# ddlee-cn/LeRF-PyTorch

Hardware: AMD Instinct MI355X
Metric: Mpix/s LeRF-G x2 SR (2K->4K) (higher is better)
Workload: dtype i32+f32 (u8 io); 1 GPU; LeRF-G LUT x2 SR, 1920x1080->3840x2160 RGB uint8, S=2, max_sigma=10 (BASELINE configs[1]); input=noise, mode=frames, parallelism=independent frames per GPU, no data-path collective, ranks_reported_by_rccl=1, channels=3, library=lerf-pytorch_amd/liblerf_hip.so

## Files before the change

### include/lerf_hip.h

```cpp
#ifndef LERF_HIP_H
#define LERF_HIP_H

#include <stddef.h>
#include <stdint.h>

#ifdef __cplusplus
extern "C" {
#endif

#define LERF_ABI_VERSION 7
#define LERF_MAX_MODES 5
#define LERF_LUT_ENTRIES 83521
#define LERF_MAX_SUPPORT 8

enum {
    LERF_OK = 0,
    LERF_EINVAL = -1,
    LERF_EUNSUPPORTED = -2,
    LERF_ELAUNCH = -3,
    LERF_ENODEVICE = -4
};

enum { LERF_U8 = 0, LERF_F32 = 1, LERF_F64 = 2, LERF_I16 = 3 };
enum {
    LERF_KIND_GAUSS = 0,
    LERF_KIND_LINEAR = 1,
    LERF_KIND_NEAREST = 2,
    LERF_KIND_CUBIC = 3,
    LERF_KIND_BILINEAR = 4,
    LERF_KIND_LANCZOS2 = 5,
    LERF_KIND_LANCZOS3 = 6
};

enum {
    LERF_PAD_CONSTANT = 0,
    LERF_PAD_EDGE = 1,
    LERF_PAD_REFLECT = 2,
    LERF_PAD_SYMMETRIC = 3,
    LERF_PAD_WRAP = 4
};

typedef struct {
    const void* ptr;
    int dtype;
    int64_t sy, sx, sc;
} lerf_plane_t;

typedef struct {
    void* ptr;
    int dtype;
    int64_t sy, sx, sc;
} lerf_mplane_t;

typedef struct {
    int n_modes1;
    int n_modes2;
    char modes1[LERF_MAX_MODES];
    char modes2[LERF_MAX_MODES];
    int oC;
    const int8_t* s1[LERF_MAX_MODES];
    const int8_t* s2[LERF_MAX_MODES][2];
    const void* fused_pack;
} lerf_luts_t;

typedef struct {
    int S;
    int out_h, out_w;
    const int32_t* left_r;
    const float* dis_r;
    const int32_t* left_c;
    const float* dis_c;
    const double* dis_r64;
    const double* dis_c64;
    int pad_mode;
    int tie_queue_cap;
    int roi_y, roi_x;
    int roi_h, roi_w;
    int flags;
    int out_row_pitch;
} lerf_sr_geo_t;
#define LERF_GEO_FORCE_GENERAL 1
#define LERF_GEO_SINGLE_LAUNCH 2
#define LERF_GEO_X2_TABLES 16
#define LERF_GEO_NO_PERSIST 32
#define LERF_GEO_TILE_ROWS_64 64
#define LERF_GEO_TILE_ROWS_32 128
#define LERF_GEO_TILE_ROWS_16 256
#define LERF_GEO_INPUT_DEVICE 4
#define LERF_GEO_INPUT_HOST 8

typedef struct {
    int S;
    int out_h, out_w;
    double minv[9];
    int pad_r_lo, pad_r_hi, pad_c_lo, pad_c_hi;
    int pad_mode;
    int out_y0, out_x0, src_y0;
} lerf_warp_geo_t;

#define LERF_REMAP_PADS_FROM_MAP (-1)
typedef struct {
    int S;
    int out_h, out_w;
    const void* coords;
    int coords_dtype;
    int64_t row_stride;
    int pad_mode;
    int pad_r_lo, pad_c_lo;
} lerf_remap_geo_t;

int lerf_abi_version(void);
const char* lerf_strerror(int code);

int lerf_device_count(void);

int lerf_mode_offsets(char mode, int rot, int8_t dy[4], int8_t dx[4]);

int lerf_sr_axis_tables(int n_in, int n_out, double scale, int S,
                        int32_t* left, double* dis64, float* dis32, int32_t* pads);

int lerf_sr_axis_tables_f32(int n_in, int n_out, double scale, int S, int32_t* left, float* dis32, int32_t* pads);

int lerf_out_size(int n_in, double scale);

int lerf_invert3x3(const double m[9], double out[9]);

int lerf_warp_pads(const double minv[9], int in_h, int in_w, int out_h, int out_w, int S,
                   int32_t pads[4]);


int lerf_lut_interp_i16(const lerf_plane_t* img, int img_h, int img_w, int C,
                        int h, int w, const int8_t dy[4], const int8_t dx[4],
                        const int8_t* lut, int oC, int interval, int16_t* out, void* stream);

int lerf_lut_interp(const lerf_plane_t* img, int img_h, int img_w, int C, int h, int w, const int8_t dy[4], const int8_t dx[4],
                    const int8_t* lut, int oC, int interval, const lerf_mplane_t* out, void* stream);

#define LERF_INTERP_ACCUMULATE 1
#define LERF_INTERP_LDS 2
#define LERF_INTERP_DIRECT 4
#define LERF_INTERP_TILE64 8
#define LERF_INTERP_TILE32 16
#define LERF_INTERP_LUT_PLANAR 32
#define LERF_LUT_PLANE_BYTES 83584
int lerf_lut_interp_ex(const lerf_plane_t* img, int img_h, int img_w, int C, int h, int w, const int8_t dy[4], const int8_t dx[4],
                       const int8_t* lut, int oC, int interval, const lerf_mplane_t* out, int flags, void* stream);

enum { LERF_EPI_DIV = 0, LERF_EPI_MUL = 1, LERF_EPI_ADD = 2, LERF_EPI_CLIP = 3, LERF_EPI_ROUND = 4 };
#define LERF_EPI_MAX_OPS 8
typedef struct { int op; double a, b; } lerf_epi_op_t;
int lerf_numer_epilogue_f32(const int16_t* acc, int64_t n, int interval, const lerf_epi_op_t* ops, int n_ops, float* out, void* stream);

size_t lerf_fused_lutpack_bytes(const lerf_luts_t* luts);
int lerf_fused_lutpack_build(const lerf_luts_t* luts, void* buf, void* stream);

int lerf_lut_stages_u8(const lerf_plane_t* img, int H, int W, int C,
                       const lerf_luts_t* luts,
                       const lerf_mplane_t* feat, const lerf_mplane_t* hyper,
                       void* stream);

int lerf_resize(const lerf_plane_t* feat, const lerf_plane_t hyper[3],
                int H, int W, int C, const lerf_sr_geo_t* geo,
                int kind, double max_sigma, const lerf_mplane_t* out, void* stream);

int lerf_warp(const lerf_plane_t* feat, const lerf_plane_t hyper[3],
              int H, int W, int C, const lerf_warp_geo_t* geo,
              int kind, double max_sigma, const lerf_mplane_t* out, void* stream);

int lerf_stages_packed_u8(const uint8_t* img, int64_t in_sn, int n, int H, int W, int C,
                          const lerf_luts_t* luts, uint32_t* packed, int64_t packed_sn,
                          void* workspace, size_t workspace_bytes, void* stream);

int lerf_unpack_stages(const uint32_t* packed, int64_t n_pxch, int oC, uint8_t* feat, uint8_t* hq, void* stream);

int lerf_warp_packed(const uint32_t* packed, int64_t packed_sn, int n, int H, int W, int C, const lerf_warp_geo_t* geo,
                     int kind, double max_sigma, const lerf_mplane_t* out, int64_t out_sn, void* stream);

int lerf_remap(const lerf_plane_t* feat, const lerf_plane_t hyper[3],
               int H, int W, int C, const lerf_remap_geo_t* geo,
               int kind, double max_sigma, const lerf_mplane_t* out, void* stream);
int lerf_remap_packed(const uint32_t* packed, int64_t packed_sn, int n, int H, int W, int C, const lerf_remap_geo_t* geo,
                      int kind, double max_sigma, const lerf_mplane_t* out, int64_t out_sn, void* stream);
int lerf_remap_host_geometry(const lerf_remap_geo_t* geo, int H, int W, double* gr, double* gc, int32_t* lr, int32_t* lc,
                             int32_t pads[2]);

int lerf_remap_batched(const lerf_plane_t* feat, const lerf_plane_t hyper[3], int H, int W, int C, const lerf_remap_geo_t* geo,
                       int n_maps, int64_t map_stride, int planes_per_map, int kind, double max_sigma, const lerf_mplane_t* out,
                       void* stream);
int lerf_remap_packed_batched(const uint32_t* packed, int64_t packed_sn, int n, int H, int W, int C, const lerf_remap_geo_t* geo,
                              int n_maps, int64_t map_stride, int kind, double max_sigma, const lerf_mplane_t* out, int64_t out_sn,
                              void* stream);

int lerf_warp_tile_boxes(const lerf_warp_geo_t* geo, int H, int W, int32_t* boxes);
int lerf_warp_fused_supported(int C, const lerf_luts_t* luts, const lerf_warp_geo_t* geo, int H, int W, int kind, double max_sigma);
int lerf_warp_fused_u8(const uint8_t* img, int64_t in_sn, int n, int H, int W, int C, const lerf_luts_t* luts, const lerf_warp_geo_t* geo,
                       const int32_t* tile_boxes, int kind, double max_sigma, uint8_t* out, int64_t out_sn, void* workspace,
                       size_t workspace_bytes, void* stream);

size_t lerf_sr_fused_workspace_bytes(int H, int W, int C, int n);
int lerf_sr_fused_u8(const uint8_t* img, int64_t in_sn, int n, int H, int W, int C,
                     const lerf_luts_t* luts, const lerf_sr_geo_t* geo,
                     int kind, double max_sigma,
                     uint8_t* out, int64_t out_sn, void* workspace, size_t workspace_bytes, void* stream);
int lerf_sr_fused_supported(int C, const lerf_luts_t* luts, const lerf_sr_geo_t* geo, int H, int W, int kind, double max_sigma);
// ... 336 lines not shown
```

### lerf-pytorch_amd/_lib.py

```python
from __future__ import annotations

import ctypes as C
import os

import numpy as np

_HERE = os.path.dirname(os.path.abspath(__file__))
LIB_PATH = os.path.join(_HERE, "liblerf_hip.so")

LERF_MAX_MODES = 5
LERF_LUT_ENTRIES = 83521
LERF_MAX_SUPPORT = 8
LERF_U8, LERF_F32, LERF_F64, LERF_I16 = 0, 1, 2, 3
KIND_GAUSS, KIND_LINEAR, KIND_NEAREST, KIND_CUBIC, KIND_BILINEAR, KIND_LANCZOS2, KIND_LANCZOS3 = range(7)
KINDS = {"gauss": KIND_GAUSS, "linear": KIND_LINEAR, "nearest": KIND_NEAREST, "cubic": KIND_CUBIC,
         "bilinear": KIND_BILINEAR, "lanczos2": KIND_LANCZOS2, "lanczos3": KIND_LANCZOS3}

PAD_MODES = {"constant": 0, "edge": 1, "replicate": 1, "reflect": 2, "symmetric": 3, "wrap": 4, "circular": 4}
NUMPY_PAD_MODES = ("constant", "edge", "reflect", "symmetric", "wrap")
TORCH_PAD_MODES = ("constant", "replicate", "reflect", "circular")


def pad_mode_code(name, allowed):
    if name not in allowed:
        raise NotImplementedError("pad_mode {!r} is not implemented (supported: {})".format(name, ", ".join(allowed)))
    return PAD_MODES[name]


EXPORTS = [
    "lerf_abi_version", "lerf_strerror", "lerf_device_count", "lerf_mode_offsets", "lerf_sr_axis_tables", "lerf_sr_axis_tables_f32",
    "lerf_out_size", "lerf_invert3x3", "lerf_warp_pads", "lerf_lut_interp_i16", "lerf_lut_interp", "lerf_lut_interp_ex", "lerf_numer_epilogue_f32", "lerf_fused_lutpack_bytes", "lerf_fused_lutpack_build",
    "lerf_lut_stages_u8",
    "lerf_resize", "lerf_warp", "lerf_sr_fused_workspace_bytes", "lerf_sr_fused_supported", "lerf_sr_fused_u8",
    "lerf_sr_ragged_workspace_bytes", "lerf_sr_fused_ragged_u8", "lerf_stages_ragged_workspace_bytes", "lerf_stages_packed_ragged_u8",
    "lerf_stages_packed_u8", "lerf_unpack_stages", "lerf_warp_packed", "lerf_rect_copy_u8",
    "lerf_warp_tile_boxes", "lerf_warp_fused_supported", "lerf_warp_fused_u8",
    "lerf_remap", "lerf_remap_packed", "lerf_remap_host_geometry", "lerf_remap_batched", "lerf_remap_packed_batched",
    "lerf_metric_y_sse_u8", "lerf_metric_ssim_y_u8", "lerf_metric_masked_sse_u8",
    "lerf_swf2lut_interp_f32", "lerf_swf2lut_interp_bwd_f32", "lerf_resize_bwd_f32", "lerf_warp_bwd", "lerf_remap_bwd",
    "lerf_remap_bwd_batched",
    "lerf_srnet_weight_floats", "lerf_srnet_to_lut", "lerf_srnet_fwd_f32", "lerf_srnet_bwd_workspace_bytes", "lerf_srnet_bwd_f32",
    "lerf_imdn_weight_floats", "lerf_imdn_workspace_bytes", "lerf_imdn_fwd_f32",
    "lerf_imdn_saved_bytes", "lerf_imdn_fwd_train_f32", "lerf_imdn_bwd_workspace_bytes", "lerf_imdn_bwd_f32",
    "lerf_rr_axis", "lerf_rr_adjoint_csr", "lerf_patch_batch_u8",
    "lerf_coords_build", "lerf_coords_build_host", "lerf_coords_mesh", "lerf_coords_mesh_host", "lerf_coords_mesh_bwd_workspace_bytes",
    "lerf_coords_mesh_bwd", "lerf_coords_compose", "lerf_coords_compose_host", "lerf_coords_invert", "lerf_coords_invert_host",
    "lerf_coords_invert_raster", "lerf_coords_invert_raster_host", "lerf_coords_compose_bwd", "lerf_coords_compose_bwd_host", "lerf_coords_invert_bwd", "lerf_coords_invert_bwd_host",
    "lerf_coords_build_dev", "lerf_coords_build_bwd_workspace_bytes", "lerf_coords_build_bwd", "lerf_coords_build_bwd_host", "lerf_coords_math", "lerf_coords_math_host",
    "lerf_coords_mesh_batched", "lerf_coords_mesh_batched_host", "lerf_coords_mesh_bwd_batched", "lerf_coords_compose_batched", "lerf_coords_compose_batched_host",
    "lerf_coords_invert_batched", "lerf_coords_invert_batched_host", "lerf_coords_invert_raster_batched", "lerf_coords_invert_raster_batched_host",
    "lerf_coords_compose_bwd_batched", "lerf_coords_compose_bwd_batched_host", "lerf_coords_invert_bwd_batched", "lerf_coords_invert_bwd_batched_host",
    "lerf_coords_reproject", "lerf_coords_reproject_host", "lerf_coords_reproject_bwd_workspace_bytes", "lerf_coords_reproject_bwd",
    "lerf_coords_reproject_bwd_host",
    "lerf_splat", "lerf_splat_host", "lerf_splat_bwd", "lerf_splat_bwd_host",
    "lerf_scatter_ordered_workspace_bytes", "lerf_splat_ordered", "lerf_splat_ordered_host",
    "lerf_coords_compose_bwd_ordered", "lerf_coords_compose_bwd_ordered_host", "lerf_coords_compose_bwd_batched_ordered",
    "lerf_coords_compose_bwd_batched_ordered_host", "lerf_coords_invert_bwd_ordered", "lerf_coords_invert_bwd_ordered_host",
    "lerf_coords_invert_bwd_batched_ordered", "lerf_coords_invert_bwd_batched_ordered_host",
    "lerf_scan_exclusive_u32_block", "lerf_scan_exclusive_u32_workspace_bytes", "lerf_scan_exclusive_u32", "lerf_scan_exclusive_u32_host",
    "lerf_ubench_lds_gather",
]


class LerfError(RuntimeError):
    pass


class Plane(C.Structure):
    _fields_ = [("ptr", C.c_void_p), ("dtype", C.c_int), ("sy", C.c_int64), ("sx", C.c_int64), ("sc", C.c_int64)]


class EpiOp(C.Structure):
    _fields_ = [("op", C.c_int), ("a", C.c_double), ("b", C.c_double)]


class Luts(C.Structure):
    _fields_ = [
        ("n_modes1", C.c_int), ("n_modes2", C.c_int),
        ("modes1", C.c_char * LERF_MAX_MODES), ("modes2", C.c_char * LERF_MAX_MODES),
        ("oC", C.c_int),
        ("s1", C.c_void_p * LERF_MAX_MODES),
        ("s2", (C.c_void_p * 2) * LERF_MAX_MODES),
        ("fused_pack", C.c_void_p),
    ]


class SrGeo(C.Structure):
    _fields_ = [
        ("S", C.c_int), ("out_h", C.c_int), ("out_w", C.c_int),
        ("left_r", C.c_void_p), ("dis_r", C.c_void_p), ("left_c", C.c_void_p), ("dis_c", C.c_void_p),
        ("dis_r64", C.c_void_p), ("dis_c64", C.c_void_p),
        ("pad_mode", C.c_int),
        ("tie_queue_cap", C.c_int),
        ("roi_y", C.c_int), ("roi_x", C.c_int), ("roi_h", C.c_int), ("roi_w", C.c_int),
        ("flags", C.c_int),
        ("out_row_pitch", C.c_int),
    ]


GEO_FORCE_GENERAL, GEO_SINGLE_LAUNCH, GEO_INPUT_DEVICE, GEO_INPUT_HOST, GEO_X2_TABLES, GEO_NO_PERSIST = 1, 2, 4, 8, 16, 32
GEO_TILE_ROWS_64, GEO_TILE_ROWS_32, GEO_TILE_ROWS_16 = 64, 128, 256


class SrItem(C.Structure):
    _fields_ = [("img", C.c_void_p), ("out", C.c_void_p), ("H", C.c_int), ("W", C.c_int), ("geo", SrGeo)]


class StageItem(C.Structure):
    _fields_ = [("img", C.c_void_p), ("packed", C.c_void_p), ("H", C.c_int), ("W", C.c_int)]


class Rect(C.Structure):
    _fields_ = [("y", C.c_int), ("x", C.c_int), ("h", C.c_int), ("w", C.c_int), ("off", C.c_int64)]


LERF_MAX_RECTS = 8


class WarpGeo(C.Structure):
    _fields_ = [
        ("S", C.c_int), ("out_h", C.c_int), ("out_w", C.c_int),
        ("minv", C.c_double * 9),
        ("pad_r_lo", C.c_int), ("pad_r_hi", C.c_int), ("pad_c_lo", C.c_int), ("pad_c_hi", C.c_int),
        ("pad_mode", C.c_int),
        ("out_y0", C.c_int), ("out_x0", C.c_int), ("src_y0", C.c_int),
    ]


REMAP_PADS_FROM_MAP = -1

COORDS_MODELS = {"homography": 0, "radial": 1, "brown": 2, "fisheye": 16, "equirect": 17}
COORDS_MODEL_PARAMS = {"homography": 9, "radial": 8, "brown": 21, "fisheye": 17, "equirect": 13}
COORDS_MATH_OPS = {"sqrt": 0, "atan": 1, "atan2": 2}
MESH_INTERPS = {"bilinear": 0, "bicubic": 1}


class RemapGeo(C.Structure):
    _fields_ = [
        ("S", C.c_int), ("out_h", C.c_int), ("out_w", C.c_int),
        ("coords", C.c_void_p), ("coords_dtype", C.c_int), ("row_stride", C.c_int64),
        ("pad_mode", C.c_int),
        ("pad_r_lo", C.c_int), ("pad_c_lo", C.c_int),
    ]


class RrAxis(C.Structure):
    _fields_ = [("n_in", C.c_int), ("n_out", C.c_int), ("taps", C.c_int), ("left", C.c_void_p), ("row_ptr", C.c_void_p),
                ("idx", C.c_void_p), ("w", C.c_void_p), ("pad_mode", C.c_int)]


class PatchDesc(C.Structure):
    _fields_ = [("lr_off", C.c_int64), ("hr_off", C.c_int64), ("lr_h", C.c_int32), ("lr_w", C.c_int32), ("lr_pitch", C.c_int32),
                ("hr_h", C.c_int32), ("hr_w", C.c_int32), ("hr_pitch", C.c_int32), ("li", C.c_int32), ("lj", C.c_int32),
                ("hi", C.c_int32), ("hj", C.c_int32), ("chan", C.c_int32), ("fliplr", C.c_int32), ("flipud", C.c_int32),
                ("k", C.c_int32)]


PATCH_DESC_DTYPE = np.dtype([(n, np.int64 if t is C.c_int64 else np.int32) for n, t in PatchDesc._fields_])
assert PATCH_DESC_DTYPE.itemsize == C.sizeof(PatchDesc) == 72


_lib = None


def use_library(path):
    global LIB_PATH
    if _lib is not None:
        raise LerfError("use_library(%s): liblerf_hip.so is already loaded from %s" % (path, LIB_PATH))
    LIB_PATH = os.path.abspath(path)


def lib():
    global _lib
    if _lib is not None:
        return _lib
    if not os.path.exists(LIB_PATH):
        raise LerfError(
            "liblerf_hip.so not found at %s -- build it with `python __graft_entry__.py` "
            "(hipcc --offload-arch=gfx950); there is no CPU fallback." % LIB_PATH)
    try:
        import torch
    except ImportError:
        pass
    L = C.CDLL(LIB_PATH)
    L.lerf_abi_version.restype = C.c_int
    L.lerf_strerror.restype = C.c_char_p
    L.lerf_strerror.argtypes = [C.c_int]
    L.lerf_device_count.restype = C.c_int
    L.lerf_mode_offsets.argtypes = [C.c_char, C.c_int, C.c_void_p, C.c_void_p]
    L.lerf_sr_axis_tables.argtypes = [C.c_int, C.c_int, C.c_double, C.c_int, C.c_void_p, C.c_void_p, C.c_void_p, C.c_void_p]
    L.lerf_sr_axis_tables_f32.argtypes = [C.c_int, C.c_int, C.c_double, C.c_int, C.c_void_p, C.c_void_p, C.c_void_p]
    L.lerf_out_size.argtypes = [C.c_int, C.c_double]
    L.lerf_invert3x3.argtypes = [C.c_void_p, C.c_void_p]
    L.lerf_warp_pads.argtypes = [C.c_void_p, C.c_int, C.c_int, C.c_int, C.c_int, C.c_int, C.c_void_p]
    L.lerf_lut_interp_i16.argtypes = [C.POINTER(Plane), C.c_int, C.c_int, C.c_int, C.c_int, C.c_int, C.c_void_p,
                                      C.c_void_p, C.c_void_p, C.c_int, C.c_int, C.c_void_p, C.c_void_p]
    L.lerf_lut_interp.argtypes = [C.POINTER(Plane), C.c_int, C.c_int, C.c_int, C.c_int, C.c_int, C.c_void_p,
                                  C.c_void_p, C.c_void_p, C.c_int, C.c_int, C.POINTER(Plane), C.c_void_p]
    L.lerf_lut_interp_ex.argtypes = [C.POINTER(Plane), C.c_int, C.c_int, C.c_int, C.c_int, C.c_int, C.c_void_p,
                                     C.c_void_p, C.c_void_p, C.c_int, C.c_int, C.POINTER(Plane), C.c_int, C.c_void_p]
    L.lerf_numer_epilogue_f32.argtypes = [C.c_void_p, C.c_int64, C.c_int, C.c_void_p, C.c_int, C.c_void_p, C.c_void_p]
    L.lerf_warp_tile_boxes.argtypes = [C.POINTER(WarpGeo), C.c_int, C.c_int, C.c_void_p]
    L.lerf_warp_fused_supported.argtypes = [C.c_int, C.POINTER(Luts), C.POINTER(WarpGeo), C.c_int, C.c_int, C.c_int, C.c_double]
    L.lerf_warp_fused_u8.argtypes = [C.c_void_p, C.c_int64, C.c_int, C.c_int, C.c_int, C.c_int, C.POINTER(Luts), C.POINTER(WarpGeo), C.c_void_p,
                                     C.c_int, C.c_double, C.c_void_p, C.c_int64, C.c_void_p, C.c_size_t, C.c_void_p]
    L.lerf_fused_lutpack_bytes.restype = C.c_size_t
    L.lerf_fused_lutpack_bytes.argtypes = [C.POINTER(Luts)]
    L.lerf_fused_lutpack_build.argtypes = [C.POINTER(Luts), C.c_void_p, C.c_void_p]
    L.lerf_lut_stages_u8.argtypes = [C.POINTER(Plane), C.c_int, C.c_int, C.c_int, C.POINTER(Luts),
                                     C.POINTER(Plane), C.POINTER(Plane), C.c_void_p]
    L.lerf_resize.argtypes = [C.POINTER(Plane), C.POINTER(Plane), C.c_int, C.c_int, C.c_int, C.POINTER(SrGeo),
                              C.c_int, C.c_double, C.POINTER(Plane), C.c_void_p]
    L.lerf_warp.argtypes = [C.POINTER(Plane), C.POINTER(Plane), C.c_int, C.c_int, C.c_int, C.POINTER(WarpGeo),
                            C.c_int, C.c_double, C.POINTER(Plane), C.c_void_p]
    L.lerf_stages_packed_u8.argtypes = [C.c_void_p, C.c_int64, C.c_int, C.c_int, C.c_int, C.c_int, C.POINTER(Luts),
                                        C.c_void_p, C.c_int64, C.c_void_p, C.c_size_t, C.c_void_p]
    L.lerf_unpack_stages.argtypes = [C.c_void_p, C.c_int64, C.c_int, C.c_void_p, C.c_void_p, C.c_void_p]
    L.lerf_warp_packed.argtypes = [C.c_void_p, C.c_int64, C.c_int, C.c_int, C.c_int, C.c_int, C.POINTER(WarpGeo), C.c_int, C.c_double,
                                   C.POINTER(Plane), C.c_int64, C.c_void_p]
    L.lerf_remap.argtypes = [C.POINTER(Plane), C.POINTER(Plane), C.c_int, C.c_int, C.c_int, C.POINTER(RemapGeo),
                             C.c_int, C.c_double, C.POINTER(Plane), C.c_void_p]
    L.lerf_remap_packed.argtypes = [C.c_void_p, C.c_int64, C.c_int, C.c_int, C.c_int, C.c_int, C.POINTER(RemapGeo), C.c_int, C.c_double,
                                    C.POINTER(Plane), C.c_int64, C.c_void_p]
    L.lerf_remap_batched.argtypes = [C.POINTER(Plane), C.POINTER(Plane), C.c_int, C.c_int, C.c_int, C.POINTER(RemapGeo), C.c_int,
                                     C.c_int64, C.c_int, C.c_int, C.c_double, C.POINTER(Plane), C.c_void_p]
    L.lerf_remap_packed_batched.argtypes = [C.c_void_p, C.c_int64, C.c_int, C.c_int, C.c_int, C.c_int, C.POINTER(RemapGeo), C.c_int,
                                            C.c_int64, C.c_int, C.c_double, C.POINTER(Plane), C.c_int64, C.c_void_p]
    L.lerf_remap_host_geometry.argtypes = [C.POINTER(RemapGeo), C.c_int, C.c_int, C.c_void_p, C.c_void_p, C.c_void_p, C.c_void_p,
                                           C.c_void_p]
    L.lerf_rect_copy_u8.argtypes = [C.c_void_p, C.c_int, C.c_int, C.c_int, C.c_int, C.c_void_p, C.POINTER(Rect), C.c_int, C.c_int,
                                    C.c_void_p]
    L.lerf_sr_fused_supported.argtypes = [C.c_int, C.POINTER(Luts), C.POINTER(SrGeo), C.c_int, C.c_int, C.c_int, C.c_double]
    L.lerf_sr_ragged_workspace_bytes.restype = C.c_size_t
    L.lerf_sr_ragged_workspace_bytes.argtypes = [C.POINTER(SrItem), C.c_int, C.c_int]
    L.lerf_sr_fused_ragged_u8.argtypes = [C.POINTER(SrItem), C.c_int, C.c_int, C.POINTER(Luts), C.c_int, C.c_double, C.c_void_p,
                                          C.c_size_t, C.c_void_p]
    L.lerf_stages_ragged_workspace_bytes.restype = C.c_size_t
    L.lerf_stages_ragged_workspace_bytes.argtypes = [C.POINTER(StageItem), C.c_int, C.c_int]
    L.lerf_stages_packed_ragged_u8.argtypes = [C.POINTER(StageItem), C.c_int, C.c_int, C.POINTER(Luts), C.c_void_p, C.c_size_t,
                                               C.c_void_p]
    L.lerf_sr_fused_workspace_bytes.restype = C.c_size_t
    L.lerf_sr_fused_workspace_bytes.argtypes = [C.c_int, C.c_int, C.c_int, C.c_int]
    L.lerf_sr_fused_u8.argtypes = [C.c_void_p, C.c_int64, C.c_int, C.c_int, C.c_int, C.c_int, C.POINTER(Luts),
                                   C.POINTER(SrGeo), C.c_int, C.c_double, C.c_void_p, C.c_int64, C.c_void_p, C.c_size_t, C.c_void_p]
    L.lerf_metric_y_sse_u8.argtypes = [C.c_void_p, C.c_int64, C.c_void_p, C.c_int64, C.c_int, C.c_int, C.c_int,
                                       C.c_void_p, C.c_void_p]
    L.lerf_metric_ssim_y_u8.argtypes = [C.c_void_p, C.c_int64, C.c_void_p, C.c_int64, C.c_int, C.c_int, C.c_void_p, C.c_void_p]
    L.lerf_metric_masked_sse_u8.argtypes = [C.c_void_p, C.c_void_p, C.c_void_p, C.c_int64, C.c_void_p, C.c_void_p]
    L.lerf_swf2lut_interp_f32.argtypes = [C.c_void_p, C.c_int, C.c_char, C.c_void_p, C.c_int, C.c_int, C.c_int, C.c_int,
                                          C.c_void_p, C.c_void_p]
    L.lerf_swf2lut_interp_bwd_f32.argtypes = [C.c_void_p, C.c_int, C.c_char, C.c_void_p, C.c_void_p, C.c_int, C.c_int, C.c_int,
                                              C.c_int, C.c_void_p, C.c_void_p, C.c_void_p]
    L.lerf_resize_bwd_f32.argtypes = [C.c_void_p, C.c_void_p, C.c_void_p, C.c_void_p, C.c_int, C.c_int, C.c_int, C.POINTER(SrGeo),
                                      C.c_int, C.c_double, C.c_void_p, C.c_void_p, C.c_void_p, C.c_void_p, C.c_void_p, C.c_void_p]
    L.lerf_warp_bwd.argtypes = [C.c_void_p, C.c_void_p, C.c_void_p, C.c_void_p, C.c_int, C.c_int, C.c_int, C.POINTER(WarpGeo),
                                C.c_int, C.c_double, C.c_void_p, C.c_void_p, C.c_void_p, C.c_void_p, C.c_void_p, C.c_void_p]
    L.lerf_remap_bwd.argtypes = [C.c_void_p, C.c_void_p, C.c_void_p, C.c_void_p, C.c_int, C.c_int, C.c_int, C.POINTER(RemapGeo),
                                 C.c_int, C.c_double, C.c_void_p, C.c_void_p, C.c_void_p, C.c_void_p, C.c_void_p, C.c_void_p, C.c_void_p]
    L.lerf_remap_bwd_batched.argtypes = [C.c_void_p, C.c_void_p, C.c_void_p, C.c_void_p, C.c_int, C.c_int, C.c_int, C.POINTER(RemapGeo),
                                         C.c_int, C.c_int64, C.c_int, C.c_int, C.c_double, C.c_void_p, C.c_void_p, C.c_void_p, C.c_void_p,
                                         C.c_void_p, C.c_void_p, C.c_void_p]
    L.lerf_srnet_weight_floats.restype = C.c_size_t
    L.lerf_srnet_weight_floats.argtypes = [C.c_int]
    L.lerf_srnet_to_lut.argtypes = [C.c_void_p, C.c_int, C.c_int, C.c_void_p, C.c_void_p, C.c_void_p]
    L.lerf_srnet_fwd_f32.argtypes = [C.c_void_p, C.c_int, C.c_char, C.c_void_p, C.c_int, C.c_int, C.c_int, C.c_int, C.c_void_p,
                                     C.c_void_p]
    L.lerf_srnet_bwd_workspace_bytes.restype = C.c_size_t
    L.lerf_srnet_bwd_workspace_bytes.argtypes = [C.c_int, C.c_int, C.c_int, C.c_int]
    L.lerf_srnet_bwd_f32.argtypes = [C.c_void_p, C.c_int, C.c_char, C.c_void_p, C.c_void_p, C.c_int, C.c_int, C.c_int, C.c_int,
                                     C.c_void_p, C.c_void_p, C.c_void_p, C.c_size_t, C.c_void_p]
    L.lerf_imdn_weight_floats.restype = C.c_size_t
    L.lerf_imdn_weight_floats.argtypes = [C.c_int, C.c_int, C.c_int]
    L.lerf_imdn_workspace_bytes.restype = C.c_size_t
    L.lerf_imdn_workspace_bytes.argtypes = [C.c_int, C.c_int, C.c_int, C.c_int]
# ... 45 lines not shown
        getattr(L, "lerf_coords_%s_batched" % name).argtypes = batched + [C.c_void_p]
        getattr(L, "lerf_coords_%s_batched_host" % name).argtypes = batched
    L.lerf_coords_mesh_bwd_batched.argtypes = L.lerf_coords_mesh_bwd.argtypes[:-1] + [C.c_int, C.c_int64, C.c_int64, C.c_void_p]
    _reproject = [C.c_int, C.c_void_p, C.c_int, C.c_void_p, C.c_int, C.c_int64, C.c_void_p, C.c_int, C.c_int64, C.c_int64, C.c_void_p, C.c_int64,
                  C.c_int, C.c_int, C.c_int, C.c_int]
    L.lerf_coords_reproject.argtypes, L.lerf_coords_reproject_host.argtypes = _reproject + [C.c_void_p], _reproject
    _reproject_bwd = [C.c_int, C.c_void_p, C.c_int, C.c_void_p, C.c_int, C.c_int64, C.c_void_p, C.c_void_p, C.c_int, C.c_int, C.c_int, C.c_int,
                      C.c_void_p, C.c_void_p]
    L.lerf_coords_reproject_bwd.argtypes = _reproject_bwd + [C.c_void_p, C.c_size_t, C.c_void_p]
    L.lerf_coords_reproject_bwd_host.argtypes = _reproject_bwd
    L.lerf_coords_reproject_bwd_workspace_bytes.restype = C.c_size_t
    L.lerf_coords_reproject_bwd_workspace_bytes.argtypes = [C.c_int] * 3
    _splat_in = [C.c_void_p, C.c_int, C.c_int, C.c_int, C.c_int, C.c_int64, C.c_void_p, C.c_int, C.c_int64, C.c_int64, C.c_void_p, C.c_int64]
    _splat = _splat_in + [C.c_void_p, C.c_int, C.c_int, C.c_int, C.c_int64, C.c_int]
    _splat_bwd = _splat_in + [C.c_void_p, C.c_int, C.c_int, C.c_int, C.c_int64] + [C.c_void_p, C.c_int64] * 3 + [C.c_int]
    L.lerf_splat.argtypes, L.lerf_splat_host.argtypes = _splat + [C.c_void_p], _splat
    L.lerf_splat_bwd.argtypes, L.lerf_splat_bwd_host.argtypes = _splat_bwd + [C.c_void_p], _splat_bwd
    _ordered = [C.c_void_p, C.c_size_t, C.c_int]
    L.lerf_scatter_ordered_workspace_bytes.restype = C.c_size_t
    L.lerf_scatter_ordered_workspace_bytes.argtypes = [C.c_int64, C.c_int64, C.c_int]
    L.lerf_splat_ordered.argtypes, L.lerf_splat_ordered_host.argtypes = _splat + _ordered + [C.c_void_p], _splat + _ordered
    for name, single, n_strides in (("compose_bwd", _compose_bwd, 5), ("invert_bwd", _invert_bwd, 4)):
        batched = single + [C.c_int] + [C.c_int64] * n_strides
        getattr(L, "lerf_coords_%s_ordered" % name).argtypes = single + _ordered + [C.c_void_p]
        getattr(L, "lerf_coords_%s_ordered_host" % name).argtypes = single + _ordered
        getattr(L, "lerf_coords_%s_batched_ordered" % name).argtypes = batched + _ordered + [C.c_void_p]
        getattr(L, "lerf_coords_%s_batched_ordered_host" % name).argtypes = batched + _ordered
    L.lerf_scan_exclusive_u32_workspace_bytes.restype = C.c_size_t
    L.lerf_scan_exclusive_u32_workspace_bytes.argtypes = [C.c_int64]
    L.lerf_scan_exclusive_u32.argtypes = [C.c_void_p, C.c_int64, C.c_void_p, C.c_size_t, C.c_void_p]
    L.lerf_scan_exclusive_u32_host.argtypes = [C.c_void_p, C.c_int64]
    L.lerf_ubench_lds_gather.argtypes = [C.c_int, C.c_int, C.c_int, C.c_void_p, C.c_void_p]
    for name in EXPORTS:
        getattr(L, name)
    if L.lerf_abi_version() != 7:
        raise LerfError("liblerf_hip.so ABI version mismatch")
    _lib = L
    return L


def check(rc: int, what: str = ""):
    if rc != 0:
        msg = lib().lerf_strerror(rc).decode()
        if rc == -1:
            raise ValueError("%s: %s" % (what, msg))
        raise LerfError("%s: %s (code %d)" % (what, msg, rc))


_MODE_OFFSETS = {}


def mode_offsets(mode: str, rot: int):
    hit = _MODE_OFFSETS.get((mode, int(rot)))
    if hit is not None:
        return hit[0].copy(), hit[1].copy()
    dy, dx = _mode_offsets(mode, rot)
    _MODE_OFFSETS[(mode, int(rot))] = (dy.copy(), dx.copy())
    return dy, dx


def _mode_offsets(mode: str, rot: int):
    dy = np.zeros(4, np.int8)
    dx = np.zeros(4, np.int8)
    rc = lib().lerf_mode_offsets(mode.encode()[:1] if mode else b"\0", int(rot), dy.ctypes.data, dx.ctypes.data)
    if rc != 0:
        raise ValueError("Mode {} not implemented.".format(mode))
    return dy, dx


def out_size(n_in: int, scale: float) -> int:
    return int(lib().lerf_out_size(int(n_in), float(scale)))


def sr_axis_tables(n_in: int, n_out: int, scale: float, S: int):
    left = np.zeros(n_out, np.int32)
    dis64 = np.zeros((n_out, S), np.float64)
    dis32 = np.zeros((n_out, S), np.float32)
    pads = np.zeros(2, np.int32)
    check(lib().lerf_sr_axis_tables(int(n_in), int(n_out), float(scale), int(S), left.ctypes.data,
                                    dis64.ctypes.data, dis32.ctypes.data, pads.ctypes.data), "lerf_sr_axis_tables")
    return left, dis64, dis32, (int(pads[0]), int(pads[1]))


def sr_axis_tables_f32(n_in: int, n_out: int, scale: float, S: int):
    left = np.zeros(n_out, np.int32)
    dis32 = np.zeros((n_out, S), np.float32)
    pads = np.zeros(2, np.int32)
    check(lib().lerf_sr_axis_tables_f32(int(n_in), int(n_out), float(scale), int(S), left.ctypes.data,
                                        dis32.ctypes.data, pads.ctypes.data), "lerf_sr_axis_tables_f32")
    return left, dis32.astype(np.float64), dis32, (int(pads[0]), int(pads[1]))


def warp_pads(minv: np.ndarray, in_hw, out_hw, S: int):
    m = np.ascontiguousarray(minv, dtype=np.float64).reshape(9)
    pads = np.zeros(4, np.int32)
    check(lib().lerf_warp_pads(m.ctypes.data, int(in_hw[0]), int(in_hw[1]), int(out_hw[0]), int(out_hw[1]), int(S),
                               pads.ctypes.data), "lerf_warp_pads")
    return tuple(int(p) for p in pads)


def remap_host_geometry(coords: np.ndarray, in_hw, S: int, pads=None):
    c = np.asarray(coords)
    if c.ndim != 3 or c.shape[2] != 2 or c.dtype not in (np.float32, np.float64):
        raise ValueError("coords must be a float32 / float64 [oH, oW, 2] array")
    c = np.ascontiguousarray(c)
    oH, oW = c.shape[:2]
    g = RemapGeo()
    g.S, g.out_h, g.out_w = int(S), oH, oW
    g.coords, g.coords_dtype, g.row_stride = c.ctypes.data, (LERF_F32 if c.dtype == np.float32 else LERF_F64), 2 * oW
    g.pad_r_lo, g.pad_c_lo = (REMAP_PADS_FROM_MAP, REMAP_PADS_FROM_MAP) if pads is None else (int(pads[0]), int(pads[1]))
    gr, gc = np.zeros((oH, oW), np.float64), np.zeros((oH, oW), np.float64)
    lr, lc = np.zeros((oH, oW), np.int32), np.zeros((oH, oW), np.int32)
    out = np.zeros(2, np.int32)
    check(lib().lerf_remap_host_geometry(C.byref(g), int(in_hw[0]), int(in_hw[1]), gr.ctypes.data, gc.ctypes.data, lr.ctypes.data,
                                         lc.ctypes.data, out.ctypes.data), "lerf_remap_host_geometry")
    return gr, gc, lr, lc, (int(out[0]), int(out[1]))


class _Operands:

    def is_float(self, a):
        return a.dtype == self.f32 or a.dtype == self.f64

    def code(self, a):
        return LERF_F32 if a.dtype == self.f32 else LERF_F64

    def map(self, a, what):
        if not self.is_array(a) or a.ndim != 3 or a.shape[2] != 2 or a.shape[0] < 1 or a.shape[1] < 1:
            raise ValueError("%s must be %s [h, w, 2]" % (what, self.noun))
        if not self.is_float(a):
            raise ValueError("%s must be float32 or float64, not %s" % (what, a.dtype))
        s = self.strides(a)
        if s[2] != 1 or s[1] != 2 or s[0] is None:
            raise ValueError("%s: contiguous (row, col) pairs, column stride 2" % what)
        return a, s[0]

    def out(self, out, out_hw, dtype, default, device, what):
        oH, oW = int(out_hw[0]), int(out_hw[1])
        if out is None:
            if oH < 1 or oW < 1:
                raise ValueError("%s: out_hw must be positive" % what)
            out = self.new((oH, oW, 2), self.dtype(dtype, default, what), device)
        elif tuple(out.shape[:2]) != (oH, oW):
            raise ValueError("%s: out must be [%d, %d, 2]" % (what, oH, oW))
        return self.map(out, "out")

    def batch(self, a, what, out=False):
        if not (self.is_array(a) and a.ndim == 4):
            a, s = self.map(a, what)
            return a, s, 0, 0
        if a.shape[3] != 2 or min(a.shape[:3]) < 1:
            raise ValueError("%s must be %s [B, h, w, 2]" % (what, self.noun))
        if not self.is_float(a):
            raise ValueError("%s must be float32 or float64, not %s" % (what, a.dtype))
        for copy in (False, True):
            if copy:
                if out:
                    raise ValueError("%s: contiguous (row, col) pairs, even row and set strides, sets that do not overlap" % what)
                a = self.contiguous(a)
            s = self.strides(a)
            B, h, w = a.shape[:3]
            if s[3] == 1 and s[2] == 2 and s[1] is not None and s[1] % 2 == 0 and s[1] >= 2 * w and (
                    B == 1 or (s[0] is not None and s[0] % 2 == 0 and s[0] >= (h - 1) * s[1] + 2 * w)):
                return a, s[1], (0 if B == 1 else s[0]), B
        raise ValueError("%s: contiguous (row, col) pairs, column stride 2" % what)

# ... 595 lines not shown
```

### lerf-pytorch_amd/csrc/lerf_api.hip

```cpp
#include <math.h>
#include <string.h>

#include "lerf_dispatch.h"
#include "lerf_kernels.h"
#include "lerf_remap_point.h"

using namespace lerf;

namespace {

inline hipStream_t as_stream(void* s) {
    clear_stale_error();
    return reinterpret_cast<hipStream_t>(s);
}

inline int check_launch() { return launch_status(); }

inline bool plane_ok(const lerf_plane_t* p) { return p && p->ptr; }

inline int hyper_count(int kind) { return kind == LERF_KIND_GAUSS ? 3 : (kind == LERF_KIND_LINEAR ? 1 : 0); }

inline bool hyper_planes_ok(const lerf_plane_t* hyper, int nh) {
    if (nh > 0 && !hyper) return false;
    for (int k = 0; k < nh; ++k)
        if (!hyper[k].ptr || hyper[k].dtype != hyper[0].dtype || hyper[k].sy != hyper[0].sy ||
            hyper[k].sx != hyper[0].sx || hyper[k].sc != hyper[0].sc)
            return false;
    return true;
}

void warp_operands(WarpArgs& a, const lerf_plane_t* feat, const lerf_plane_t* hyper, int nh, int H, int W, int C, int kind, double max_sigma,
                   const lerf_mplane_t* out) {
    a.feat = feat->ptr; a.in_dtype = feat->dtype; a.fy = feat->sy; a.fx = feat->sx; a.fc = feat->sc;
    for (int k = 0; k < 3; ++k) a.h[k] = nh > 0 ? (k < nh ? hyper[k].ptr : hyper[0].ptr) : feat->ptr;
    a.h_dtype = nh > 0 ? hyper[0].dtype : feat->dtype;
    a.hy = nh > 0 ? hyper[0].sy : 0; a.hx = nh > 0 ? hyper[0].sx : 0; a.hc = nh > 0 ? hyper[0].sc : 0;
    a.H = H; a.W = W; a.C = C;
    a.kind = kind; a.max_sigma = max_sigma;
    a.out = out->ptr; a.out_dtype = out->dtype; a.oy = out->sy; a.ox = out->sx; a.oc = out->sc;
}

int build_stage_luts(const lerf_luts_t* L, int stage, StageLuts* out) {
    int n = stage == 1 ? L->n_modes1 : L->n_modes2;
    if (n < 1 || n > LERF_MAX_MODES) return LERF_EINVAL;
    out->n_modes = n;
    for (int m = 0; m < n; ++m) {
        char mode = stage == 1 ? L->modes1[m] : L->modes2[m];
        for (int r = 0; r < 4; ++r)
            if (!mode_offsets(mode, r, out->off[m][r].dy, out->off[m][r].dx)) return LERF_EINVAL;
        if (stage == 1) {
            if (!L->s1[m]) return LERF_EINVAL;
            out->lut[m][0] = out->lut[m][1] = L->s1[m];
        } else {
            if (!L->s2[m][0] || !L->s2[m][1]) return LERF_EINVAL;
            out->lut[m][0] = L->s2[m][0];
            out->lut[m][1] = L->s2[m][1];
        }
    }
    return LERF_OK;
}

}

extern "C" {

int lerf_abi_version(void) { return LERF_ABI_VERSION; }

const char* lerf_strerror(int code) {
    switch (code) {
        case LERF_OK: return "ok";
        case LERF_EINVAL: return "invalid argument";
        case LERF_EUNSUPPORTED: return "unsupported configuration";
        case LERF_ELAUNCH: return "HIP launch failed";
        case LERF_ENODEVICE: return "no gfx950 device";
        default: return "unknown error";
    }
}

int lerf_device_count(void) {
    int n = 0;
    if (hipGetDeviceCount(&n) != hipSuccess) return LERF_ENODEVICE;
    return n;
}

int lerf_mode_offsets(char mode, int rot, int8_t dy[4], int8_t dx[4]) {
    if (!dy || !dx) return LERF_EINVAL;
    return mode_offsets(mode, rot, dy, dx) ? LERF_OK : LERF_EINVAL;
}

int lerf_out_size(int n_in, double scale) { return host::out_size(n_in, scale); }

int lerf_sr_axis_tables(int n_in, int n_out, double scale, int S, int32_t* left, double* dis64, float* dis32, int32_t* pads) {
    return host::sr_axis_tables(n_in, n_out, scale, S, left, dis64, dis32, pads);
}

int lerf_sr_axis_tables_f32(int n_in, int n_out, double scale, int S, int32_t* left, float* dis32, int32_t* pads) {
    return host::sr_axis_tables_f32(n_in, n_out, scale, S, left, dis32, pads);
}

int lerf_invert3x3(const double m[9], double out[9]) { return host::invert3x3(m, out); }

int lerf_warp_pads(const double minv[9], int in_h, int in_w, int out_h, int out_w, int S, int32_t pads[4]) {
    return host::warp_pads(minv, in_h, in_w, out_h, out_w, S, pads);
}

int lerf_lut_interp_i16(const lerf_plane_t* img, int img_h, int img_w, int C, int h, int w, const int8_t dy[4],
                        const int8_t dx[4], const int8_t* lut, int oC, int interval, int16_t* out, void* stream) {
    if (!out) return LERF_EINVAL;
    lerf_mplane_t o;
    o.ptr = out; o.dtype = LERF_I16; o.sy = w; o.sx = 1; o.sc = (int64_t)h * w;
    return lerf_lut_interp(img, img_h, img_w, C, h, w, dy, dx, lut, oC, interval, &o, stream);
}

int lerf_lut_interp(const lerf_plane_t* img, int img_h, int img_w, int C, int h, int w, const int8_t dy[4], const int8_t dx[4],
                    const int8_t* lut, int oC, int interval, const lerf_mplane_t* out, void* stream) {
    return lerf_lut_interp_ex(img, img_h, img_w, C, h, w, dy, dx, lut, oC, interval, out, 0, stream);
}

int lerf_lut_interp_ex(const lerf_plane_t* img, int img_h, int img_w, int C, int h, int w, const int8_t dy[4], const int8_t dx[4],
                       const int8_t* lut, int oC, int interval, const lerf_mplane_t* out, int flags, void* stream) {
    if (!plane_ok(img) || (img->dtype != LERF_U8 && img->dtype != LERF_F32) || !lut || !dy || !dx) return LERF_EINVAL;
    if (!out || !out->ptr || (out->dtype != LERF_I16 && out->dtype != LERF_F32 && out->dtype != LERF_F64)) return LERF_EINVAL;
    if (img_h < 1 || img_w < 1 || C < 1 || h < 1 || w < 1) return LERF_EINVAL;
    if (flags & ~(LERF_INTERP_ACCUMULATE | LERF_INTERP_LDS | LERF_INTERP_DIRECT | LERF_INTERP_TILE64 | LERF_INTERP_TILE32 | LERF_INTERP_LUT_PLANAR)) return LERF_EINVAL;
    if ((flags & LERF_INTERP_LDS) && (flags & LERF_INTERP_DIRECT)) return LERF_EINVAL;
    Offsets4 off;
    memcpy(off.dy, dy, 4);
    memcpy(off.dx, dx, 4);
    int rc = launch_lut_interp(img->ptr, img->dtype, img->sy, img->sx, img->sc, img_h, img_w, C, h, w, off, lut, oC, interval,
                               out->ptr, out->dtype, out->sy, out->sx, out->sc, flags, as_stream(stream));
    return rc != LERF_OK ? rc : check_launch();
}

int lerf_numer_epilogue_f32(const int16_t* acc, int64_t n, int interval, const lerf_epi_op_t* ops, int n_ops, float* out, void* stream) {
    if (!acc || !out || n < 1 || (n_ops > 0 && !ops)) return LERF_EINVAL;
    int rc = launch_numer_epilogue(acc, n, interval, ops, n_ops, out, as_stream(stream));
    return rc != LERF_OK ? rc : check_launch();
}

size_t lerf_fused_lutpack_bytes(const lerf_luts_t* luts) { return luts ? fused_lutpack_bytes(luts) : 0; }

int lerf_fused_lutpack_build(const lerf_luts_t* luts, void* buf, void* stream) {
    if (!luts || !buf) return LERF_EINVAL;
    if (fused_lutpack_bytes(luts) == 0) return LERF_EUNSUPPORTED;
    int rc = fused_lutpack_build(luts, buf, as_stream(stream));
    return rc != LERF_OK ? rc : check_launch();
}

int lerf_lut_stages_u8(const lerf_plane_t* img, int H, int W, int C, const lerf_luts_t* luts,
                       const lerf_mplane_t* feat, const lerf_mplane_t* hyper, void* stream) {
    if (!plane_ok(img) || img->dtype != LERF_U8 || !luts || H < 1 || W < 1 || C < 1) return LERF_EINVAL;
    if (!feat || !feat->ptr || feat->dtype != LERF_U8) return LERF_EINVAL;
    if (luts->oC != 1 && luts->oC != 3) return LERF_EUNSUPPORTED;
    StageLuts s1, s2;
    int rc = build_stage_luts(luts, 1, &s1);
    if (rc != LERF_OK) return rc;
    hipStream_t st = as_stream(stream);
    rc = launch_lut_stage((const uint8_t*)img->ptr, img->sy, img->sx, img->sc, H, W, C, s1, 1, kQ * luts->n_modes1, 0,
                          (uint8_t*)feat->ptr, feat->sy, feat->sx, feat->sc, st);
    if (rc != LERF_OK) return rc;
    if (hyper && hyper->ptr) {
        if (hyper->dtype != LERF_U8) return LERF_EINVAL;
        rc = build_stage_luts(luts, 2, &s2);
        if (rc != LERF_OK) return rc;
        rc = launch_lut_stage((const uint8_t*)feat->ptr, feat->sy, feat->sx, feat->sc, H, W, C, s2, luts->oC,
                              kQ * 4 * luts->n_modes2, 127, (uint8_t*)hyper->ptr, hyper->sy, hyper->sx, hyper->sc, st);
        if (rc != LERF_OK) return rc;
    }
    return check_launch();
}

int lerf_resize(const lerf_plane_t* feat, const lerf_plane_t hyper[3], int H, int W, int C, const lerf_sr_geo_t* geo,
                int kind, double max_sigma, const lerf_mplane_t* out, void* stream) {
    if (!plane_ok(feat) || !geo || !out || !out->ptr || H < 1 || W < 1 || C < 1) return LERF_EINVAL;
    if (kind < LERF_KIND_GAUSS || kind > LERF_KIND_LANCZOS3) return LERF_EUNSUPPORTED;
    const int nh = hyper_count(kind);
    if (!hyper_planes_ok(hyper, nh)) return LERF_EINVAL;
    if (!geo->left_r || !geo->left_c || geo->out_h < 1 || geo->out_w < 1) return LERF_EINVAL;
    ResizeArgs a{};
    a.feat = feat->ptr; a.in_dtype = feat->dtype; a.fy = feat->sy; a.fx = feat->sx; a.fc = feat->sc;
// ... 443 lines not shown
```

### lerf-pytorch_amd/csrc/lerf_fused.hip

```cpp
#define LERF_FUSED_NS fused
#define LERF_FUSED_CH 3
#define LERF_FUSED_WITH_WARP 1
#include "lerf_fused_impl.h"

namespace lerf {

static bool modes_ok(const char* m, int n) {
    if (n < 1 || n > fused::MAXM) return false;
    for (int i = 0; i < n; ++i)
        if (m[i] != 's' && m[i] != 'd' && m[i] != 'y' && m[i] != 'c' && m[i] != 't') return false;
    return true;
}
static bool luts_packable(const lerf_luts_t* L) {
    return L && (L->oC == 1 || L->oC == 3) && modes_ok(L->modes1, L->n_modes1) && modes_ok(L->modes2, L->n_modes2);
}

static bool fused_fast(const FusedArgs& a) {
    const lerf_luts_t* L = a.luts;
    if (a.C != 3 || a.items != nullptr) return false;
    if (a.flags & LERF_GEO_FORCE_GENERAL) return false;
    if (L->n_modes1 != 3 || L->n_modes2 != 3 || memcmp(L->modes1, "sct", 3) != 0 || memcmp(L->modes2, "sct", 3) != 0) return false;
    return (int64_t)a.oH <= 4 * (int64_t)a.H + 8 && (int64_t)a.oW <= 4 * (int64_t)a.W + 8;
}

static bool shape_ok(int H, int W, int oH, int oW) {
    if (oH < H || oW < W) return false;
    return (int64_t)oH <= 8 * (int64_t)H + 8 && (int64_t)oW <= 8 * (int64_t)W + 8;
}

bool fused_supported(const FusedArgs& a) {
    const lerf_luts_t* L = a.luts;
    if (!luts_packable(L) || !L->fused_pack) return false;
    if ((a.C != 1 && a.C != 3 && a.C != 4) || (a.S != 2 && a.S != 4)) return false;
    if (a.kind == LERF_KIND_LINEAR && a.S != 2) return false;
    if (a.kind == LERF_KIND_GAUSS && !(a.max_sigma <= s3::kNoShiftMaxSigma)) return false;
    if (a.pad_mode < LERF_PAD_CONSTANT || a.pad_mode > LERF_PAD_WRAP) return false;
    const bool roi = a.roi_h > 0 && a.roi_w > 0;
    if (a.pad_mode == LERF_PAD_WRAP && (a.workspace == nullptr || (a.flags & LERF_GEO_SINGLE_LAUNCH) || roi)) return false;
    if (a.items != nullptr) {
        if (a.n_items < 1 || roi) return false;
        for (int i = 0; i < a.n_items; ++i)
            if (a.items[i].H < 1 || a.items[i].W < 1 || !shape_ok(a.items[i].H, a.items[i].W, a.items[i].oH, a.items[i].oW)) return false;
        return true;
    }
    if (roi && (a.roi_y < 0 || a.roi_x < 0 || a.roi_y + a.roi_h > a.H || a.roi_x + a.roi_w > a.W)) return false;
    return shape_ok(roi ? a.roi_h : a.H, roi ? a.roi_w : a.W, a.oH, a.oW);
}

size_t fused_workspace_bytes(const FusedArgs& a) {
    if (a.items != nullptr) {
        size_t t = 0;
        for (int i = 0; i < a.n_items; ++i) t += ((size_t)a.items[i].H * a.items[i].W * a.C + 15) / 16 * 16;
        return t;
    }
    return (size_t)a.n * (((size_t)a.H * a.W * a.C + 15) / 16 * 16);
}

static int tile_rows_for(const FusedArgs& a) {
    if (a.flags & LERF_GEO_TILE_ROWS_64) return 64;
    if (a.flags & LERF_GEO_TILE_ROWS_32) return 32;
    if (a.flags & LERF_GEO_TILE_ROWS_16) return 16;
    auto tiles = [&](int th) {
        int64_t t = 0;
        if (a.items != nullptr) {
            for (int i = 0; i < a.n_items; ++i) t += (int64_t)((a.items[i].H + th - 1) / th) * ((a.items[i].W + 63) / 64);
            return t;
        }
        const bool roi = a.roi_h > 0 && a.roi_w > 0;
        return (int64_t)a.n * (((roi ? a.roi_h : a.H) + th - 1) / th) * (((roi ? a.roi_w : a.W) + 63) / 64);
    };
    constexpr int64_t kEnough = 192;
    if (tiles(64) >= kEnough) return 64;
    if (tiles(32) >= kEnough) return 32;
    return tiles(32) >= 96 ? 32 : 16;
}

int launch_sr_fused(const FusedArgs& a, hipStream_t st) {
    if (a.C == 1) return launch_sr_fused_c1(a, st);
    if (a.C == 4) return launch_sr_fused_c4(a, st);
    if (a.C != 3) return LERF_EUNSUPPORTED;
    const int th = tile_rows_for(a);
    if (th == 32) return launch_sr_fused_h32(a, st);
    if (th == 16) return launch_sr_fused_h16(a, st);
    return fused_fast(a) ? fused::launch_sr<false>(a, st) : launch_sr_fused_g3(a, st);
// ... 84 lines not shown
```

### lerf-pytorch_amd/csrc/lerf_fused_impl.h

```cpp
#include <string.h>
#include <atomic>
#include <type_traits>

#include "lerf_kernels.h"
#include "lerf_simplex_lds.h"
#include "lerf_stage3.h"
#include "lerf_warp_px.h"

namespace lerf {
namespace LERF_FUSED_NS {

constexpr int NT = 1024;
constexpr int NW = NT / 64;
constexpr int CH = LERF_FUSED_CH;
static_assert(CH == 1 || CH == 3 || CH == 4, "192 pixel-channels per tile row");
#ifndef LERF_FUSED_TH
#define LERF_FUSED_TH 64
#endif
constexpr int TH = LERF_FUSED_TH, TW = 192 / CH;
constexpr int R1 = 3, R2 = 3;
constexpr int MAXM = 4;
constexpr int LUT_PAD = 83584;
constexpr int NBIN = 3;
__host__ __device__ constexpr int bin_lo(int b) { return b == 0 ? 0 : (b == 1 ? 6 : (b == 2 ? 11 : 16)); }
// ... 1047 lines not shown
                uint32_t rb0 = lds_pixel_hi(cpa + (uint32_t)o0.o[0]), rc0 = lds_pixel_hi(cpa + (uint32_t)o0.o[1]),
                         rd0 = lds_pixel_hi(cpa + (uint32_t)o0.o[2]);
                uint32_t rb1 = lds_pixel_hi(cpa + (uint32_t)o1.o[0]), rc1 = lds_pixel_hi(cpa + (uint32_t)o1.o[1]),
                         rd1 = lds_pixel_hi(cpa + (uint32_t)o1.o[2]);
                asm volatile("s_waitcnt lgkmcnt(0)" : "+v"(ra), "+v"(rb0), "+v"(rc0), "+v"(rd0), "+v"(rb1), "+v"(rc1), "+v"(rd1));
                const int basea = (int)(__umul24(msb_of(ra), kStrideA * 4) + qbase);
                const unsigned ka = key_of(ra, st_a);
                const Walk<4> W0 = simplex_walk<4>(ka, basea, rb0, rc0, rd0, st_b, st_c, st_d);
                const Walk<4> W1 = simplex_walk<4>(ka, basea, rb1, rc1, rd1, st_b, st_c, st_d);
                uint32_t d0[5], d1[5];
#pragma unroll
                for (int n = 0; n < 5; ++n) d0[n] = W0.ld32(n);
#pragma unroll
                for (int n = 0; n < 5; ++n) d1[n] = W1.ld32(n);
                __builtin_amdgcn_sched_barrier(0);
                const unsigned w0[5] = {(unsigned)kQ - W0.f0, W0.f0 - W0.f1, W0.f1 - W0.f2, W0.f2 - W0.f3, W0.f3};
                const unsigned w1[5] = {(unsigned)kQ - W1.f0, W1.f0 - W1.f1, W1.f1 - W1.f2, W1.f2 - W1.f3, W1.f3};
                uint32_t a = accA[k], bb = accB[k];
#pragma unroll
                for (int n = 0; n < 5; ++n) {
                    a = mad_u24(w0[n], d0[n], a);
                    bb = mad_hi16(w0[n], d0[n], bb);
                }
#pragma unroll
                for (int n = 0; n < 5; ++n) {
                    a = mad_u24(w1[n], d1[n], a);
                    bb = mad_hi16(w1[n], d1[n], bb);
                }
                accA[k] = a;
                accB[k] = bb;
            }
        }
        __syncthreads();
        LERF_STAMP_ADD(9, t_look);
        if (++l == NL2) { l = 0; ++bi; }
    }
    LERF_STAMP(10);
    const int div2 = GEN ? kQ * 4 * P.n2 : kQ * 12;
#pragma unroll
    for (int k = 0; k < MAXR; ++k) {
        if ((vmask >> k) & 1u) {
            int n0 = (int)(accA[k] & 0xFFFFu) - div2;
            int n2 = (int)(accA[k] >> 16) - div2;
            int n1 = (int)((accB[k] - (accA[k] >> 16)) >> 8) - div2;
            uint32_t h0 = (uint32_t)rne_div_clip255_fast(n0, div2);
            uint32_t h1 = (uint32_t)rne_div_clip255_fast(n1, div2);
            uint32_t h2 = (uint32_t)rne_div_clip255_fast(n2, div2);
            const uint32_t a = (k & 1) ? (slot2[k >> 1] >> 16) : (slot2[k >> 1] & 0xFFFFu);
            const uint32_t row = a / (uint32_t)D::FP;
            const uint32_t p = a - row * (uint32_t)(D::FP - D::HP) - (uint32_t)(D::HO * D::HP + D::HO * CH);
            Dt[p] = h0 | (h1 << 8) | (h2 << 16) | ((uint32_t)Bt[a] << 24);
        }
    }
}

template <typename D, typename Outside>
__device__ __forceinline__ void fill_outside(uint32_t* Dt, int hy0, int hx0, int H, int W, int tid, Outside outside_pixel) {
    __syncthreads();
    for (int p = tid; p < D::NH; p += NT) {
        const int ry = p / D::HP, r3 = p - ry * D::HP, rx = r3 / CH, c = r3 - rx * CH;
        const int gy = hy0 + ry, gx = hx0 + rx;
        const int cy = clampi(gy, 0, H - 1), cx = clampi(gx, 0, W - 1);
        if (cy != gy || cx != gx)
            Dt[p] = (Dt[(cy - hy0) * D::HP + (cx - hx0) * CH + c] & 0x00FFFFFFu) | (outside_pixel(gy, gx, c) << 24);
    }
}

template <typename D>
__device__ __forceinline__ void emit_tile(const uint32_t* Dt, uint32_t* eo, int H, int W, int ty0, int tx0, int tid) {
    const int lane = tid & 63, wave = tid >> 6;
    __syncthreads();
    const int rows = min(TH, H - ty0), cols3 = min(TW, W - tx0) * CH;
    for (int il = wave; il < rows; il += NW) {
        const uint32_t* srow = Dt + (il + D::HR) * D::HP + D::HR * CH;
        uint32_t* drow = eo + ((int64_t)(ty0 + il) * W + tx0) * CH;
        for (int x = lane; x < cols3; x += 64) drow[x] = srow[x];
    }
}

struct MagicDiv {
    unsigned n, magic;
    __device__ __forceinline__ explicit MagicDiv(int n_)
        : n((unsigned)n_), magic((unsigned)((0x100000000ull + (unsigned)n_ - 1) / (unsigned)(n_ > 0 ? n_ : 1))) {}
    __device__ __forceinline__ int div(int t) const { return n == 1 ? t : (int)__umulhi((unsigned)t, magic); }
};

template <typename D, int S>
struct GeoTables {
    int* lr; float* dr; int* lc; float* dc; int* grp;
    __device__ __forceinline__ explicit GeoTables(uint8_t* smem)
        : lr(reinterpret_cast<int*>(smem + D::OFF_GEO)), dr(reinterpret_cast<float*>(lr + D::GEO_ROWS)), lc(reinterpret_cast<int*>(dr + D::GEO_ROWS * S)),
          dc(reinterpret_cast<float*>(lc + D::GEO_COLS)), grp(reinterpret_cast<int*>(dc + D::GEO_COLS * S)) {}
};

template <typename D>
__device__ __forceinline__ void stage3_geo_search(const FrameView& F, int tyi, int txi, int ty0, int tx0, int* ctl, int tid) {
    const int lane = tid & 63, wave = tid >> 6;
    if (wave < 4) {
        const bool rows = wave < 2;
        const int* tab = rows ? F.left_r : F.left_c;
        const int n = rows ? F.oH : F.oW;
        const int ti = rows ? tyi : txi, tn = rows ? F.tiles_y : F.tiles_x, t0 = rows ? ty0 : tx0;
        int r;
        if (!(wave & 1)) r = ti == 0 ? 0 : wave_lower_bound(tab, n, t0 - D::R3, lane);
        else r = ti == tn - 1 ? n : wave_lower_bound(tab, n, t0 + (rows ? TH : TW) - D::R3, lane);
        if (lane == 0) ctl[CTL_I0 + wave] = r;
    }
}
template <typename D, int S, int KIND>
__device__ __forceinline__ void stage3_geo_stage(uint8_t* smem, const FrameView& F, float max_sigma, int hy0, int hx0, const int* ctl,
                                                 int tid) {
    const GeoTables<D, S> g(smem);
    const int gi0 = ctl[CTL_I0], gi1 = ctl[CTL_I1], gj0 = ctl[CTL_J0], gj1 = ctl[CTL_J1];
    const float gscale = KIND == LERF_KIND_GAUSS ? s3::gauss_scale(max_sigma) : 1.0f;
    for (int e = tid; e < gi1 - gi0; e += NT) {
        g.lr[e] = F.left_r[gi0 + e] - hy0;
#pragma unroll
        for (int b = 0; b < S; ++b) g.dr[e * S + b] = F.dis_r[(gi0 + e) * S + b] * gscale;
    }
    for (int e = tid; e < gj1 - gj0; e += NT) {
        g.lc[e] = F.left_c[gj0 + e] - hx0;
#pragma unroll
        for (int a = 0; a < S; ++a) g.dc[e * S + a] = F.dis_c[(gj0 + e) * S + a] * gscale;
    }
}

template <typename D_, int S_, int KIND_>
struct Stage3 {
    using D = D_;
    static constexpr int S = S_, SS = S_ * S_, KIND = KIND_;
    static constexpr bool GAUSS = KIND_ == LERF_KIND_GAUSS;
    static constexpr int GMAX = S_ == 2 ? 5 : 3;
    static constexpr bool BLK = GAUSS && (S_ == 2 || S_ == 4) && D::OUT_FITS;
    static constexpr bool BLKL = KIND_ == LERF_KIND_LINEAR && S_ == 2 && D::OUT_FITS;
    static constexpr int QRP = S_ == 4 ? 2 : 1, QCP = S_ == 4 ? 2 : 1;
    static constexpr bool QUADS = BLK && QRP * QCP > 1;
    GeoTables<D, S> g;
    const uint32_t* Dt;
    uint32_t* tq; int* tq_count;
    uint8_t* outt;
    int* cgrp;
    const double* dis_r64; const double* dis_c64;
    uint8_t* seg0;
    int64_t rowpitch;
    bool rows_align;
    int i0, j0, nrow, ncol;
    int ncolc, ndw, ophase;
    MagicDiv by_ndw;
    int ngrp, gsame, rcode, ccode;
    bool lin_ok;

    __device__ __forceinline__ Stage3(uint8_t* smem, const Params& P, const FrameView& F, uint8_t* outp, int* ctl) : g(smem), by_ndw(1) {
        Dt = reinterpret_cast<const uint32_t*>(smem + D::OFF_D);
        tq = reinterpret_cast<uint32_t*>(smem + D::OFF_TQ);
        tq_count = ctl + CTL_TQ_COUNT;
        outt = smem + D::OFF_OUT;
        cgrp = reinterpret_cast<int*>(smem + D::OFF_CGRP);
        dis_r64 = F.dis_r64; dis_c64 = F.dis_c64;
        i0 = ctl[CTL_I0]; j0 = ctl[CTL_J0];
        nrow = ctl[CTL_I1] - i0; ncol = ctl[CTL_J1] - j0;
        ncolc = ncol * CH;
        rowpitch = P.out_pitch > 0 ? (int64_t)P.out_pitch : (int64_t)F.oW * CH;
        seg0 = outp + (int64_t)i0 * rowpitch + (int64_t)j0 * CH;
        rows_align = (rowpitch & 3) == 0;
        const bool seg_aligned = rows_align && (reinterpret_cast<uintptr_t>(seg0) & 3u) == 0;
        ndw = seg_aligned ? (ncolc + 3) >> 2 : (ncolc + 6) >> 2;
        ophase = (int)(reinterpret_cast<uintptr_t>(seg0) & 15u);
    }
    __device__ __forceinline__ void read_census(const int* ctl) {
        ngrp = ctl[CTL_NGRP];
        gsame = __builtin_amdgcn_readfirstlane(ctl[CTL_GSAME]);
        rcode = __builtin_amdgcn_readfirstlane(ctl[CTL_RCODE]); ccode = __builtin_amdgcn_readfirstlane(ctl[CTL_CCODE]);
        if constexpr (BLKL) lin_ok = ctl[CTL_LIN_ROWS_OK] != 0 && ctl[CTL_LIN_COLS_OK] != 0;
        else lin_ok = false;
        by_ndw = MagicDiv(ndw);
    }
};

__device__ __forceinline__ void pair_census(const int* t, int n, int lane, int* code, int* step) {
    bool ok0 = true, ok1 = true, step1 = true;
    for (int base = 0; base < n; base += 64) {
        const int k = base + lane;
        if (k + 1 < n && t[k + 1] != t[k]) { if (k & 1) ok1 = false; else ok0 = false; }
        if (!(k & 1) && k + 2 < n && t[k + 2] != t[k] + 1) step1 = false;
    }
    const bool p0 = __ballot(!ok0) == 0ull, p1 = __ballot(!ok1) == 0ull, q1 = __ballot(!step1) == 0ull;
    if (lane == 0) { *code = p0 ? 1 : (p1 ? 2 : 0); *step = q1 ? 1 : 0; }
}

template <typename X_>
__device__ __forceinline__ void stage3_census(const X_& X, int* ctl, int tid) {
    constexpr int KIND = X_::KIND, GMAX = X_::GMAX;
    const int lane = tid & 63, wave = tid >> 6;
    const int nrow = X.nrow, ncol = X.ncol;
    const int* g_lr = X.g.lr;
    const int* g_lc = X.g.lc;
    int* g_grp = X.g.grp;
    if (wave == 0) {
        int ng = 0;
        for (int base = 0; base < nrow; base += 64) {
            const int il = base + lane;
            bool start = false;
            if (il < nrow)
                start = il == 0 || !X.rows_align || g_lr[il] != g_lr[il - 1] || (il >= GMAX && g_lr[il - GMAX] == g_lr[il]);
            const unsigned long long m = __ballot(start);
            if (start) g_grp[ng + __builtin_amdgcn_mbcnt_hi((unsigned)(m >> 32), __builtin_amdgcn_mbcnt_lo((unsigned)m, 0u))] = il;
            ng += __popcll(m);
        }
        if (lane == 0) g_grp[ng] = nrow;
        const int g0 = ng > 0 ? g_grp[1] - g_grp[0] : 0;
        bool same = true, small = true;
        for (int base = 0; base < ng; base += 64) {
            const int idx = base + lane;
            if (idx < ng && g_grp[idx + 1] - g_grp[idx] != g0) same = false;
            if (X_::BLKL && idx < ng && g_grp[idx + 1] - g_grp[idx] > 2) small = false;
        }
        const bool uniform = __ballot(!same) == 0ull;
        if (lane == 0) {
            ctl[CTL_NGRP] = ng;
            ctl[CTL_GSAME] = uniform ? g0 : 0;
            ctl[CTL_TQ_COUNT] = 0;
        }
        if constexpr (X_::BLKL) {
            const bool ok = __ballot(!small) == 0ull;
            if (lane == 0) ctl[CTL_LIN_ROWS_OK] = ok ? 1 : 0;
        }
    } else if (wave == 1 && X_::BLKL) {
        int* g_cgrp = X.cgrp;
        constexpr int NCMAX = 2 * TW + 14;
        int nc = 0;
        for (int base = 0; base < ncol; base += 64) {
            const int jl = base + lane;
            bool start = false;
            if (jl < ncol) {
                int back = 0;
                while (back < 16 && jl - back - 1 >= 0 && g_lc[jl - back - 1] == g_lc[jl]) ++back;
                start = (back & 1) == 0;
            }
            const unsigned long long m = __ballot(start);
            if (start) {
                const int idx = nc + (int)__builtin_amdgcn_mbcnt_hi((unsigned)(m >> 32), __builtin_amdgcn_mbcnt_lo((unsigned)m, 0u));
                if (idx < NCMAX) g_cgrp[idx] = jl;
            }
            nc += __popcll(m);
        }
        if (lane == 0) {
            if (nc <= NCMAX) g_cgrp[nc] = ncol;
            ctl[CTL_NCGRP] = nc;
            ctl[CTL_LIN_COLS_OK] = (nc <= NCMAX) ? 1 : 0;
        }
    } else if (wave == 1) {
        pair_census(g_lc, ncol, lane, &ctl[CTL_CCODE], &ctl[CTL_CSTEP]);
    } else if (wave == 2 && KIND == LERF_KIND_GAUSS) {
        pair_census(g_lr, nrow, lane, &ctl[CTL_RCODE], &ctl[CTL_RSTEP]);
    }
}

template <typename X_>
__device__ __forceinline__ uint8_t resolve_output(const X_& X, float max_sigma, int il, int xc) {
    using D = typename X_::D;
    constexpr int S = X_::S;
    const int jl = xc / CH;
    const int c = xc - jl * CH;
    const uint32_t* dp = X.Dt + X.g.lr[il] * D::HP + X.g.lc[jl] * CH + c;
    return s3::resolve_taps_u8<X_::GAUSS, S>([&](int a, int b) __attribute__((always_inline)) { return dp[b * D::HP + a * CH]; },
                                            X.dis_r64 + (int64_t)(X.i0 + il) * S, X.dis_c64 + (int64_t)(X.j0 + jl) * S, max_sigma);
}
template <int N>
__device__ __forceinline__ unsigned tie_mask(const float (&dist)[N]) {
    unsigned m = 0;
#pragma unroll
    for (int q = 0; q < N; ++q)
        if (__builtin_fabsf(dist[q]) > 0.5f - s3::kTieEps) m |= 1u << q;
    return m;
}
template <typename X_, typename Decode, typename Patch>
__device__ __forceinline__ void queue_ties(const X_& X, const Params& P, unsigned mask, Decode decode, Patch patch) {
    while (mask != 0) {
        const int q = __builtin_ctz(mask);
        mask &= mask - 1;
        int il, xc;
        decode(q, il, xc);
        const int slot = atomicAdd(X.tq_count, 1);
        if (slot < P.tq_cap) {
            X.tq[slot] = ((uint32_t)il << 16) | (uint32_t)xc;
            continue;
        }
        patch(q, resolve_output(X, P.max_sigma, il, xc));
    }
}
__device__ __forceinline__ void put_block_byte(float xf, bool have, uint8_t* dst, float& dist, float& dmax) {
    const float rr = __builtin_rintf(xf);
    dist = have ? xf - rr : 0.0f;
    dmax = __builtin_fmaxf(dmax, __builtin_fabsf(dist));
    if (have) *dst = (uint8_t)__builtin_amdgcn_cvt_pk_u8_f32(rr, 0u, 0u);
}

template <int GS, typename X_>
__device__ __forceinline__ void stage3_tasks(const X_& X, const Params& P, int tid) {
    using D = typename X_::D;
    constexpr int S = X_::S, SS = X_::SS, KIND = X_::KIND;
    constexpr int GN = GS > 0 ? GS : X_::GMAX;
    const int* g_lr = X.g.lr; const float* g_dr = X.g.dr; const int* g_lc = X.g.lc; const float* g_dc = X.g.dc; const int* g_grp = X.g.grp;
    const uint32_t* Dt = X.Dt;
    const int ndw = X.ndw, ncolc = X.ncolc;
    const int64_t rowpitch = X.rowpitch;
    const float ms255 = P.max_sigma * (1.0f / 255.0f);
    const int ntask = X.ngrp * ndw;
    for (int t = tid; t < ntask; t += NT) {
        const int g = X.by_ndw.div(t);
        const int dw = t - g * ndw;
        const int il0 = g_grp[g];
        const int gs = GS > 0 ? GS : g_grp[g + 1] - il0;
        uint8_t* seg = X.seg0 + il0 * rowpitch;
        const int a0 = (int)(reinterpret_cast<uintptr_t>(seg) & 3u);
        const int b0 = dw * 4 - a0;
        const int lr = g_lr[il0];
        uint32_t packed[GN];
        constexpr bool DIST = S == 2;
        float dist[DIST ? GN * 4 : 1];
        float dmax = 0.0f;
        unsigned tiebits = 0;
#pragma unroll
        for (int r = 0; r < GN; ++r) packed[r] = 0;
        s3::f2 DXP[S];
        if constexpr (KIND == LERF_KIND_GAUSS && S == 4 && GS == 2) {
#pragma unroll
            for (int b = 0; b < S; ++b) { DXP[b].x = g_dr[il0 * S + b]; DXP[b].y = g_dr[(il0 + 1) * S + b]; }
        }
#pragma unroll
        for (int u = 0; u < 4; ++u) {
            const int xc = min(max(b0 + u, 0), ncolc - 1);
            const int jl = xc / CH;
            const int c = xc - jl * CH;
            const int lc = g_lc[jl];
            if constexpr (KIND == LERF_KIND_GAUSS && S == 4 && GS == 2) {
                s3::f2 PT[SS], KV[SS];
#pragma unroll
                for (int a = 0; a < S; ++a) {
                    const float dy = g_dc[jl * S + a];
#pragma unroll
                    for (int b = 0; b < S; ++b) {
                        const uint32_t d = Dt[(lr + b) * D::HP + (lc + a) * CH + c];
                        const float tyv = s3::gauss_t_u8((float)((d >> 16) & 0xFFu), dy);
                        PT[a * S + b].x = s3::gauss_m2rho_u8((float)(d & 0xFFu)) * tyv;
                        PT[a * S + b].y = tyv * tyv;
                        KV[a * S + b].x = (float)((d >> 8) & 0xFFu);
                        KV[a * S + b].y = (float)(d >> 24);
                    }
                }
                s3::f2 NUM, DEN;
#pragma unroll
                for (int a = 0; a < S; ++a)
#pragma unroll
                    for (int b = 0; b < S; ++b) {
                        const int k = a * S + b;
                        const s3::f2 TX = s3::pk_mul_blo(DXP[b], KV[k]);
                        const s3::f2 E = s3::pk_fma_pb<false>(TX, PT[k], s3::pk_fma_ppb<true>(TX, PT[k]));
                        s3::f2 W;
                        W.x = __builtin_amdgcn_exp2f(-E.x);
                        W.y = __builtin_amdgcn_exp2f(-E.y);
                        if (k == 0) {
                            DEN = W;
                            NUM = s3::pk_mul_bhi_after_trans(W, KV[k]);
                        } else {
                            DEN = DEN + W;
                            NUM = s3::pk_fma_bhi_after_trans(W, KV[k], NUM);
                        }
                    }
#pragma unroll
                for (int r = 0; r < 2; ++r) {
                    const float xf = s3::finish_div(r ? NUM.y : NUM.x, r ? DEN.y : DEN.x);
                    bool tie;
                    packed[r] = s3::pack_u8_tie(xf, u, packed[r], &tie);
                    if (tie) tiebits |= 1u << (r * 4 + u);
                }
                continue;
            }
            float p0[SS], k1[SS], ty[SS], v[SS];
#pragma unroll
            for (int a = 0; a < S; ++a) {
                const float dy = g_dc[jl * S + a];
#pragma unroll
                for (int b = 0; b < S; ++b) {
                    const uint32_t d = Dt[(lr + b) * D::HP + (lc + a) * CH + c];
                    v[a * S + b] = (float)(d >> 24);
                    const float k0 = (float)(d & 0xFFu);
                    if (KIND == LERF_KIND_GAUSS) {
                        const float tyv = s3::gauss_t_u8((float)((d >> 16) & 0xFFu), dy);
                        p0[a * S + b] = s3::gauss_m2rho_u8(k0) * tyv;
                        k1[a * S + b] = (float)((d >> 8) & 0xFFu);
                        ty[a * S + b] = tyv * tyv;
                    } else {
                        const float alpha = s3::lin_alpha_u8(k0, ms255);
                        p0[a * S + b] = alpha;
                        ty[a * S + b] = s3::lin_factor(alpha, dy, s3::dist_class_f(dy));
                        k1[a * S + b] = 0.0f;
                    }
                }
            }
#pragma unroll
            for (int r = 0; r < GN; ++r) {
                if (r < gs) {
                    float e[SS];
#pragma unroll
                    for (int a = 0; a < S; ++a)
#pragma unroll
                        for (int b = 0; b < S; ++b) {
                            const float dx = g_dr[(il0 + r) * S + b];
                            if (KIND == LERF_KIND_GAUSS)
                                e[a * S + b] = s3::gauss_form_cols(s3::gauss_t_u8(k1[a * S + b], dx), ty[a * S + b], p0[a * S + b]);
                            else
                                e[a * S + b] = s3::lin_factor(p0[a * S + b], dx, s3::dist_class_f(dx)) * ty[a * S + b];
                        }
                    const float xf = s3::finish<KIND == LERF_KIND_GAUSS, SS, true, true, true>(e, v);
                    if (DIST) {
                        packed[r] = s3::pack_u8_dist(xf, u, packed[r], &dist[DIST ? r * 4 + u : 0]);
                        dmax = __builtin_fmaxf(dmax, __builtin_fabsf(dist[DIST ? r * 4 + u : 0]));
                    } else {
                        bool tie;
                        packed[r] = s3::pack_u8_tie(xf, u, packed[r], &tie);
                        if (tie) tiebits |= 1u << (r * 4 + u);
                    }
                }
            }
        }
        if ((DIST ? dmax > 0.5f - s3::kTieEps : tiebits != 0) && X.dis_r64 != nullptr) {
            unsigned tiemask = tiebits;
            if (DIST) {
#pragma unroll
                for (int q = 0; q < GN * 4; ++q)
                    if ((GS > 0 || (q >> 2) < gs) && __builtin_fabsf(dist[DIST ? q : 0]) > 0.5f - s3::kTieEps) tiemask |= 1u << q;
            }
            queue_ties(X, P, tiemask,
                       [&](int q, int& il, int& xc) __attribute__((always_inline)) { il = il0 + (q >> 2); xc = min(max(b0 + (q & 3), 0), ncolc - 1); },
                       [&](int q, uint32_t r8) __attribute__((always_inline)) {
                           const int r = q >> 2, u = q & 3;
#pragma unroll
                           for (int rr = 0; rr < GN; ++rr)
                               packed[rr] = rr == r ? (packed[rr] & ~(0xFFu << (8 * u))) | (r8 << (8 * u)) : packed[rr];
                       });
        }
#pragma unroll
        for (int r = 0; r < GN; ++r) {
            if (r < gs) {
                uint8_t* sr = seg + r * rowpitch;
                if (b0 >= 0 && b0 + 3 < ncolc) {
                    __builtin_nontemporal_store(packed[r], reinterpret_cast<uint32_t*>(sr + b0));
                } else {
#pragma unroll
                    for (int u = 0; u < 4; ++u)
                        if (b0 + u >= 0 && b0 + u < ncolc) sr[b0 + u] = (uint8_t)(packed[r] >> (8 * u));
                }
            }
        }
    }
}

template <bool UNI, typename X_>
__device__ __forceinline__ void stage3_blocks(const X_& X, const Params& P, int tid) {
    if constexpr (X_::BLK) {
        using D = typename X_::D;
        constexpr int S = X_::S;
        const int* g_lr = X.g.lr; const float* g_dr = X.g.dr; const int* g_lc = X.g.lc; const float* g_dc = X.g.dc;
        const int nrow = X.nrow, ncol = X.ncol, ophase = X.ophase;
        const int rofs = UNI ? 0 : X.rcode - 1, cofs = UNI ? 0 : X.ccode - 1;
        const int ncg = (ncol + cofs + 1) >> 1;
        const int nblk = ((nrow + rofs + 1) >> 1) * ncg;
        const MagicDiv by_ncg(ncg);
        for (int t = tid; t < nblk; t += NT) {
            const int g = by_ncg.div(t);
            const int h = t - g * ncg;
            const int il0 = 2 * g - rofs, jl0 = 2 * h - cofs;
            const int lr = g_lr[UNI ? il0 : max(il0, 0)], lc = g_lc[UNI ? jl0 : max(jl0, 0)];
            s3::f2 DX[S], DY[S];
#pragma unroll
            for (int b = 0; b < S; ++b) { DX[b].x = g_dr[il0 * S + b]; DX[b].y = g_dr[il0 * S + S + b]; }
#pragma unroll
            for (int a = 0; a < S; ++a) { DY[a].x = g_dc[jl0 * S + a]; DY[a].y = g_dc[jl0 * S + S + a]; }
            const uint32_t* dp = X.Dt + lr * D::HP + lc * CH;
            uint8_t* ob = X.outt + il0 * D::OUT_PITCH + ophase + jl0 * CH;
            float dist[4 * CH];
            float dmax = 0.0f;
#pragma unroll
            for (int c = 0; c < CH; ++c) {
                s3::f2 NUM[2], DEN[2];
#pragma unroll
                for (int a = 0; a < S; ++a)
#pragma unroll
                    for (int b = 0; b < S; ++b) {
                        const s3::BlockTap T(dp[b * D::HP + a * CH + c]);
                        s3::f2 P0, TY2;
                        T.cols(DY[a], P0, TY2);
                        T.sum(T.rows(DX[b]), P0, TY2, a == 0 && b == 0, NUM, DEN);
                    }
#pragma unroll
                for (int r = 0; r < 2; ++r)
#pragma unroll
                    for (int q = 0; q < 2; ++q) {
                        const float den = q ? DEN[r].y : DEN[r].x, num = q ? NUM[r].y : NUM[r].x;
                        const bool have = UNI || ((unsigned)(il0 + r) < (unsigned)nrow && (unsigned)(jl0 + q) < (unsigned)ncol);
                        put_block_byte(s3::finish_div(num, den), have, ob + r * D::OUT_PITCH + q * CH + c, dist[(c * 2 + r) * 2 + q], dmax);
                    }
            }
            if (dmax > 0.5f - s3::kTieEps && X.dis_r64 != nullptr)
                queue_ties(X, P, tie_mask(dist),
                           [&](int q, int& il, int& xc) __attribute__((always_inline)) { il = il0 + ((q >> 1) & 1); xc = (jl0 + (q & 1)) * CH + (q >> 2); },
                           [&](int q, uint32_t r8) __attribute__((always_inline)) { ob[((q >> 1) & 1) * D::OUT_PITCH + (q & 1) * CH + (q >> 2)] = (uint8_t)r8; });
        }
    }
}

template <typename X_>
__device__ __forceinline__ void stage3_quads(const X_& X, const Params& P, int tid) {
    if constexpr (X_::QUADS) {
        using D = typename X_::D;
        constexpr int S = X_::S, RP = X_::QRP, CP = X_::QCP, TR = S + RP - 1, TC = S + CP - 1;
        const int* g_lr = X.g.lr; const float* g_dr = X.g.dr; const int* g_lc = X.g.lc; const float* g_dc = X.g.dc;
        const int ophase = X.ophase;
        const int ncq = (X.ncol >> 1) / CP;
        const int ntq = ((X.nrow >> 1) / RP) * ncq;
        const MagicDiv by_ncq(ncq);
        for (int t = tid; t < ntq; t += NT) {
            const int g = by_ncq.div(t);
            const int h = t - g * ncq;
            const int il0 = 2 * RP * g, jl0 = 2 * CP * h;
            const int lr = g_lr[il0], lc = g_lc[jl0];
            s3::f2 DX[RP][S], DY[CP][S];
#pragma unroll
            for (int rp = 0; rp < RP; ++rp)
#pragma unroll
                for (int b = 0; b < S; ++b) { DX[rp][b].x = g_dr[(il0 + 2 * rp) * S + b]; DX[rp][b].y = g_dr[(il0 + 2 * rp + 1) * S + b]; }
#pragma unroll
            for (int cp = 0; cp < CP; ++cp)
#pragma unroll
                for (int a = 0; a < S; ++a) { DY[cp][a].x = g_dc[(jl0 + 2 * cp) * S + a]; DY[cp][a].y = g_dc[(jl0 + 2 * cp + 1) * S + a]; }
            const uint32_t* dp = X.Dt + lr * D::HP + lc * CH;
            uint8_t* ob = X.outt + il0 * D::OUT_PITCH + ophase + jl0 * CH;
#pragma unroll 1
            for (int c = 0; c < CH; ++c) {
                s3::f2 NUM[RP][CP][2], DEN[RP][CP][2];
#pragma unroll
                for (int A = 0; A < TC; ++A) {
#pragma unroll
                    for (int B = 0; B < TR; ++B) {
                        const s3::BlockTap T(dp[B * D::HP + A * CH + c]);
                        s3::f2 P0[CP], TY2[CP], TX[RP];
#pragma unroll
                        for (int cp = 0; cp < CP; ++cp) {
                            const int a = A - cp;
                            if (a >= 0 && a < S) T.cols(DY[cp][a < 0 ? 0 : (a >= S ? 0 : a)], P0[cp], TY2[cp]);
                        }
#pragma unroll
                        for (int rp = 0; rp < RP; ++rp) {
                            const int b = B - rp;
                            if (b >= 0 && b < S) TX[rp] = T.rows(DX[rp][b < 0 ? 0 : (b >= S ? 0 : b)]);
                        }
#pragma unroll
                        for (int cp = 0; cp < CP; ++cp) {
                            const int a = A - cp;
                            if (a < 0 || a >= S) continue;
#pragma unroll
                            for (int rp = 0; rp < RP; ++rp) {
                                const int b = B - rp;
                                if (b < 0 || b >= S) continue;
                                T.sum(TX[rp], P0[cp], TY2[cp], a == 0 && b == 0, NUM[rp][cp], DEN[rp][cp]);
                            }
                        }
                    }
                }
                float dist[RP * CP * 4];
                float dmax = 0.0f;
#pragma unroll
                for (int rp = 0; rp < RP; ++rp)
#pragma unroll
                    for (int cp = 0; cp < CP; ++cp)
#pragma unroll
                        for (int r = 0; r < 2; ++r)
#pragma unroll
                            for (int q = 0; q < 2; ++q) {
                                const float den = q ? DEN[rp][cp][r].y : DEN[rp][cp][r].x, num = q ? NUM[rp][cp][r].y : NUM[rp][cp][r].x;
                                put_block_byte(s3::finish_div(num, den), true, ob + (2 * rp + r) * D::OUT_PITCH + (2 * cp + q) * CH + c,
                                               dist[((rp * CP + cp) * 2 + r) * 2 + q], dmax);
                            }
                if (dmax > 0.5f - s3::kTieEps && X.dis_r64 != nullptr)
                    queue_ties(X, P, tie_mask(dist),
                               [&](int k, int& il, int& xc) __attribute__((always_inline)) {
                                   const int rp = (k >> 2) / CP, cp = (k >> 2) - rp * CP;
                                   il = il0 + 2 * rp + ((k >> 1) & 1);
                                   xc = (jl0 + 2 * cp + (k & 1)) * CH + c;
                               },
                               [&](int k, uint32_t r8) __attribute__((always_inline)) {
                                   const int rp = (k >> 2) / CP, cp = (k >> 2) - rp * CP;
                                   ob[(2 * rp + ((k >> 1) & 1)) * D::OUT_PITCH + (2 * cp + (k & 1)) * CH + c] = (uint8_t)r8;
                               });
            }
        }
    }
}

template <typename X_>
__device__ __forceinline__ void stage3_blocks_lin(const X_& X, const Params& P, const int* ctl, int tid) {
    if constexpr (X_::BLKL) {
        using D = typename X_::D;
        const int* g_lr = X.g.lr; const float* g_dr = X.g.dr; const int* g_lc = X.g.lc; const float* g_dc = X.g.dc; const int* g_grp = X.g.grp;
        const int* g_cgrp = X.cgrp;
        const int ophase = X.ophase;
        const float ms255 = P.max_sigma * (1.0f / 255.0f);
        const int ncg = __builtin_amdgcn_readfirstlane(ctl[CTL_NCGRP]);
        const int nblk = X.ngrp * ncg;
        const MagicDiv by_ncg(ncg);
        for (int t = tid; t < nblk; t += NT) {
            const int g = by_ncg.div(t);
            const int h = t - g * ncg;
            const int il0 = g_grp[g], jl0 = g_cgrp[h];
            const bool two_r = g_grp[g + 1] - il0 > 1, two_c = g_cgrp[h + 1] - jl0 > 1;
            const int lr = g_lr[il0], lc = g_lc[jl0];
            float ax[2][2], mx[2][2], ay[2][2], my[2][2];
            auto abs_and_mask = [](const float* d, float (&a)[2][2], float (&m)[2][2]) __attribute__((always_inline)) {
#pragma unroll
                for (int k = 0; k < 4; ++k) {
                    a[k >> 1][k & 1] = __builtin_fabsf(d[k]);
                    m[k >> 1][k & 1] = s3::dist_class_f(d[k]) != 0 ? 1.0f : 0.0f;
                }
            };
            abs_and_mask(g_dr + il0 * 2, ax, mx);
            abs_and_mask(g_dc + jl0 * 2, ay, my);
            const uint32_t* dp = X.Dt + lr * D::HP + lc * CH;
            uint8_t* ob = X.outt + il0 * D::OUT_PITCH + ophase + jl0 * CH;
            float dist[4 * CH];
            float dmax = 0.0f;
#pragma unroll
            for (int c = 0; c < CH; ++c) {
                float v[4], fy[2][4], fx[2][4];
#pragma unroll
                for (int a = 0; a < 2; ++a)
#pragma unroll
                    for (int b = 0; b < 2; ++b) {
                        const uint32_t d = dp[b * D::HP + a * CH + c];
                        v[a * 2 + b] = (float)(d >> 24);
                        const float alpha = s3::lin_alpha_u8((float)(d & 0xFFu), ms255);
#pragma unroll
                        for (int q = 0; q < 2; ++q) fy[q][a * 2 + b] = s3::lin_factor_abs(alpha, ay[q][a], my[q][a]);
#pragma unroll
                        for (int r = 0; r < 2; ++r) fx[r][a * 2 + b] = s3::lin_factor_abs(alpha, ax[r][b], mx[r][b]);
                    }
#pragma unroll
                for (int r = 0; r < 2; ++r)
#pragma unroll
                    for (int q = 0; q < 2; ++q) {
                        float e[4];
#pragma unroll
                        for (int k = 0; k < 4; ++k) e[k] = fx[r][k] * fy[q][k];
                        const bool have = (r == 0 || two_r) && (q == 0 || two_c);
                        put_block_byte(s3::finish<false, 4, true, true, true>(e, v), have, ob + r * D::OUT_PITCH + q * CH + c,
                                       dist[(c * 2 + r) * 2 + q], dmax);
                    }
            }
            if (dmax > 0.5f - s3::kTieEps && X.dis_r64 != nullptr)
                queue_ties(X, P, tie_mask(dist),
                           [&](int q, int& il, int& xc) __attribute__((always_inline)) { il = il0 + ((q >> 1) & 1); xc = (jl0 + (q & 1)) * CH + (q >> 2); },
                           [&](int q, uint32_t r8) __attribute__((always_inline)) { ob[((q >> 1) & 1) * D::OUT_PITCH + (q & 1) * CH + (q >> 2)] = (uint8_t)r8; });
        }
    }
}

template <typename X_>
__device__ __forceinline__ void flush_blocks(const X_& X, int tid) {
    using D = typename X_::D;
    typedef uint32_t v4u __attribute__((ext_vector_type(4)));
    const int ophase = X.ophase, ncolc = X.ncolc, nrow = X.nrow;
    const int64_t rowpitch = X.rowpitch;
    const uint8_t* outt = X.outt;
    const int nchunk = (ophase + ncolc + 15) >> 4;
    const MagicDiv by_nchunk(nchunk);
    uint8_t* gbase = X.seg0 - ophase;
    const int total = nrow * nchunk;
    const int full_lo = ophase == 0 ? 0 : 1, full_hi = ((ophase + ncolc) & 15) == 0 ? nchunk : nchunk - 1;
    for (int i = tid; i < total; i += NT) {
        const int row = by_nchunk.div(i);
        const int ch = i - row * nchunk;
        if (ch >= full_lo && ch < full_hi) {
            const v4u x = *reinterpret_cast<const v4u*>(outt + row * D::OUT_PITCH + ch * 16);
            uint8_t* dst = gbase + row * rowpitch + ch * 16;
            const uintptr_t line = reinterpret_cast<uintptr_t>(dst) & ~(uintptr_t)63;
            const uintptr_t r0 = reinterpret_cast<uintptr_t>(gbase + row * rowpitch) + (uintptr_t)ophase;
            if (line >= r0 && line + 64 <= r0 + (uintptr_t)ncolc) __builtin_nontemporal_store(x, reinterpret_cast<v4u*>(dst));
            else *reinterpret_cast<v4u*>(dst) = x;
        }
    }
    for (int i = tid; i < 2 * nrow; i += NT) {
        const int row = i >> 1;
        const int ch = (i & 1) ? nchunk - 1 : 0;
        if (ch >= full_lo && ch < full_hi) continue;
        if ((i & 1) && nchunk == 1) continue;
        const uint8_t* src = outt + row * D::OUT_PITCH + ch * 16;
        uint8_t* dst = gbase + row * rowpitch + ch * 16;
        const int lo = max(ophase - ch * 16, 0), hi = min(ophase + ncolc - ch * 16, 16);
        const v4u x = *reinterpret_cast<const v4u*>(src);
#pragma unroll
        for (int k = 0; k < 4; ++k) {
            const uint32_t w = x[k];
            if (lo <= 4 * k && hi >= 4 * k + 4) {
                *reinterpret_cast<uint32_t*>(dst + 4 * k) = w;
            } else {
#pragma unroll
                for (int u = 0; u < 4; ++u)
                    if (4 * k + u >= lo && 4 * k + u < hi) dst[4 * k + u] = (uint8_t)(w >> (8 * u));
            }
        }
    }
}

template <bool IMAGE, typename X_>
__device__ __forceinline__ void stage3_ties(const X_& X, const Params& P, int tid) {
    using D = typename X_::D;
    if (IMAGE) {
        __syncthreads();
        LERF_STAMP(15);
    }
    if (X.dis_r64 == nullptr) return;
    if (!IMAGE) {
        asm volatile("s_waitcnt vmcnt(0)" ::: "memory");
        __syncthreads();
    }
    const int nq = min(*X.tq_count, P.tq_cap);
    for (int i = tid; i < nq; i += NT) {
        const uint32_t e = X.tq[i];
        const int il = (int)(e >> 16), xc = (int)(e & 0xFFFFu);
        const uint8_t r8 = resolve_output(X, P.max_sigma, il, xc);
        if (IMAGE) X.outt[il * D::OUT_PITCH + X.ophase + xc] = r8;
        else X.seg0[il * X.rowpitch + xc] = r8;
    }
    if (IMAGE && nq > 0) __syncthreads();
}

constexpr int LERF_FUSED_WARP = 16;
template <int S, int KINDW, bool EMIT, bool FROM_FEAT = false, bool GEN = false>
__global__ void __launch_bounds__(NT)
sr_fused_kernel(Params P, std::conditional_t<GEN, RaggedTable, NoTable> T) {
    constexpr int KIND = KINDW & 15;
    constexpr bool WARP = (KINDW & LERF_FUSED_WARP) != 0;
    static_assert(!WARP || (!EMIT && S == 2 && CH == 3 && !GEN), "tile-fused warp: RGB, 2 x 2 support, specialised kernel");
    using D = Dims<S, GEN, EMIT>;
    extern __shared__ __attribute__((aligned(16))) uint8_t smem[];
    const int tid = threadIdx.x;

    int bid = xcd_order((int)blockIdx.x, (int)gridDim.x);
    const FrameView F = frame_view<GEN>(P, T, bid);
    const int tyi = bid / F.tiles_x, txi = bid - tyi * F.tiles_x;
    const int ty0 = P.ty_org + tyi * TH, tx0 = P.tx_org + txi * TW;
    const int H = F.H, W = F.W;
    const uint8_t* __restrict__ img = F.img;
    uint8_t* __restrict__ outp = F.out;

    const int hy0 = ty0 - D::HR, hx0 = tx0 - D::HR;
    const int fy0 = ty0 - D::R3 - R2, fx0 = tx0 - D::R3 - R2;
    const int iy0 = fy0 - R1, ix0 = fx0 - R1;

    uint8_t* Bt = smem + D::OFF_B;
    int* ctl = reinterpret_cast<int*>(smem + D::OFF_CTL);
    const bool interior = FROM_FEAT ? (fy0 >= 0 && fx0 >= 0 && fy0 + D::FY <= F.H && fx0 + D::FX <= F.W)
                                    : (iy0 >= 0 && ix0 >= 0 && iy0 + D::IY <= F.H && ix0 + D::IX <= F.W);
    const int Hc = interior ? -1 : F.H, Wc = F.W;

    LERF_STAMP_RT(13);
    LERF_STAMP(0);
#ifdef LERF_STAMPS
    if (tid == 0) { P.stamps[(size_t)blockIdx.x * 16 + 8] = 0; P.stamps[(size_t)blockIdx.x * 16 + 9] = 0; P.stamps[(size_t)blockIdx.x * 16 + 15] = 0; }
#endif
    auto geo_search = [&]() { stage3_geo_search<D>(F, tyi, txi, ty0, tx0, ctl, tid); };
    auto geo_stage = [&]() { stage3_geo_stage<D, S, KIND>(smem, F, P.max_sigma, hy0, hx0, ctl, tid); };
    auto early_search = [&]() { if (D::GEO_EARLY && !EMIT && !WARP) geo_search(); };
    if constexpr (!FROM_FEAT) {
        stage1<D, GEN, false, false>(smem, P, img, H, W, fy0, fx0, interior, Bt, tid, early_search, [&](int k) {
            if (k == 0) {
                if (D::GEO_EARLY && !EMIT && !WARP) geo_stage();
                LERF_STAMP(1);
            } else {
                LERF_STAMP(1 + k);
            }
        });
    } else {
        load_feat_tile<D>(Bt, F.feat, H, W, fy0, fx0, interior, tid, early_search);
        __syncthreads();
        if (D::GEO_EARLY && !EMIT && !WARP) geo_stage();
        LERF_STAMP(6);
    }

    uint32_t* Dt = reinterpret_cast<uint32_t*>(smem + D::OFF_D);

    const int pad_mode = P.pad_mode;
    auto outside_pixel = [&](int gy, int gx, int c) -> uint32_t {
        if (pad_mode == LERF_PAD_CONSTANT) return 0u;
        bool zy, zx;
        const int sy = pad_index(gy, H, pad_mode, &zy), sx = pad_index(gx, W, pad_mode, &zx);
        const int ry = sy - fy0, rx = sx - fx0;
        if (ry >= 0 && ry < D::FY && rx >= 0 && rx < D::FX) return (uint32_t)Bt[ry * D::FP + rx * CH + c];
        if (FROM_FEAT) return (uint32_t)F.feat[((int64_t)sy * W + sx) * CH + c];
        return 0u;
    };

    if constexpr (KIND == LERF_KIND_LINEAR)
        stage2_linear<D, GEN, FROM_FEAT>(smem, P, Bt, Dt, F.feat, W, hy0, hx0, fy0, fx0, interior, Hc, Wc, tid, outside_pixel);
    else
        stage2_gauss<D, GEN>(smem, P, Bt, Dt, hy0, hx0, fy0, fx0, Hc, Wc, tid);
    if (!EMIT && !WARP && KIND == LERF_KIND_GAUSS && Hc >= 0) fill_outside<D>(Dt, hy0, hx0, H, W, tid, outside_pixel);

    if constexpr (WARP) {
        __syncthreads();
        warp_tile<KIND, D::HP>(P, Dt, hy0, hx0, ty0, tx0, H, W, tyi * F.tiles_x + txi, outp, tid);
        return;
    }
    if (EMIT) {
        emit_tile<D>(Dt, F.emit, H, W, ty0, tx0, tid);
        return;
    }

    if (!D::GEO_EARLY) {
        geo_search();
        __syncthreads();
        geo_stage();
    }
    __syncthreads();
    using X3 = Stage3<D, S, KIND>;
    X3 X(smem, P, F, outp, ctl);
    LERF_STAMP(11);
    stage3_census(X, ctl, tid);
    __syncthreads();
    X.read_census(ctl);
    const bool image_ok = X.rows_align && (X.rowpitch & 15) == 0 && X.nrow <= D::OUT_ROWS && X.ophase + X.ncolc <= D::OUT_PITCH;
    const bool blk = X3::BLK && image_ok && X.rcode != 0 && X.ccode != 0;
    const bool blk_uni = blk && X.rcode == 1 && X.ccode == 1 && ((X.nrow | X.ncol) & 1) == 0;
    const bool quad = X3::QUADS && blk_uni && __builtin_amdgcn_readfirstlane(ctl[CTL_CSTEP]) != 0 && __builtin_amdgcn_readfirstlane(ctl[CTL_RSTEP]) != 0 &&
                      ((X.nrow >> 1) % X3::QRP) == 0 && ((X.ncol >> 1) % X3::QCP) == 0;
    const bool blkl = X3::BLKL && __builtin_amdgcn_readfirstlane((image_ok && X.lin_ok) ? 1 : 0) != 0;
    constexpr bool WIDE = KIND == LERF_KIND_GAUSS && S == 2;
    if (quad) stage3_quads(X, P, tid);
    else if (blk_uni) stage3_blocks<true>(X, P, tid);
    else if (blk) stage3_blocks<false>(X, P, tid);
    else if (blkl) stage3_blocks_lin(X, P, ctl, tid);
    else if (X.gsame == 2) stage3_tasks<2>(X, P, tid);
    else if (WIDE && X.gsame == 3) stage3_tasks<WIDE ? 3 : 0>(X, P, tid);
    else if (WIDE && X.gsame == 4) stage3_tasks<WIDE ? 4 : 0>(X, P, tid);
    else stage3_tasks<0>(X, P, tid);
    if (blk || blkl) {
        stage3_ties<true>(X, P, tid);
        flush_blocks(X, tid);
    } else {
        stage3_ties<false>(X, P, tid);
    }
#ifdef LERF_STAMPS
    __syncthreads();
    LERF_STAMP(12);
    LERF_STAMP_RT(14);
#endif
}

constexpr int up16c(int x) { return (x + 15) / 16 * 16; }
struct DimsA {
    static constexpr int FY = TH, FX = TW, FP = FX * CH, NF = FY * FP;
    static constexpr int IY = FY + 2 * R1, IX = FX + 2 * R1, IPB = IX * CH, IP = (IPB + 3 + 3) / 4 * 4, NI = IY * IP;
    static constexpr int OFF_LUT = 0;
    static constexpr int OFF_C = LUT_PAD;
    static constexpr int OFF_ACC = OFF_C + up16c(NI);
    static constexpr int OFF_F = OFF_ACC + up16c(NF * 2);
    static constexpr int LDS_BYTES = OFF_F + up16c(NF);
};

template <bool GEN = false>
__global__ void __launch_bounds__(NT)
s1_kernel(Params P, std::conditional_t<GEN, RaggedTable, NoTable> T) {
    using D = DimsA;
    extern __shared__ __attribute__((aligned(16))) uint8_t smem[];
    const int tid = threadIdx.x;
    int bid = xcd_order((int)blockIdx.x, (int)gridDim.x);
    const FrameView F = frame_view<GEN>(P, T, bid);
    const int tyi = bid / F.tiles_x, txi = bid - tyi * F.tiles_x;
    const int fy0 = P.ty_org + tyi * TH, fx0 = P.tx_org + txi * TW;
    const int iy0 = fy0 - R1, ix0 = fx0 - R1;
    const int H = F.H, W = F.W;
    const uint8_t* __restrict__ img = F.img;
    const bool interior = iy0 >= 0 && ix0 >= 0 && iy0 + D::IY <= H && ix0 + D::IX <= W;
    uint8_t* Ft = smem + D::OFF_F;
    LERF_STAMP(0);
    stage1<D, GEN, true, true>(smem, P, img, H, W, fy0, fx0, interior, Ft, tid, []() {}, NoMark{});
    LERF_STAMP(1);
    uint8_t* __restrict__ fdst = F.feat;
    const int rows = min(TH, H - fy0), cols3 = min(TW, W - fx0) * CH;
    const bool dwords = cols3 == D::FP && ((W * CH) & 3) == 0 && (reinterpret_cast<uintptr_t>(F.feat) & 3) == 0;
    if (dwords) {
        constexpr int RD = D::FP / 4;
        uint32_t* dst = reinterpret_cast<uint32_t*>(fdst + ((int64_t)fy0 * W + fx0) * CH);
        const int rowdw = (W * CH) >> 2;
        for (int i = tid; i < rows * RD; i += NT) {
            const int r = i / RD;
            __builtin_nontemporal_store(reinterpret_cast<const uint32_t*>(Ft)[i], &dst[(int64_t)r * rowdw + (i - r * RD)]);
        }
    } else {
        for (int i = tid; i < rows * cols3; i += NT) {
            const int r = i / cols3, c3 = i - r * cols3;
            fdst[((int64_t)(fy0 + r) * W + fx0) * CH + c3] = Ft[r * D::FP + c3];
        }
    }
#ifdef LERF_STAMPS
    __syncthreads();
    LERF_STAMP(2);
#endif
}

#undef LERF_ADDTID
#undef LERF_ADDTID4
#undef LERF_SET_M0


template <auto KERN>
static int ensure_lds(int bytes) {
    static std::atomic<uint64_t> done{0};
    int dev = 0;
    if (hipGetDevice(&dev) != hipSuccess) return LERF_ELAUNCH;
    const uint64_t bit = 1ull << (dev & 63);
    if (done.load(std::memory_order_relaxed) & bit) return LERF_OK;
    if (hipFuncSetAttribute(reinterpret_cast<const void*>(KERN), hipFuncAttributeMaxDynamicSharedMemorySize, bytes) != hipSuccess)
        return LERF_ELAUNCH;
    done.fetch_or(bit, std::memory_order_relaxed);
    return LERF_OK;
}

inline size_t feat_slice_bytes(int H, int W) { return ((size_t)H * W * CH + 15) / 16 * 16; }

template <int S, int KIND, bool EMIT, bool GEN>
static int launch_fused_t(const FusedArgs& a, hipStream_t st) {
    using D = Dims<S, GEN, EMIT>;
    using TableT = std::conditional_t<GEN, RaggedTable, NoTable>;
    const lerf_luts_t* L = a.luts;
    Params P{};
    P.tq_cap = a.tq_cap == 0 ? D::TQ_CAP : (a.tq_cap < 0 ? 0 : (a.tq_cap > D::TQ_CAP ? D::TQ_CAP : a.tq_cap));
    P.pad_mode = a.pad_mode;
    P.host_input = a.host_input ? 1 : 0;
    P.out_pitch = a.out_pitch;
    P.img = a.img; P.in_sn = a.in_sn; P.out = a.out; P.out_sn = a.out_sn;
    P.H = a.H; P.W = a.W; P.oH = a.oH; P.oW = a.oW;
    const bool roi = a.roi_h > 0 && a.roi_w > 0;
    P.ty_org = roi ? a.roi_y : 0; P.tx_org = roi ? a.roi_x : 0;
    P.tiles_y = ((roi ? a.roi_h : a.H) + TH - 1) / TH;
    P.tiles_x = ((roi ? a.roi_w : a.W) + TW - 1) / TW;
    P.pack = (const uint8_t*)L->fused_pack;
    P.left_r = a.left_r; P.dis_r = a.dis_r; P.left_c = a.left_c; P.dis_c = a.dis_c;
    P.dis_r64 = a.dis_r64; P.dis_c64 = a.dis_c64;
    P.max_sigma = a.max_sigma;
    P.n1 = L->n_modes1; P.n2 = L->n_modes2;
    P.stamps = EMIT ? nullptr : (unsigned long long*)a.workspace;
    for (int l = 0; l < 2 * P.n2; ++l) {
        const char mc = L->modes2[l >> 1];
        const Off3 o0 = tile_offsets<D::FP>(mc, l & 1), o1 = tile_offsets<D::FP>(mc, (l & 1) + 2);
        for (int i = 0; i < 3; ++i) {
            P.s2off[l][i] = o0.o[i];
            P.s2off[l][3 + i] = o1.o[i];
        }
    }
    for (int m = 0; m < P.n1; ++m)
        for (int r = 0; r < 4; ++r) {
            const DyDx q = pattern_dydx(L->modes1[m], r);
            for (int i = 0; i < 3; ++i) P.s1dyx[m][3 * r + i] = (q.dy[i] << 16) | (q.dx[i] & 0xFFFF);
        }
    for (int l = 0; l < 2 * P.n2; ++l)
        for (int h = 0; h < 2; ++h) {
            const DyDx q = pattern_dydx(L->modes2[l >> 1], (l & 1) + 2 * h);
            for (int i = 0; i < 3; ++i) P.s2dyx[l][3 * h + i] = (q.dy[i] << 16) | (q.dx[i] & 0xFFFF);
        }
    P.emit = (uint32_t*)a.emit; P.emit_sn = a.emit_sn;
    P.feat = nullptr; P.feat_sn = 0;
    if constexpr ((KIND & LERF_FUSED_WARP) != 0) {
        if (!a.wgeo || !a.wboxes || a.workspace == nullptr || a.roi_h > 0 || a.items != nullptr) return LERF_EINVAL;
        P.wgeo = *a.wgeo;
        P.wboxes = a.wboxes;
    }
    auto set_s1off = [&](Params& Q, int pitch_kind) {
        for (int m = 0; m < Q.n1; ++m)
            for (int r = 0; r < 4; ++r) {
                const Off3 o = pitch_kind == 0 ? tile_offsets<D::IP>(L->modes1[m], r) : tile_offsets<DimsA::IP>(L->modes1[m], r);
                for (int i = 0; i < 3; ++i) Q.s1off[m][3 * r + i] = o.o[i];
            }
    };
    set_s1off(P, 0);
    bool two = a.workspace != nullptr && !(a.flags & LERF_GEO_SINGLE_LAUNCH);
#ifdef LERF_STAMPS
    size_t stamp_bytes = 0;
    {
        const size_t per = 16 * sizeof(unsigned long long);
        const size_t nb = (size_t)a.n * P.tiles_y * P.tiles_x;
        stamp_bytes = ((2 * nb + nb / 4 + 64) * per + 255) & ~(size_t)255;
        two = two && a.items == nullptr && !EMIT && a.workspace_bytes >= stamp_bytes + (size_t)a.n * feat_slice_bytes(a.H, a.W);
    }
#endif
    auto ka = s1_kernel<GEN>;
    auto kb = sr_fused_kernel<S, KIND, EMIT, true, GEN>;
    auto kc = sr_fused_kernel<S, KIND, EMIT, false, GEN>;
    int rc;
    if (two) {
        if ((rc = ensure_lds<s1_kernel<GEN>>(DimsA::LDS_BYTES)) != LERF_OK) return rc;
        if ((rc = ensure_lds<sr_fused_kernel<S, KIND, EMIT, true, GEN>>(D::LDS_BYTES)) != LERF_OK) return rc;
    } else if ((rc = ensure_lds<sr_fused_kernel<S, KIND, EMIT, false, GEN>>(D::LDS_BYTES)) != LERF_OK) return rc;

    if constexpr (GEN) {
        if (a.items != nullptr) {
            size_t ws_off = 0;
            for (int i0 = 0; i0 < a.n_items; i0 += RAGGED_MAX) {
                RaggedTable T{};
                T.n = a.n_items - i0 < RAGGED_MAX ? a.n_items - i0 : RAGGED_MAX;
                int64_t blocks = 0;
                for (int k = 0; k < T.n; ++k) {
                    const FusedItem& it = a.items[i0 + k];
                    FrameDesc& d = T.d[k];
                    d.img = it.img; d.out = it.out; d.emit = (uint32_t*)it.emit;
                    d.left_r = it.left_r; d.dis_r = it.dis_r; d.left_c = it.left_c; d.dis_c = it.dis_c;
                    d.dis_r64 = (it.dis_r64 && it.dis_c64) ? it.dis_r64 : nullptr;
                    d.dis_c64 = (it.dis_r64 && it.dis_c64) ? it.dis_c64 : nullptr;
                    d.H = it.H; d.W = it.W; d.oH = it.oH; d.oW = it.oW;
                    d.tiles_x = (it.W + TW - 1) / TW; d.tiles_y = (it.H + TH - 1) / TH;
                    d.first_block = (int)blocks;
                    blocks += (int64_t)d.tiles_x * d.tiles_y;
                    d.feat = two ? (uint8_t*)a.workspace + ws_off : nullptr;
                    if (two) ws_off += feat_slice_bytes(it.H, it.W);
                }
                if (blocks > 0x7FFFFFFF) return LERF_EUNSUPPORTED;
                if (two) {
                    Params Pa = P;
                    set_s1off(Pa, 1);
                    hipLaunchKernelGGL(ka, dim3((unsigned)blocks), dim3(NT), DimsA::LDS_BYTES, st, Pa, T);
                    hipLaunchKernelGGL(kb, dim3((unsigned)blocks), dim3(NT), D::LDS_BYTES, st, P, T);
                } else {
                    hipLaunchKernelGGL(kc, dim3((unsigned)blocks), dim3(NT), D::LDS_BYTES, st, P, T);
                }
            }
            return LERF_OK;
        }
    }
    const int64_t blocks = (int64_t)a.n * P.tiles_y * P.tiles_x;
    if (blocks > 0x7FFFFFFF) return LERF_EUNSUPPORTED;
    TableT T{};
    if (two) {
        P.feat = (uint8_t*)a.workspace;
#ifdef LERF_STAMPS
        P.feat += stamp_bytes;
#endif
        P.feat_sn = (int64_t)feat_slice_bytes(a.H, a.W);
        Params Pa = P;
#ifdef LERF_STAMPS
        Pa.stamps = P.stamps + (size_t)blocks * 16;
#endif
        set_s1off(Pa, 1);
        int64_t blocks1 = blocks;
        if (roi) {
            const int reach = R2 + D::R3;
            const int y0 = a.roi_y - reach > 0 ? a.roi_y - reach : 0, x0 = a.roi_x - reach > 0 ? (a.roi_x - reach) & ~3 : 0;
            const int y1 = a.roi_y + a.roi_h + reach < a.H ? a.roi_y + a.roi_h + reach : a.H;
            const int x1 = a.roi_x + a.roi_w + reach < a.W ? a.roi_x + a.roi_w + reach : a.W;
            Pa.ty_org = y0; Pa.tx_org = x0;
            Pa.tiles_y = (y1 - y0 + TH - 1) / TH; Pa.tiles_x = (x1 - x0 + TW - 1) / TW;
            blocks1 = (int64_t)a.n * Pa.tiles_y * Pa.tiles_x;
            if (blocks1 > 0x7FFFFFFF) return LERF_EUNSUPPORTED;
        }
        hipLaunchKernelGGL(ka, dim3((unsigned)blocks1), dim3(NT), DimsA::LDS_BYTES, st, Pa, T);
        hipLaunchKernelGGL(kb, dim3((unsigned)blocks), dim3(NT), D::LDS_BYTES, st, P, T);
        return LERF_OK;
    }
    hipLaunchKernelGGL(kc, dim3((unsigned)blocks), dim3(NT), D::LDS_BYTES, st, P, T);
    return LERF_OK;
}

template <bool GEN>
static int launch_sr(const FusedArgs& a, hipStream_t st) {
    if (a.kind == LERF_KIND_GAUSS) {
        if (a.S == 2) return launch_fused_t<2, LERF_KIND_GAUSS, false, GEN>(a, st);
        if (a.S == 4) return launch_fused_t<4, LERF_KIND_GAUSS, false, GEN>(a, st);
    } else if (a.kind == LERF_KIND_LINEAR) {
        if (a.S == 2) return launch_fused_t<2, LERF_KIND_LINEAR, false, GEN>(a, st);
    }
    return LERF_EUNSUPPORTED;
}
#ifdef LERF_FUSED_WITH_WARP
static int launch_warp(const FusedArgs& a, hipStream_t st) {
    if (a.kind == LERF_KIND_GAUSS) return launch_fused_t<2, LERF_KIND_GAUSS | LERF_FUSED_WARP, false, false>(a, st);
    if (a.kind == LERF_KIND_LINEAR) return launch_fused_t<2, LERF_KIND_LINEAR | LERF_FUSED_WARP, false, false>(a, st);
    return LERF_EUNSUPPORTED;
}
#endif
template <bool GEN>
static int launch_stages(const FusedArgs& a, hipStream_t st) {
    if (a.luts->oC == 3) return launch_fused_t<2, LERF_KIND_GAUSS, true, GEN>(a, st);
    if (a.luts->oC == 1) return launch_fused_t<2, LERF_KIND_LINEAR, true, GEN>(a, st);
    return LERF_EUNSUPPORTED;
}

}
}
```

### lerf-pytorch_amd/csrc/lerf_host_geometry.h

```cpp
#pragma once

#include <math.h>
#include <stdint.h>

#include "lerf_hip.h"

#ifdef __HIPCC__
#define LERF_HD __host__ __device__
#else
#define LERF_HD
#endif

namespace lerf {

constexpr float kEps32 = 1.1920928955078125e-07f;

LERF_HD inline int clampi(int v, int lo, int hi) { return v < lo ? lo : (v > hi ? hi : v); }

LERF_HD inline bool mode_pattern(char mode, int8_t dy[4], int8_t dx[4]) {
    dy[0] = 0; dx[0] = 0;
    switch (mode) {
        case 's': dy[1] = 0; dx[1] = 1; dy[2] = 1; dx[2] = 0; dy[3] = 1; dx[3] = 1; return true;
        case 'd': dy[1] = 0; dx[1] = 2; dy[2] = 2; dx[2] = 0; dy[3] = 2; dx[3] = 2; return true;
        case 'y': dy[1] = 1; dx[1] = 1; dy[2] = 1; dx[2] = 2; dy[3] = 2; dx[3] = 1; return true;
        case 'c': dy[1] = 0; dx[1] = 1; dy[2] = 0; dx[2] = 2; dy[3] = 0; dx[3] = 3; return true;
        case 't': dy[1] = 1; dx[1] = 1; dy[2] = 2; dx[2] = 2; dy[3] = 3; dx[3] = 3; return true;
        default: return false;
    }
}

LERF_HD inline bool mode_offsets(char mode, int rot, int8_t dy[4], int8_t dx[4]) {
    if (!mode_pattern(mode, dy, dx)) return false;
    rot &= 3;
    for (int k = 0; k < 4; ++k)
        for (int r = 0; r < rot; ++r) {
            int8_t t = dy[k];
            dy[k] = dx[k];
            dx[k] = (int8_t)(-t);
        }
    return true;
}

LERF_HD inline void project_unclipped(const double* m, int i, int j, double* row, double* col) {
#pragma clang fp contract(off)
    double x = (double)j, y = (double)i;
    double X = m[0] * x + m[1] * y + m[2];
    double Y = m[3] * x + m[4] * y + m[5];
    double Wh = m[6] * x + m[7] * y + m[8];
    X = X / Wh;
    Y = Y / Wh;
    *row = Y;
    *col = X;
}

LERF_HD inline void project_point(const double* m, int i, int j, int H, int W, double* gr, double* gc) {
    double r, c;
    project_unclipped(m, i, j, &r, &c);
    r = r < 0.0 ? 0.0 : (r > (double)H ? (double)H : r);
    c = c < 0.0 ? 0.0 : (c > (double)W ? (double)W : c);
    *gr = r;
    *gc = c;
}

LERF_HD inline int left_boundary(double g, int S) {
#pragma clang fp contract(off)
    return (int)ceil(g - (double)S / 2 - (double)kEps32);
}


LERF_HD inline int pad_index(int i, int n, int mode, bool* zero) {
    *zero = false;
    if (i >= 0 && i < n) return i;
    if (mode == 1) return i < 0 ? 0 : n - 1;
    if (mode == 2) {
        const int p = 2 * (n - 1);
        if (p == 0) return 0;
        const int m = ((i % p) + p) % p;
        return m < n ? m : p - m;
    }
    if (mode == 3) {
        const int p = 2 * n;
        const int m = ((i % p) + p) % p;
        return m < n ? m : p - 1 - m;
    }
    if (mode == 4) return ((i % n) + n) % n;
    *zero = true;
    return i < 0 ? 0 : n - 1;
}

struct WarpPixel {
    double gr, gc;
    int lr, lc;
};

LERF_HD inline WarpPixel pixel_of_point(double gr, double gc, int S, int pad_r_lo, int pad_c_lo) {
    WarpPixel p;
    p.gr = gr;
    p.gc = gc;
    p.lr = left_boundary(p.gr, S) + pad_r_lo;
    p.lc = left_boundary(p.gc, S) + pad_c_lo;
    p.gr += (double)pad_r_lo;
    p.gc += (double)pad_c_lo;
    return p;
}

LERF_HD inline WarpPixel warp_pixel(const double minv[9], int S, int pad_r_lo, int pad_c_lo, int i, int j, int H, int W) {
    double gr, gc;
    project_point(minv, i, j, H, W, &gr, &gc);
    return pixel_of_point(gr, gc, S, pad_r_lo, pad_c_lo);
}

LERF_HD inline double clip_coord(double v, int n) { return !(v >= 0.0) ? 0.0 : (v > (double)n ? (double)n : v); }

LERF_HD inline WarpPixel remap_pixel(double row, double col, int S, int pad_r_lo, int pad_c_lo, int H, int W) {
    return pixel_of_point(clip_coord(row, H), clip_coord(col, W), S, pad_r_lo, pad_c_lo);
}

LERF_HD inline int remap_pad_lo(double v0, int n, int S) {
    const int l = left_boundary(clip_coord(v0, n), S);
    return -l > 0 ? -l : 0;
}

struct SourceTap {
    int cl;
    bool inside;
    int s;
    bool z;
};

LERF_HD inline SourceTap source_tap(int s, int n, int pad_mode) {
    SourceTap t;
    t.cl = clampi(s, 0, n - 1);
    t.inside = s == t.cl;
    t.s = pad_index(s, n, pad_mode, &t.z);
    return t;
}

struct AxisTap : SourceTap {
    double d;
};

LERF_HD inline AxisTap axis_tap(double g, int l, int k, int n, int pad_lo, int pad_mode) {
    AxisTap t;
    const int p = clampi(l + k, 0, n - 1);
    t.d = g - (double)p;
    const SourceTap s = source_tap(p - pad_lo, n, pad_mode);
    t.cl = s.cl;
    t.inside = s.inside;
    t.s = s.s;
    t.z = s.z;
    return t;
}


namespace host {

inline int dclass(double x) { return (x >= -1.0 && x < 0.0) ? 1 : ((x >= 0.0 && x <= 1.0) ? 2 : 0); }
inline int fclass(float x) { return (x >= -1.0f && x < 0.0f) ? 1 : ((x >= 0.0f && x <= 1.0f) ? 2 : 0); }

inline float class_preserving_f32(double d) {
    float f = (float)d;
    int want = dclass(d);
    if (fclass(f) == want) return f;
    float up = nextafterf(f, INFINITY), dn = nextafterf(f, -INFINITY);
    if (fclass(up) == want) return up;
    if (fclass(dn) == want) return dn;
    return f;
}


inline int out_size(int n_in, double scale) { return (int)ceil(scale * (double)n_in); }

inline int sr_axis_tables(int n_in, int n_out, double scale, int S, int32_t* left, double* dis64, float* dis32,
                        int32_t* pads) {
#pragma clang fp contract(off)
    if (n_in < 1 || n_out < 1 || !(scale > 0.0) || S < 1 || S > LERF_MAX_SUPPORT || !left || !dis64) return LERF_EINVAL;
    const double a = (double)(n_in - 1) / 2;
    const double b = (double)(n_out - 1) / (2 * scale);
    int pad_lo = 0;
    for (int i = 0; i < n_out; ++i) {
        double g = (double)i / scale + a - b;
        int l = left_boundary(g, S);
        if (i == 0) pad_lo = -l;
        left[i] = l;
        double gp = g + (double)pad_lo;
        for (int k = 0; k < S; ++k) {
            double d = gp - (double)(l + pad_lo + k);
            dis64[i * S + k] = d;
            if (dis32) dis32[i * S + k] = class_preserving_f32(d);
        }
    }
    if (pads) {
        pads[0] = pad_lo;
        pads[1] = left[n_out - 1] + S - 1 - n_in + 1;
    }
    return LERF_OK;
}

inline int sr_axis_tables_f32(int n_in, int n_out, double scale, int S, int32_t* left, float* dis32, int32_t* pads) {
#pragma clang fp contract(off)
    if (n_in < 1 || n_out < 1 || !(scale > 0.0) || S < 1 || S > LERF_MAX_SUPPORT || !left || !dis32) return LERF_EINVAL;
    const float sf = (float)scale;
    const float a = (float)((double)(n_in - 1) / 2);
    const float b = (float)((double)(n_out - 1) / (2 * scale));
    const float half = (float)((double)S / 2);
    int pad_lo = 0;
    for (int i = 0; i < n_out; ++i) {
        float g = (float)i / sf;
        g = g + a;
        g = g - b;
        float t = g - half;
        t = t - kEps32;
        const int l = (int)ceilf(t);
        if (i == 0) pad_lo = -l;
        left[i] = l;
        const float gp = g + (float)pad_lo;
        for (int k = 0; k < S; ++k) dis32[i * S + k] = gp - (float)(l + pad_lo + k);
    }
    if (pads) {
        pads[0] = pad_lo;
        pads[1] = left[n_out - 1] + S - 1 - n_in + 1;
    }
    return LERF_OK;
}

inline int invert3x3(const double m[9], double out[9]) {
    if (!m || !out) return LERF_EINVAL;
    double c00 = m[4] * m[8] - m[5] * m[7], c01 = m[5] * m[6] - m[3] * m[8], c02 = m[3] * m[7] - m[4] * m[6];
    double det = m[0] * c00 + m[1] * c01 + m[2] * c02;
    if (det == 0.0) return LERF_EINVAL;
    out[0] = c00 / det;
    out[1] = (m[2] * m[7] - m[1] * m[8]) / det;
    out[2] = (m[1] * m[5] - m[2] * m[4]) / det;
    out[3] = c01 / det;
    out[4] = (m[0] * m[8] - m[2] * m[6]) / det;
    out[5] = (m[2] * m[3] - m[0] * m[5]) / det;
    out[6] = c02 / det;
    out[7] = (m[1] * m[6] - m[0] * m[7]) / det;
    out[8] = (m[0] * m[4] - m[1] * m[3]) / det;
    return LERF_OK;
}

inline int warp_pads(const double minv[9], int in_h, int in_w, int out_h, int out_w, int S, int32_t pads[4]) {
    if (!minv || !pads || in_h < 1 || in_w < 1 || out_h < 1 || out_w < 1 || S < 1) return LERF_EINVAL;
    double gr, gc;
    project_point(minv, 0, 0, in_h, in_w, &gr, &gc);
    int l0r = left_boundary(gr, S), l0c = left_boundary(gc, S);
    project_point(minv, out_h - 1, out_w - 1, in_h, in_w, &gr, &gc);
    int l1r = left_boundary(gr, S), l1c = left_boundary(gc, S);
    pads[0] = -l0r > 0 ? -l0r : 0;
    pads[1] = (l1r + S - 1 - in_h + 1) > 0 ? (l1r + S - 1 - in_h + 1) : 0;
    pads[2] = -l0c > 0 ? -l0c : 0;
    pads[3] = (l1c + S - 1 - in_w + 1) > 0 ? (l1c + S - 1 - in_w + 1) : 0;
    return LERF_OK;
}

inline int remap_geometry(const lerf_remap_geo_t* geo, int H, int W, double* gr, double* gc, int32_t* lr, int32_t* lc, int32_t pads[2]) {
    if (!geo || !geo->coords || H < 1 || W < 1 || geo->out_h < 1 || geo->out_w < 1 || geo->S < 1 || geo->S > LERF_MAX_SUPPORT) return LERF_EINVAL;
    if ((geo->coords_dtype != LERF_F32 && geo->coords_dtype != LERF_F64) || geo->row_stride < 2 * (int64_t)geo->out_w) return LERF_EINVAL;
    auto entry = [&](int i, int j, int k) -> double {
        const int64_t o = (int64_t)i * geo->row_stride + 2 * (int64_t)j + k;
        return geo->coords_dtype == LERF_F32 ? (double)((const float*)geo->coords)[o] : ((const double*)geo->coords)[o];
    };
    const int pr = geo->pad_r_lo < 0 ? remap_pad_lo(entry(0, 0, 0), H, geo->S) : geo->pad_r_lo;
    const int pc = geo->pad_c_lo < 0 ? remap_pad_lo(entry(0, 0, 1), W, geo->S) : geo->pad_c_lo;
    if (pads) { pads[0] = pr; pads[1] = pc; }
    for (int i = 0; i < geo->out_h; ++i)
        for (int j = 0; j < geo->out_w; ++j) {
            const WarpPixel p = remap_pixel(entry(i, j, 0), entry(i, j, 1), geo->S, pr, pc, H, W);
            const int64_t o = (int64_t)i * geo->out_w + j;
            if (gr) gr[o] = p.gr;
            if (gc) gc[o] = p.gc;
            if (lr) lr[o] = p.lr;
            if (lc) lc[o] = p.lc;
        }
    return LERF_OK;
}

LERF_HD inline void warp_owner_key(const double minv[9], int pad_r_lo, int pad_c_lo, int i, int j, int H, int W, int* key_r, int* key_c) {
    const WarpPixel p = warp_pixel(minv, 2, pad_r_lo, pad_c_lo, i, j, H, W);
    const int r0 = axis_tap(p.gr, p.lr, 0, H, pad_r_lo, LERF_PAD_CONSTANT).cl, c0 = axis_tap(p.gc, p.lc, 0, W, pad_c_lo, LERF_PAD_CONSTANT).cl;
    *key_r = r0 + 1 < H - 1 ? r0 + 1 : H - 1;
    *key_c = c0 + 1 < W - 1 ? c0 + 1 : W - 1;
}

inline int warp_tile_boxes(const double minv[9], int pad_r_lo, int pad_c_lo, int H, int W, int oH, int oW, int tile, int32_t* boxes) {
    if (!minv || !boxes || H < 1 || W < 1 || oH < 1 || oW < 1 || tile < 1) return LERF_EINVAL;
    const int ty = (H + tile - 1) / tile, tx = (W + tile - 1) / tile;
    for (int t = 0; t < ty * tx; ++t) { boxes[4 * t] = oH; boxes[4 * t + 1] = -1; boxes[4 * t + 2] = oW; boxes[4 * t + 3] = -1; }
    for (int i = 0; i < oH; ++i)
        for (int j = 0; j < oW; ++j) {
            int kr, kc;
            warp_owner_key(minv, pad_r_lo, pad_c_lo, i, j, H, W, &kr, &kc);
            int32_t* b = boxes + 4 * ((kr / tile) * tx + kc / tile);
            if (i < b[0]) b[0] = i;
            if (i > b[1]) b[1] = i;
            if (j < b[2]) b[2] = j;
            if (j > b[3]) b[3] = j;
        }
    for (int t = 0; t < ty * tx; ++t) {
        int32_t* b = boxes + 4 * t;
        if (b[1] < 0) { b[0] = b[1] = b[2] = b[3] = 0; continue; }
        b[0] = b[0] - 2 > 0 ? b[0] - 2 : 0;
        b[1] = b[1] + 3 < oH ? b[1] + 3 : oH;
        b[2] = b[2] - 2 > 0 ? b[2] - 2 : 0;
        b[3] = b[3] + 3 < oW ? b[3] + 3 : oW;
    }
    return LERF_OK;
// ... 33 lines not shown
```

### lerf-pytorch_amd/csrc/lerf_host_sanitize.cpp

```cpp
#include "lerf_host_geometry.h"

using namespace lerf;

extern "C" {
int lerf_abi_version(void) { return LERF_ABI_VERSION; }
int lerf_mode_offsets(char mode, int rot, int8_t dy[4], int8_t dx[4]) {
    if (!dy || !dx) return LERF_EINVAL;
    return mode_offsets(mode, rot, dy, dx) ? LERF_OK : LERF_EINVAL;
}
int lerf_out_size(int n_in, double scale) { return host::out_size(n_in, scale); }
int lerf_sr_axis_tables(int n_in, int n_out, double scale, int S, int32_t* left, double* dis64, float* dis32, int32_t* pads) {
    return host::sr_axis_tables(n_in, n_out, scale, S, left, dis64, dis32, pads);
}
int lerf_sr_axis_tables_f32(int n_in, int n_out, double scale, int S, int32_t* left, float* dis32, int32_t* pads) {
    return host::sr_axis_tables_f32(n_in, n_out, scale, S, left, dis32, pads);
}
int lerf_invert3x3(const double m[9], double out[9]) { return host::invert3x3(m, out); }
int lerf_warp_pads(const double minv[9], int in_h, int in_w, int out_h, int out_w, int S, int32_t pads[4]) {
    return host::warp_pads(minv, in_h, in_w, out_h, out_w, S, pads);
}
int lerf_warp_tile_boxes(const lerf_warp_geo_t* geo, int H, int W, int32_t* boxes) {
    if (!geo || geo->S != 2) return LERF_EINVAL;
    return host::warp_tile_boxes(geo->minv, geo->pad_r_lo, geo->pad_c_lo, H, W, geo->out_h, geo->out_w, 64, boxes);
}
int lerf_rr_adjoint_csr(int n_in, int n_out, int taps, const int32_t* left, const void* w, int w_dtype, int pad_mode,
                        int32_t* row_ptr, int32_t* idx, void* wt) {
    return host::rr_adjoint_csr(n_in, n_out, taps, left, w, w_dtype, pad_mode, row_ptr, idx, wt);
}
int lerf_remap_host_geometry(const lerf_remap_geo_t* geo, int H, int W, double* gr, double* gc, int32_t* lr, int32_t* lc,
                             int32_t pads[2]) {
    return host::remap_geometry(geo, H, W, gr, gc, lr, lc, pads);
}
int lerf_rr_axis(const void*, int, int64_t, int64_t, const lerf_rr_axis_t*, int, void*, int, void*) { return LERF_ENODEVICE; }
}
```

### lerf-pytorch_amd/ops.py

```python
from __future__ import annotations

import ctypes as C

import numpy as np

from . import _lib
from ._lib import KINDS


def _torch():
    return _lib.require_gpu()


class SrGeometry:

    def __init__(self, in_hw, scale_factors=None, out_hw=None, support=2, device=None, arithmetic="f64", dis_scale=1.0,
                 pad_mode=0):
        torch = _torch()
        H, W = int(in_hw[0]), int(in_hw[1])
        if out_hw is not None and scale_factors is None:
            scale_factors = [out_hw[0] / H, out_hw[1] / W]
        if not isinstance(scale_factors, (list, tuple)):
            scale_factors = [scale_factors, scale_factors]
        sh, sw = float(scale_factors[0]), float(scale_factors[1])
        if not (sh > 0.0 and sw > 0.0):
            raise ValueError("scale factors must be positive")
        if not 1 <= int(support) <= _lib.LERF_MAX_SUPPORT:
            raise NotImplementedError("support size {} (after anti-aliasing enlargement) exceeds the kernels' maximum of {}"
                                      .format(support, _lib.LERF_MAX_SUPPORT))
        if out_hw is None:
            out_hw = (_lib.out_size(H, sh), _lib.out_size(W, sw))
        self.in_hw, self.out_hw, self.scales, self.S = (H, W), (int(out_hw[0]), int(out_hw[1])), (sh, sw), int(support)
        self.device = torch.device(device if device is not None else "cuda")
        self.pad_mode = int(pad_mode)
        tables = {"f64": _lib.sr_axis_tables, "torch32": _lib.sr_axis_tables_f32}[arithmetic]
        lr, dr64, dr32, pr = tables(H, self.out_hw[0], sh, self.S)
        lc, dc64, dc32, pc = tables(W, self.out_hw[1], sw, self.S)
        if float(dis_scale) != 1.0:
            dr64, dc64 = float(dis_scale) * dr64, float(dis_scale) * dc64
            dr32, dc32 = dr64.astype(np.float32), dc64.astype(np.float32)
        self.pad_vec = ((0, 0), pr, pc)
        self.host = dict(left_r=lr, dis_r=dr64, dis_r32=dr32, left_c=lc, dis_c=dc64, dis_c32=dc32)
        if sh == 2.0 and sw == 2.0 and arithmetic == "f64" and float(dis_scale) == 1.0 and self.S == 2 \
                and self.out_hw == (2 * H, 2 * W):
            self.flags = _lib.GEO_X2_TABLES
        self._upload()

    def _upload(self):
        torch = _torch()
        h = self.host
        up = lambda a: torch.from_numpy(np.ascontiguousarray(a)).to(self.device)
        self.t = dict(left_r=up(h["left_r"]), dis_r=up(h["dis_r32"]), left_c=up(h["left_c"]), dis_c=up(h["dis_c32"]),
                      dis_r64=up(h["dis_r"]), dis_c64=up(h["dis_c"]))
        g = _lib.SrGeo()
        g.S, g.out_h, g.out_w = self.S, self.out_hw[0], self.out_hw[1]
        g.pad_mode = getattr(self, "pad_mode", 0)
        g.tie_queue_cap = int(getattr(self, "tie_queue_cap", 0))
        g.roi_y, g.roi_x, g.roi_h, g.roi_w = getattr(self, "roi", (0, 0, 0, 0))
        g.flags = int(getattr(self, "flags", 0))
        for k in ("left_r", "dis_r", "left_c", "dis_c", "dis_r64", "dis_c64"):
            setattr(g, k, self.t[k].data_ptr())
        self.struct = g

    def with_tie_queue_cap(self, cap):
        g = object.__new__(SrGeometry)
        g.__dict__.update(self.__dict__)
        g.tie_queue_cap = 0 if cap is None else (-1 if int(cap) == 0 else int(cap))
        g._upload()
        return g

    def with_flags(self, flags):
        g = object.__new__(SrGeometry)
        g.__dict__.update(self.__dict__)
        g.flags = int(getattr(self, "flags", 0)) | int(flags)
        g._upload()
        return g

    def _check_partition_pad(self):
        if self.pad_mode == _lib.PAD_MODES["wrap"]:
            raise ValueError("strip / block partitions do not support pad_mode 'wrap' (the far side of the frame is on another rank)")

    def row_slice(self, lr_row0, lr_rows, out_row0, out_row1):
        self._check_partition_pad()
        g = object.__new__(SrGeometry)
        g.in_hw = (int(lr_rows), self.in_hw[1])
        g.out_hw = (int(out_row1 - out_row0), self.out_hw[1])
        g.scales, g.S, g.device, g.pad_vec = self.scales, self.S, self.device, self.pad_vec
        g.pad_mode = self.pad_mode
        g.flags = int(getattr(self, "flags", 0))
        h = self.host
        g.host = dict(left_r=(h["left_r"][out_row0:out_row1] - lr_row0).astype(np.int32),
                      dis_r=h["dis_r"][out_row0:out_row1], dis_r32=h["dis_r32"][out_row0:out_row1],
                      left_c=h["left_c"], dis_c=h["dis_c"], dis_c32=h["dis_c32"])
        g._upload()
        return g

    def block_slice(self, lr_row0, lr_rows, out_row0, out_row1, lr_col0, lr_cols, out_col0, out_col1, roi=None):
        g = self.row_slice(lr_row0, lr_rows, out_row0, out_row1)
        h = self.host
        g.in_hw = (int(lr_rows), int(lr_cols))
        g.out_hw = (int(out_row1 - out_row0), int(out_col1 - out_col0))
        g.host.update(left_c=(h["left_c"][out_col0:out_col1] - lr_col0).astype(np.int32),
                      dis_c=h["dis_c"][out_col0:out_col1], dis_c32=h["dis_c32"][out_col0:out_col1])
        if roi is not None:
            g.roi = tuple(int(v) for v in roi)
        g._upload()
        return g

    def ref(self):
        return C.byref(self.struct)


class WarpGeometry:

    def __init__(self, in_hw, matrix, out_hw, support=2, pad_mode=0, out_rect=None, src_y0=0):
        m = np.asarray(matrix.detach().cpu().numpy() if hasattr(matrix, "detach") else matrix, dtype=np.float64)
        if m.shape != (3, 3):
            raise ValueError("matrix must be 3x3")
        self.matrix = m
        self.minv = np.linalg.inv(m)
        self.in_hw, self.out_hw, self.S = (int(in_hw[0]), int(in_hw[1])), (int(out_hw[0]), int(out_hw[1])), int(support)
        pads = _lib.warp_pads(self.minv, self.in_hw, self.out_hw, self.S)
        self.pad_vec = ((0, 0), (pads[0], pads[1]), (pads[2], pads[3]))
        g = _lib.WarpGeo()
        g.S, g.out_h, g.out_w = self.S, self.out_hw[0], self.out_hw[1]
        for i, v in enumerate(self.minv.reshape(9)):
            g.minv[i] = float(v)
        g.pad_r_lo, g.pad_r_hi, g.pad_c_lo, g.pad_c_hi = pads
        g.pad_mode = self.pad_mode = int(pad_mode)
        self.full_out_hw = self.out_hw
        if out_rect is not None:
            i0, i1, j0, j1 = (int(v) for v in out_rect)
            if not (0 <= i0 < i1 <= self.out_hw[0] and 0 <= j0 < j1 <= self.out_hw[1]):
                raise ValueError("out_rect outside the output")
            g.out_y0, g.out_x0, g.out_h, g.out_w = i0, j0, i1 - i0, j1 - j0
            self.out_hw = (i1 - i0, j1 - j0)
        g.src_y0 = self.src_y0 = int(src_y0)
        self.struct = g

    def ref(self):
        return C.byref(self.struct)

    def tile_boxes(self, device):
        torch = _torch()
        key = str(device)
        cache = self.__dict__.setdefault("_boxes", {})
        if key not in cache:
            H, W = self.in_hw
            nt = ((H + 63) // 64) * ((W + 63) // 64)
            b = np.zeros((nt, 4), dtype=np.int32)
            _lib.check(_lib.lib().lerf_warp_tile_boxes(self.ref(), H, W, b.ctypes.data), "lerf_warp_tile_boxes")
            cache[key] = (torch.from_numpy(b).to(device), b)
        return cache[key][0]


class RemapGeometry:

    def __init__(self, in_hw, coords, support=2, pad_mode=0, pads=None):
        self.in_hw, self.S, self.pad_mode = (int(in_hw[0]), int(in_hw[1])), int(support), int(pad_mode)
        if self.in_hw[0] < 1 or self.in_hw[1] < 1:
            raise ValueError("in_hw must be positive")
        dev = getattr(coords, "is_cuda", False)
        c = coords if dev else np.asarray(coords.detach().numpy() if hasattr(coords, "detach") else coords)
        if c.ndim not in (3, 4) or c.shape[-1] != 2 or any(n < 1 for n in c.shape[:-1]):
            raise ValueError("coords must be [oH, oW, 2] or [B, oH, oW, 2]")
        self.batched = c.ndim == 4
        self.n_maps = int(c.shape[0]) if self.batched else 1
        if dev:
            torch = _torch()
            c = c.detach()
            if c.dtype not in (torch.float32, torch.float64):
                raise ValueError("coords must be float32 or float64")
# ... 864 lines not shown
```

Before: 29080 Mpix/s.

## Add exact-x2 fused SR path computing geometry analytically instead of LDS tables

Result: faster. 29380 Mpix/s, median of 6 (+1.0%).

```diff
diff --git a/include/lerf_hip.h b/include/lerf_hip.h
--- a/include/lerf_hip.h
+++ b/include/lerf_hip.h
@@ -88,6 +88,8 @@
 #define LERF_GEO_TILE_ROWS_16 256
 #define LERF_GEO_INPUT_DEVICE 4
 #define LERF_GEO_INPUT_HOST 8
+#define LERF_GEO_EXACT_X2 512
+#define LERF_GEO_FORCE_TABLES 1024
 
 typedef struct {
     int S;
@@ -120,6 +122,12 @@
                         int32_t* left, double* dis64, float* dis32, int32_t* pads);
 
 int lerf_sr_axis_tables_f32(int n_in, int n_out, double scale, int S, int32_t* left, float* dis32, int32_t* pads);
+
+int lerf_sr_x2_tables(int n_out, int S, int32_t* left, double* dis64, float* dis32);
+int lerf_sr_x2_owned(int n_in, int tile, int32_t* ranges);
+int lerf_sr_geometry_flags(int H, int W, int out_h, int out_w, double scale_h, double scale_w, int S,
+                           const int32_t* left_r, const double* dis_r64, const float* dis_r32,
+                           const int32_t* left_c, const double* dis_c64, const float* dis_c32);
 
 int lerf_out_size(int n_in, double scale);
 
diff --git a/lerf-pytorch_amd/_lib.py b/lerf-pytorch_amd/_lib.py
--- a/lerf-pytorch_amd/_lib.py
+++ b/lerf-pytorch_amd/_lib.py
@@ -29,6 +29,7 @@
 
 EXPORTS = [
     "lerf_abi_version", "lerf_strerror", "lerf_device_count", "lerf_mode_offsets", "lerf_sr_axis_tables", "lerf_sr_axis_tables_f32",
+    "lerf_sr_x2_tables", "lerf_sr_x2_owned", "lerf_sr_geometry_flags",
     "lerf_out_size", "lerf_invert3x3", "lerf_warp_pads", "lerf_lut_interp_i16", "lerf_lut_interp", "lerf_lut_interp_ex", "lerf_numer_epilogue_f32", "lerf_fused_lutpack_bytes", "lerf_fused_lutpack_build",
     "lerf_lut_stages_u8",
     "lerf_resize", "lerf_warp", "lerf_sr_fused_workspace_bytes", "lerf_sr_fused_supported", "lerf_sr_fused_u8",
@@ -100,6 +101,7 @@
 
 GEO_FORCE_GENERAL, GEO_SINGLE_LAUNCH, GEO_INPUT_DEVICE, GEO_INPUT_HOST, GEO_X2_TABLES, GEO_NO_PERSIST = 1, 2, 4, 8, 16, 32
 GEO_TILE_ROWS_64, GEO_TILE_ROWS_32, GEO_TILE_ROWS_16 = 64, 128, 256
+GEO_EXACT_X2, GEO_FORCE_TABLES = 512, 1024
 
 
 class SrItem(C.Structure):
@@ -190,6 +192,9 @@
     L.lerf_mode_offsets.argtypes = [C.c_char, C.c_int, C.c_void_p, C.c_void_p]
     L.lerf_sr_axis_tables.argtypes = [C.c_int, C.c_int, C.c_double, C.c_int, C.c_void_p, C.c_void_p, C.c_void_p, C.c_void_p]
     L.lerf_sr_axis_tables_f32.argtypes = [C.c_int, C.c_int, C.c_double, C.c_int, C.c_void_p, C.c_void_p, C.c_void_p]
+    L.lerf_sr_x2_tables.argtypes = [C.c_int, C.c_int, C.c_void_p, C.c_void_p, C.c_void_p]
+    L.lerf_sr_x2_owned.argtypes = [C.c_int, C.c_int, C.c_void_p]
+    L.lerf_sr_geometry_flags.argtypes = [C.c_int, C.c_int, C.c_int, C.c_int, C.c_double, C.c_double, C.c_int] + [C.c_void_p] * 6
     L.lerf_out_size.argtypes = [C.c_int, C.c_double]
     L.lerf_invert3x3.argtypes = [C.c_void_p, C.c_void_p]
     L.lerf_warp_pads.argtypes = [C.c_void_p, C.c_int, C.c_int, C.c_int, C.c_int, C.c_int, C.c_void_p]
@@ -401,6 +406,30 @@
     return left, dis64, dis32, (int(pads[0]), int(pads[1]))
 
 
+def sr_x2_tables(n_out: int, S: int):
+    left = np.empty(n_out, np.int32)
+    dis64 = np.empty((n_out, S), np.float64)
+    dis32 = np.empty((n_out, S), np.float32)
+    check(lib().lerf_sr_x2_tables(int(n_out), int(S), left.ctypes.data, dis64.ctypes.data, dis32.ctypes.data), "lerf_sr_x2_tables")
+    return left, dis64, dis32
+
+
+def sr_x2_owned(n_in: int, tile: int):
+    r = np.empty(((int(n_in) + int(tile) - 1) // int(tile), 2), np.int32)
+    check(lib().lerf_sr_x2_owned(int(n_in), int(tile), r.ctypes.data), "lerf_sr_x2_owned")
+    return r
+
+
+def sr_geometry_flags(in_hw, out_hw, scales, S, left_r, dis_r64, dis_r32, left_c, dis_c64, dis_c32) -> int:
+    arrs = [np.ascontiguousarray(a, t) for a, t in ((left_r, np.int32), (dis_r64, np.float64), (dis_r32, np.float32),
+                                                    (left_c, np.int32), (dis_c64, np.float64), (dis_c32, np.float32))]
+    if arrs[0].size != out_hw[0] or arrs[3].size != out_hw[1] or any(a.size != n * S for a, n in
+                                                                     zip(arrs[1:3] + arrs[4:6], (out_hw[0],) * 2 + (out_hw[1],) * 2)):
+        return 0
+    return int(lib().lerf_sr_geometry_flags(int(in_hw[0]), int(in_hw[1]), int(out_hw[0]), int(out_hw[1]), float(scales[0]), float(scales[1]),
+                                            int(S), *[a.ctypes.data for a in arrs]))
+
+
 def sr_axis_tables_f32(n_in: int, n_out: int, scale: float, S: int):
     left = np.zeros(n_out, np.int32)
     dis32 = np.zeros((n_out, S), np.float32)
diff --git a/lerf-pytorch_amd/csrc/lerf_api.hip b/lerf-pytorch_amd/csrc/lerf_api.hip
--- a/lerf-pytorch_amd/csrc/lerf_api.hip
+++ b/lerf-pytorch_amd/csrc/lerf_api.hip
@@ -96,6 +96,18 @@
 
 int lerf_sr_axis_tables_f32(int n_in, int n_out, double scale, int S, int32_t* left, float* dis32, int32_t* pads) {
     return host::sr_axis_tables_f32(n_in, n_out, scale, S, left, dis32, pads);
+}
+
+int lerf_sr_x2_tables(int n_out, int S, int32_t* left, double* dis64, float* dis32) {
+    return host::sr_x2_tables(n_out, S, left, dis64, dis32);
+}
+
+int lerf_sr_x2_owned(int n_in, int tile, int32_t* ranges) { return host::sr_x2_owned(n_in, tile, ranges); }
+
+int lerf_sr_geometry_flags(int H, int W, int out_h, int out_w, double scale_h, double scale_w, int S, const int32_t* left_r,
+                           const double* dis_r64, const float* dis_r32, const int32_t* left_c, const double* dis_c64,
+                           const float* dis_c32) {
+    return host::sr_geometry_flags(H, W, out_h, out_w, scale_h, scale_w, S, left_r, dis_r64, dis_r32, left_c, dis_c64, dis_c32);
 }
 
 int lerf_invert3x3(const double m[9], double out[9]) { return host::invert3x3(m, out); }
diff --git a/lerf-pytorch_amd/csrc/lerf_fused.hip b/lerf-pytorch_amd/csrc/lerf_fused.hip
--- a/lerf-pytorch_amd/csrc/lerf_fused.hip
+++ b/lerf-pytorch_amd/csrc/lerf_fused.hip
@@ -1,5 +1,6 @@
 #define LERF_FUSED_NS fused
 #define LERF_FUSED_CH 3
+#define LERF_FUSED_X2 1
 #define LERF_FUSED_WITH_WARP 1
 #include "lerf_fused_impl.h"
 
diff --git a/lerf-pytorch_amd/csrc/lerf_fused_impl.h b/lerf-pytorch_amd/csrc/lerf_fused_impl.h
--- a/lerf-pytorch_amd/csrc/lerf_fused_impl.h
+++ b/lerf-pytorch_amd/csrc/lerf_fused_impl.h
@@ -1153,19 +1153,100 @@
     unsigned n, magic;
     __device__ __forceinline__ explicit MagicDiv(int n_)
         : n((unsigned)n_), magic((unsigned)((0x100000000ull + (unsigned)n_ - 1) / (unsigned)(n_ > 0 ? n_ : 1))) {}
+    __device__ __forceinline__ constexpr MagicDiv(unsigned n_, unsigned magic_) : n(n_), magic(magic_) {}
     __device__ __forceinline__ int div(int t) const { return n == 1 ? t : (int)__umulhi((unsigned)t, magic); }
+    template <bool KNOWN, int N>
+    __device__ __forceinline__ static MagicDiv of(int n_) {
+        constexpr bool POW2 = N > 1 && (N & (N - 1)) == 0;
+        if (KNOWN && POW2 && n_ == N) return MagicDiv((unsigned)N, (unsigned)(0x100000000ull / (unsigned)N));
+        return MagicDiv(n_);
+    }
 };
 
 template <typename D, int S>
-struct GeoTables {
-    int* lr; float* dr; int* lc; float* dc; int* grp;
-    __device__ __forceinline__ explicit GeoTables(uint8_t* smem)
-        : lr(reinterpret_cast<int*>(smem + D::OFF_GEO)), dr(reinterpret_cast<float*>(lr + D::GEO_ROWS)), lc(reinterpret_cast<int*>(dr + D::GEO_ROWS * S)),
-          dc(reinterpret_cast<float*>(lc + D::GEO_COLS)), grp(reinterpret_cast<int*>(dc + D::GEO_COLS * S)) {}
+struct GeoTab {
+    static constexpr bool X2 = false;
+    int* lr_; float* dr_; int* lc_; float* dc_; int* grp_; int* cgrp_;
+    const double* dis_r64; const double* dis_c64;
+    int i0, j0;
+    __device__ __forceinline__ explicit GeoTab(uint8_t* smem)
+        : lr_(reinterpret_cast<int*>(smem + D::OFF_GEO)), dr_(reinterpret_cast<float*>(lr_ + D::GEO_ROWS)), lc_(reinterpret_cast<int*>(dr_ + D::GEO_ROWS * S)),
+          dc_(reinterpret_cast<float*>(lc_ + D::GEO_COLS)), grp_(reinterpret_cast<int*>(dc_ + D::GEO_COLS * S)),
+          cgrp_(reinterpret_cast<int*>(smem + D::OFF_CGRP)), dis_r64(nullptr), dis_c64(nullptr), i0(0), j0(0) {}
+    __device__ __forceinline__ int lr(int il) const { return lr_[il]; }
+    __device__ __forceinline__ int lc(int jl) const { return lc_[jl]; }
+    __device__ __forceinline__ float dr(int il, int b) const { return dr_[il * S + b]; }
+    __device__ __forceinline__ float dc(int jl, int a) const { return dc_[jl * S + a]; }
+    __device__ __forceinline__ float dr_pair(int pair, int off, int b) const { return dr_[(2 * pair + off) * S + b]; }
+    __device__ __forceinline__ float dc_pair(int pair, int off, int a) const { return dc_[(2 * pair + off) * S + a]; }
+    __device__ __forceinline__ int grp(int g) const { return grp_[g]; }
+    __device__ __forceinline__ int cgrp(int h) const { return cgrp_[h]; }
+    __device__ __forceinline__ void dis64(int il, int jl, double (&dx)[S], double (&dy)[S]) const {
+#pragma unroll
+        for (int b = 0; b < S; ++b) dx[b] = dis_r64[(int64_t)(i0 + il) * S + b];
+#pragma unroll
+        for (int a = 0; a < S; ++a) dy[a] = dis_c64[(int64_t)(j0 + jl) * S + a];
+    }
 };
 
-template <typename D>
+template <typename D, int S>
+struct GeoX2 {
+    static constexpr bool X2 = true;
+    static_assert(S == 2, "the exact-x2 flavour serves the 2 x 2 support");
+    int rbase, cbase;
+    int nrow, ncol;
+    bool rows_align;
+    float kd[2][S];
+    __device__ __forceinline__ explicit GeoX2(uint8_t*) {}
+    __device__ __forceinline__ void set(int i0, int j0, int nrow_, int ncol_, int ty0, int tx0, bool rows_align_, float gscale) {
+        rbase = i0 + 1 - 2 * ty0; cbase = j0 + 1 - 2 * tx0;
+        nrow = nrow_; ncol = ncol_; rows_align = rows_align_;
+#pragma unroll
+        for (int p = 0; p < 2; ++p)
+#pragma unroll
+            for (int k = 0; k < S; ++k) {
+                kd[p][k] = (float)x2_dis(p, k, S) * gscale;
+            }
+    }
+    __device__ __forceinline__ int lr(int il) const { return (il + rbase) >> 1; }
+    __device__ __forceinline__ int lc(int jl) const { return (jl + cbase) >> 1; }
+    __device__ __forceinline__ float dr(int il, int b) const { return ((il + rbase) & 1) ? kd[0][b] : kd[1][b]; }
+    __device__ __forceinline__ float dc(int jl, int a) const { return ((jl + cbase) & 1) ? kd[0][a] : kd[1][a]; }
+    __device__ __forceinline__ float dr_pair(int, int off, int b) const { return ((off + rbase) & 1) ? kd[0][b] : kd[1][b]; }
+    __device__ __forceinline__ float dc_pair(int, int off, int a) const { return ((off + cbase) & 1) ? kd[0][a] : kd[1][a]; }
+    __device__ __forceinline__ int grp(int g) const { return rows_align ? min(max(2 * g - rbase, 0), nrow) : g; }
+    __device__ __forceinline__ int ngrp() const { return rows_align ? (nrow + rbase + 1) >> 1 : nrow; }
+    __device__ __forceinline__ int cgrp(int h) const { return min(max(2 * h - cbase, 0), ncol); }
+    __device__ __forceinline__ int ncgrp() const { return (ncol + cbase + 1) >> 1; }
+    __device__ __forceinline__ int gsame() const {
+        const int ng = ngrp();
+        if (ng == 0) return 0;
+        const int first = grp(1) - grp(0), last = nrow - grp(ng - 1);
+        return (first == last && (ng <= 2 || grp(2) - grp(1) == first)) ? first : 0;
+    }
+    __device__ __forceinline__ int rcode() const { return (rbase == 0 || nrow <= 1) ? 1 : 2; }
+    __device__ __forceinline__ int ccode() const { return (cbase == 0 || ncol <= 1) ? 1 : 2; }
+    __device__ __forceinline__ void dis64(int il, int jl, double (&dx)[S], double (&dy)[S]) const {
+#pragma unroll
+        for (int b = 0; b < S; ++b) dx[b] = x2_dis(il + rbase + 1, b, S);
+#pragma unroll
+        for (int a = 0; a < S; ++a) dy[a] = x2_dis(jl + cbase + 1, a, S);
+    }
+};
+
+template <typename D, bool X2>
 __device__ __forceinline__ void stage3_geo_search(const FrameView& F, int tyi, int txi, int ty0, int tx0, int* ctl, int tid) {
+    if constexpr (X2) {
+        if (tid < 2) {
+            int o0, o1;
+            if (tid == 0) x2_owned(tyi, F.tiles_y, ty0, TH, F.oH, &o0, &o1);
+            else x2_owned(txi, F.tiles_x, tx0, TW, F.oW, &o0, &o1);
+            ctl[CTL_I0 + 2 * tid] = o0;
+            ctl[CTL_I1 + 2 * tid] = o1;
+            if (tid == 0) ctl[CTL_TQ_COUNT] = 0;
+        }
+        return;
+    }
     const int lane = tid & 63, wave = tid >> 6;
     if (wave < 4) {
         const bool rows = wave < 2;
@@ -1181,22 +1262,22 @@
 template <typename D, int S, int KIND>
 __device__ __forceinline__ void stage3_geo_stage(uint8_t* smem, const FrameView& F, float max_sigma, int hy0, int hx0, const int* ctl,
                                                  int tid) {
-    const GeoTables<D, S> g(smem);
+    const GeoTab<D, S> g(smem);
     const int gi0 = ctl[CTL_I0], gi1 = ctl[CTL_I1], gj0 = ctl[CTL_J0], gj1 = ctl[CTL_J1];
     const float gscale = KIND == LERF_KIND_GAUSS ? s3::gauss_scale(max_sigma) : 1.0f;
     for (int e = tid; e < gi1 - gi0; e += NT) {
-        g.lr[e] = F.left_r[gi0 + e] - hy0;
-#pragma unroll
-        for (int b = 0; b < S; ++b) g.dr[e * S + b] = F.dis_r[(gi0 + e) * S + b] * gscale;
+        g.lr_[e] = F.left_r[gi0 + e] - hy0;
+#pragma unroll
+        for (int b = 0; b < S; ++b) g.dr_[e * S + b] = F.dis_r[(gi0 + e) * S + b] * gscale;
     }
     for (int e = tid; e < gj1 - gj0; e += NT) {
-        g.lc[e] = F.left_c[gj0 + e] - hx0;
-#pragma unroll
-        for (int a = 0; a < S; ++a) g.dc[e * S + a] = F.dis_c[(gj0 + e) * S + a] * gscale;
-    }
-}
-
-template <typename D_, int S_, int KIND_>
+        g.lc_[e] = F.left_c[gj0 + e] - hx0;
+#pragma unroll
+        for (int a = 0; a < S; ++a) g.dc_[e * S + a] = F.dis_c[(gj0 + e) * S + a] * gscale;
+    }
+}
+
+template <typename D_, int S_, int KIND_, bool X2_ = false>
 struct Stage3 {
     using D = D_;
     static constexpr int S = S_, SS = S_ * S_, KIND = KIND_;
@@ -1206,30 +1287,34 @@
     static constexpr bool BLKL = KIND_ == LERF_KIND_LINEAR && S_ == 2 && D::OUT_FITS;
     static constexpr int QRP = S_ == 4 ? 2 : 1, QCP = S_ == 4 ? 2 : 1;
     static constexpr bool QUADS = BLK && QRP * QCP > 1;
-    GeoTables<D, S> g;
+    static constexpr bool X2 = X2_;
+    std::conditional_t<X2_, GeoX2<D_, S_>, GeoTab<D_, S_>> geo;
     const uint32_t* Dt;
     uint32_t* tq; int* tq_count;
     uint8_t* outt;
-    int* cgrp;
-    const double* dis_r64; const double* dis_c64;
+    bool guard;
     uint8_t* seg0;
     int64_t rowpitch;
     bool rows_align;
     int i0, j0, nrow, ncol;
     int ncolc, ndw, ophase;
     MagicDiv by_ndw;
-    int ngrp, gsame, rcode, ccode;
+    int ngrp, gsame, rcode, ccode, ncgrp;
     bool lin_ok;
 
-    __device__ __forceinline__ Stage3(uint8_t* smem, const Params& P, const FrameView& F, uint8_t* outp, int* ctl) : g(smem), by_ndw(1) {
+    __device__ __forceinline__ Stage3(uint8_t* smem, const Params& P, const FrameView& F, uint8_t* outp, int* ctl, int ty0, int tx0)
+        : geo(smem), by_ndw(1) {
         Dt = reinterpret_cast<const uint32_t*>(smem + D::OFF_D);
         tq = reinterpret_cast<uint32_t*>(smem + D::OFF_TQ);
         tq_count = ctl + CTL_TQ_COUNT;
         outt = smem + D::OFF_OUT;
-        cgrp = reinterpret_cast<int*>(smem + D::OFF_CGRP);
-        dis_r64 = F.dis_r64; dis_c64 = F.dis_c64;
+        guard = F.dis_r64 != nullptr;
         i0 = ctl[CTL_I0]; j0 = ctl[CTL_J0];
         nrow = ctl[CTL_I1] - i0; ncol = ctl[CTL_J1] - j0;
+        if constexpr (X2) {
+            i0 = __builtin_amdgcn_readfirstlane(i0); j0 = __builtin_amdgcn_readfirstlane(j0);
+            nrow = __builtin_amdgcn_readfirstlane(nrow); ncol = __builtin_amdgcn_readfirstlane(ncol);
+        }
         ncolc = ncol * CH;
         rowpitch = P.out_pitch > 0 ? (int64_t)P.out_pitch : (int64_t)F.oW * CH;
         seg0 = outp + (int64_t)i0 * rowpitch + (int64_t)j0 * CH;
@@ -1237,13 +1322,28 @@
         const bool seg_aligned = rows_align && (reinterpret_cast<uintptr_t>(seg0) & 3u) == 0;
         ndw = seg_aligned ? (ncolc + 3) >> 2 : (ncolc + 6) >> 2;
         ophase = (int)(reinterpret_cast<uintptr_t>(seg0) & 15u);
+        if constexpr (X2) {
+            geo.set(i0, j0, nrow, ncol, ty0, tx0, rows_align, GAUSS ? s3::gauss_scale(P.max_sigma) : 1.0f);
+        } else {
+            geo.dis_r64 = F.dis_r64; geo.dis_c64 = F.dis_c64; geo.i0 = i0; geo.j0 = j0;
+        }
     }
     __device__ __forceinline__ void read_census(const int* ctl) {
+        if constexpr (X2) {
+            ngrp = geo.ngrp();
+            gsame = __builtin_amdgcn_readfirstlane(geo.gsame());
+            rcode = __builtin_amdgcn_readfirstlane(geo.rcode()); ccode = __builtin_amdgcn_readfirstlane(geo.ccode());
+            ncgrp = __builtin_amdgcn_readfirstlane(geo.ncgrp());
+            lin_ok = BLKL;
+            by_ndw = MagicDiv(ndw);
+            return;
+        }
         ngrp = ctl[CTL_NGRP];
         gsame = __builtin_amdgcn_readfirstlane(ctl[CTL_GSAME]);
         rcode = __builtin_amdgcn_readfirstlane(ctl[CTL_RCODE]); ccode = __builtin_amdgcn_readfirstlane(ctl[CTL_CCODE]);
         if constexpr (BLKL) lin_ok = ctl[CTL_LIN_ROWS_OK] != 0 && ctl[CTL_LIN_COLS_OK] != 0;
         else lin_ok = false;
+        ncgrp = 0;
         by_ndw = MagicDiv(ndw);
     }
 };
@@ -1261,12 +1361,13 @@
 
 template <typename X_>
 __device__ __forceinline__ void stage3_census(const X_& X, int* ctl, int tid) {
+  if constexpr (!X_::X2) {
     constexpr int KIND = X_::KIND, GMAX = X_::GMAX;
     const int lane = tid & 63, wave = tid >> 6;
     const int nrow = X.nrow, ncol = X.ncol;
-    const int* g_lr = X.g.lr;
-    const int* g_lc = X.g.lc;
-    int* g_grp = X.g.grp;
+    const int* g_lr = X.geo.lr_;
+    const int* g_lc = X.geo.lc_;
+    int* g_grp = X.geo.grp_;
     if (wave == 0) {
         int ng = 0;
         for (int base = 0; base < nrow; base += 64) {
@@ -1297,7 +1398,7 @@
             if (lane == 0) ctl[CTL_LIN_ROWS_OK] = ok ? 1 : 0;
         }
     } else if (wave == 1 && X_::BLKL) {
-        int* g_cgrp = X.cgrp;
+        int* g_cgrp = X.geo.cgrp_;
         constexpr int NCMAX = 2 * TW + 14;
         int nc = 0;
         for (int base = 0; base < ncol; base += 64) {
@@ -1325,6 +1426,7 @@
     } else if (wave == 2 && KIND == LERF_KIND_GAUSS) {
         pair_census(g_lr, nrow, lane, &ctl[CTL_RCODE], &ctl[CTL_RSTEP]);
     }
+  }
 }
 
 template <typename X_>
@@ -1333,9 +1435,10 @@
     constexpr int S = X_::S;
     const int jl = xc / CH;
     const int c = xc - jl * CH;
-    const uint32_t* dp = X.Dt + X.g.lr[il] * D::HP + X.g.lc[jl] * CH + c;
-    return s3::resolve_taps_u8<X_::GAUSS, S>([&](int a, int b) __attribute__((always_inline)) { return dp[b * D::HP + a * CH]; },
-                                            X.dis_r64 + (int64_t)(X.i0 + il) * S, X.dis_c64 + (int64_t)(X.j0 + jl) * S, max_sigma);
+    const uint32_t* dp = X.Dt + X.geo.lr(il) * D::HP + X.geo.lc(jl) * CH + c;
+    double dx[S], dy[S];
+    X.geo.dis64(il, jl, dx, dy);
+    return s3::resolve_taps_u8<X_::GAUSS, S>([&](int a, int b) __attribute__((always_inline)) { return dp[b * D::HP + a * CH]; }, dx, dy, max_sigma);
 }
 template <int N>
 __device__ __forceinline__ unsigned tie_mask(const float (&dist)[N]) {
@@ -1372,7 +1475,7 @@
     using D = typename X_::D;
     constexpr int S = X_::S, SS = X_::SS, KIND = X_::KIND;
     constexpr int GN = GS > 0 ? GS : X_::GMAX;
-    const int* g_lr = X.g.lr; const float* g_dr = X.g.dr; const int* g_lc = X.g.lc; const float* g_dc = X.g.dc; const int* g_grp = X.g.grp;
+    const auto& G = X.geo;
     const uint32_t* Dt = X.Dt;
     const int ndw = X.ndw, ncolc = X.ncolc;
     const int64_t rowpitch = X.rowpitch;
@@ -1381,12 +1484,12 @@
     for (int t = tid; t < ntask; t += NT) {
         const int g = X.by_ndw.div(t);
         const int dw = t - g * ndw;
-        const int il0 = g_grp[g];
-        const int gs = GS > 0 ? GS : g_grp[g + 1] - il0;
+        const int il0 = G.grp(g);
+        const int gs = GS > 0 ? GS : G.grp(g + 1) - il0;
         uint8_t* seg = X.seg0 + il0 * rowpitch;
         const int a0 = (int)(reinterpret_cast<uintptr_t>(seg) & 3u);
         const int b0 = dw * 4 - a0;
-        const int lr = g_lr[il0];
+        const int lr = G.lr(il0);
         uint32_t packed[GN];
         constexpr bool DIST = S == 2;
         float dist[DIST ? GN * 4 : 1];
@@ -1397,19 +1500,19 @@
         s3::f2 DXP[S];
         if constexpr (KIND == LERF_KIND_GAUSS && S == 4 && GS == 2) {
 #pragma unroll
-            for (int b = 0; b < S; ++b) { DXP[b].x = g_dr[il0 * S + b]; DXP[b].y = g_dr[(il0 + 1) * S + b]; }
+            for (int b = 0; b < S; ++b) { DXP[b].x = G.dr(il0, b); DXP[b].y = G.dr(il0 + 1, b); }
         }
 #pragma unroll
         for (int u = 0; u < 4; ++u) {
             const int xc = min(max(b0 + u, 0), ncolc - 1);
             const int jl = xc / CH;
             const int c = xc - jl * CH;
-            const int lc = g_lc[jl];
+            const int lc = G.lc(jl);
             if constexpr (KIND == LERF_KIND_GAUSS && S == 4 && GS == 2) {
                 s3::f2 PT[SS], KV[SS];
 #pragma unroll
                 for (int a = 0; a < S; ++a) {
-                    const float dy = g_dc[jl * S + a];
+                    const float dy = G.dc(jl, a);
 #pragma unroll
                     for (int b = 0; b < S; ++b) {
                         const uint32_t d = Dt[(lr + b) * D::HP + (lc + a) * CH + c];
@@ -1451,7 +1554,7 @@
             float p0[SS], k1[SS], ty[SS], v[SS];
 #pragma unroll
             for (int a = 0; a < S; ++a) {
-                const float dy = g_dc[jl * S + a];
+                const float dy = G.dc(jl, a);
 #pragma unroll
                 for (int b = 0; b < S; ++b) {
                     const uint32_t d = Dt[(lr + b) * D::HP + (lc + a) * CH + c];
@@ -1478,7 +1581,7 @@
                     for (int a = 0; a < S; ++a)
 #pragma unroll
                         for (int b = 0; b < S; ++b) {
-                            const float dx = g_dr[(il0 + r) * S + b];
+                            const float dx = G.dr(il0 + r, b);
                             if (KIND == LERF_KIND_GAUSS)
                                 e[a * S + b] = s3::gauss_form_cols(s3::gauss_t_u8(k1[a * S + b], dx), ty[a * S + b], p0[a * S + b]);
                             else
@@ -1496,7 +1599,7 @@
                 }
             }
         }
-        if ((DIST ? dmax > 0.5f - s3::kTieEps : tiebits != 0) && X.dis_r64 != nullptr) {
+        if ((DIST ? dmax > 0.5f - s3::kTieEps : tiebits != 0) && X.guard) {
             unsigned tiemask = tiebits;
             if (DIST) {
 #pragma unroll
@@ -1533,22 +1636,22 @@
     if constexpr (X_::BLK) {
         using D = typename X_::D;
         constexpr int S = X_::S;
-        const int* g_lr = X.g.lr; const float* g_dr = X.g.dr; const int* g_lc = X.g.lc; const float* g_dc = X.g.dc;
+        const auto& G = X.geo;
         const int nrow = X.nrow, ncol = X.ncol, ophase = X.ophase;
         const int rofs = UNI ? 0 : X.rcode - 1, cofs = UNI ? 0 : X.ccode - 1;
         const int ncg = (ncol + cofs + 1) >> 1;
         const int nblk = ((nrow + rofs + 1) >> 1) * ncg;
-        const MagicDiv by_ncg(ncg);
+        const MagicDiv by_ncg = MagicDiv::of<X_::X2, TW>(ncg);
         for (int t = tid; t < nblk; t += NT) {
             const int g = by_ncg.div(t);
             const int h = t - g * ncg;
             const int il0 = 2 * g - rofs, jl0 = 2 * h - cofs;
-            const int lr = g_lr[UNI ? il0 : max(il0, 0)], lc = g_lc[UNI ? jl0 : max(jl0, 0)];
+            const int lr = G.lr(UNI ? il0 : max(il0, 0)), lc = G.lc(UNI ? jl0 : max(jl0, 0));
             s3::f2 DX[S], DY[S];
 #pragma unroll
-            for (int b = 0; b < S; ++b) { DX[b].x = g_dr[il0 * S + b]; DX[b].y = g_dr[il0 * S + S + b]; }
-#pragma unroll
-            for (int a = 0; a < S; ++a) { DY[a].x = g_dc[jl0 * S + a]; DY[a].y = g_dc[jl0 * S + S + a]; }
+            for (int b = 0; b < S; ++b) { DX[b].x = G.dr_pair(g, -rofs, b); DX[b].y = G.dr_pair(g, 1 - rofs, b); }
+#pragma unroll
+            for (int a = 0; a < S; ++a) { DY[a].x = G.dc_pair(h, -cofs, a); DY[a].y = G.dc_pair(h, 1 - cofs, a); }
             const uint32_t* dp = X.Dt + lr * D::HP + lc * CH;
             uint8_t* ob = X.outt + il0 * D::OUT_PITCH + ophase + jl0 * CH;
             float dist[4 * CH];
@@ -1574,7 +1677,7 @@
                         put_block_byte(s3::finish_div(num, den), have, ob + r * D::OUT_PITCH + q * CH + c, dist[(c * 2 + r) * 2 + q], dmax);
                     }
             }
-            if (dmax > 0.5f - s3::kTieEps && X.dis_r64 != nullptr)
+            if (dmax > 0.5f - s3::kTieEps && X.guard)
                 queue_ties(X, P, tie_mask(dist),
                            [&](int q, int& il, int& xc) __attribute__((always_inline)) { il = il0 + ((q >> 1) & 1); xc = (jl0 + (q & 1)) * CH + (q >> 2); },
                            [&](int q, uint32_t r8) __attribute__((always_inline)) { ob[((q >> 1) & 1) * D::OUT_PITCH + (q & 1) * CH + (q >> 2)] = (uint8_t)r8; });
@@ -1587,7 +1690,7 @@
     if constexpr (X_::QUADS) {
         using D = typename X_::D;
         constexpr int S = X_::S, RP = X_::QRP, CP = X_::QCP, TR = S + RP - 1, TC = S + CP - 1;
-        const int* g_lr = X.g.lr; const float* g_dr = X.g.dr; const int* g_lc = X.g.lc; const float* g_dc = X.g.dc;
+        const auto& G = X.geo;
         const int ophase = X.ophase;
         const int ncq = (X.ncol >> 1) / CP;
         const int ntq = ((X.nrow >> 1) / RP) * ncq;
@@ -1596,16 +1699,16 @@
             const int g = by_ncq.div(t);
             const int h = t - g * ncq;
             const int il0 = 2 * RP * g, jl0 = 2 * CP * h;
-            const int lr = g_lr[il0], lc = g_lc[jl0];
+            const int lr = G.lr(il0), lc = G.lc(jl0);
             s3::f2 DX[RP][S], DY[CP][S];
 #pragma unroll
             for (int rp = 0; rp < RP; ++rp)
 #pragma unroll
-                for (int b = 0; b < S; ++b) { DX[rp][b].x = g_dr[(il0 + 2 * rp) * S + b]; DX[rp][b].y = g_dr[(il0 + 2 * rp + 1) * S + b]; }
+                for (int b = 0; b < S; ++b) { DX[rp][b].x = G.dr_pair(RP * g + rp, 0, b); DX[rp][b].y = G.dr_pair(RP * g + rp, 1, b); }
 #pragma unroll
             for (int cp = 0; cp < CP; ++cp)
 #pragma unroll
-                for (int a = 0; a < S; ++a) { DY[cp][a].x = g_dc[(jl0 + 2 * cp) * S + a]; DY[cp][a].y = g_dc[(jl0 + 2 * cp + 1) * S + a]; }
+                for (int a = 0; a < S; ++a) { DY[cp][a].x = G.dc_pair(CP * h + cp, 0, a); DY[cp][a].y = G.dc_pair(CP * h + cp, 1, a); }
             const uint32_t* dp = X.Dt + lr * D::HP + lc * CH;
             uint8_t* ob = X.outt + il0 * D::OUT_PITCH + ophase + jl0 * CH;
 #pragma unroll 1
@@ -1654,7 +1757,7 @@
                                 put_block_byte(s3::finish_div(num, den), true, ob + (2 * rp + r) * D::OUT_PITCH + (2 * cp + q) * CH + c,
                                                dist[((rp * CP + cp) * 2 + r) * 2 + q], dmax);
                             }
-                if (dmax > 0.5f - s3::kTieEps && X.dis_r64 != nullptr)
+                if (dmax > 0.5f - s3::kTieEps && X.guard)
                     queue_ties(X, P, tie_mask(dist),
                                [&](int k, int& il, int& xc) __attribute__((always_inline)) {
                                    const int rp = (k >> 2) / CP, cp = (k >> 2) - rp * CP;
@@ -1674,29 +1777,29 @@
 __device__ __forceinline__ void stage3_blocks_lin(const X_& X, const Params& P, const int* ctl, int tid) {
     if constexpr (X_::BLKL) {
         using D = typename X_::D;
-        const int* g_lr = X.g.lr; const float* g_dr = X.g.dr; const int* g_lc = X.g.lc; const float* g_dc = X.g.dc; const int* g_grp = X.g.grp;
-        const int* g_cgrp = X.cgrp;
+        const auto& G = X.geo;
         const int ophase = X.ophase;
         const float ms255 = P.max_sigma * (1.0f / 255.0f);
-        const int ncg = __builtin_amdgcn_readfirstlane(ctl[CTL_NCGRP]);
+        const int ncg = X_::X2 ? X.ncgrp : __builtin_amdgcn_readfirstlane(ctl[CTL_NCGRP]);
         const int nblk = X.ngrp * ncg;
-        const MagicDiv by_ncg(ncg);
+        const MagicDiv by_ncg = MagicDiv::of<X_::X2, TW>(ncg);
         for (int t = tid; t < nblk; t += NT) {
             const int g = by_ncg.div(t);
             const int h = t - g * ncg;
-            const int il0 = g_grp[g], jl0 = g_cgrp[h];
-            const bool two_r = g_grp[g + 1] - il0 > 1, two_c = g_cgrp[h + 1] - jl0 > 1;
-            const int lr = g_lr[il0], lc = g_lc[jl0];
+            const int il0 = G.grp(g), jl0 = G.cgrp(h);
+            const bool two_r = G.grp(g + 1) - il0 > 1, two_c = G.cgrp(h + 1) - jl0 > 1;
+            const int lr = G.lr(il0), lc = G.lc(jl0);
             float ax[2][2], mx[2][2], ay[2][2], my[2][2];
-            auto abs_and_mask = [](const float* d, float (&a)[2][2], float (&m)[2][2]) __attribute__((always_inline)) {
+            auto abs_and_mask = [](auto d, float (&a)[2][2], float (&m)[2][2]) __attribute__((always_inline)) {
 #pragma unroll
                 for (int k = 0; k < 4; ++k) {
-                    a[k >> 1][k & 1] = __builtin_fabsf(d[k]);
-                    m[k >> 1][k & 1] = s3::dist_class_f(d[k]) != 0 ? 1.0f : 0.0f;
+                    const float dk = d(k >> 1, k & 1);
+                    a[k >> 1][k & 1] = __builtin_fabsf(dk);
+                    m[k >> 1][k & 1] = s3::dist_class_f(dk) != 0 ? 1.0f : 0.0f;
                 }
             };
-            abs_and_mask(g_dr + il0 * 2, ax, mx);
-            abs_and_mask(g_dc + jl0 * 2, ay, my);
+            abs_and_mask([&](int r, int b) __attribute__((always_inline)) { return G.dr(il0 + r, b); }, ax, mx);
+            abs_and_mask([&](int q, int a) __attribute__((always_inline)) { return G.dc(jl0 + q, a); }, ay, my);
             const uint32_t* dp = X.Dt + lr * D::HP + lc * CH;
             uint8_t* ob = X.outt + il0 * D::OUT_PITCH + ophase + jl0 * CH;
             float dist[4 * CH];
@@ -1728,7 +1831,7 @@
                                        dist[(c * 2 + r) * 2 + q], dmax);
                     }
             }
-            if (dmax > 0.5f - s3::kTieEps && X.dis_r64 != nullptr)
+            if (dmax > 0.5f - s3::kTieEps && X.guard)
                 queue_ties(X, P, tie_mask(dist),
                            [&](int q, int& il, int& xc) __attribute__((always_inline)) { il = il0 + ((q >> 1) & 1); xc = (jl0 + (q & 1)) * CH + (q >> 2); },
                            [&](int q, uint32_t r8) __attribute__((always_inline)) { ob[((q >> 1) & 1) * D::OUT_PITCH + (q & 1) * CH + (q >> 2)] = (uint8_t)r8; });
@@ -1790,7 +1893,7 @@
         __syncthreads();
         LERF_STAMP(15);
     }
-    if (X.dis_r64 == nullptr) return;
+    if (!X.guard) return;
     if (!IMAGE) {
         asm volatile("s_waitcnt vmcnt(0)" ::: "memory");
         __syncthreads();
@@ -1807,11 +1910,13 @@
 }
 
 constexpr int LERF_FUSED_WARP = 16;
-template <int S, int KINDW, bool EMIT, bool FROM_FEAT = false, bool GEN = false>
+template <int S, int KINDW, bool EMIT, bool FROM_FEAT = false, bool GEN = false, bool X2 = false>
 __global__ void __launch_bounds__(NT)
 sr_fused_kernel(Params P, std::conditional_t<GEN, RaggedTable, NoTable> T) {
     constexpr int KIND = KINDW & 15;
     constexpr bool WARP = (KINDW & LERF_FUSED_WARP) != 0;
+    static_assert(!X2 || (!EMIT && !WARP && CH == 3 && S == 2), "exact-x2 flavour: the RGB SR kernels that run stage 3, 2 x 2 support");
+    static_assert(!X2 || Dims<S, GEN, EMIT>::GEO_EARLY, "exact-x2 flavour: the specialised RGB layout (geometry slot early: nothing to stage late)");
     static_assert(!WARP || (!EMIT && S == 2 && CH == 3 && !GEN), "tile-fused warp: RGB, 2 x 2 support, specialised kernel");
     using D = Dims<S, GEN, EMIT>;
     extern __shared__ __attribute__((aligned(16))) uint8_t smem[];
@@ -1840,8 +1945,8 @@
 #ifdef LERF_STAMPS
     if (tid == 0) { P.stamps[(size_t)blockIdx.x * 16 + 8] = 0; P.stamps[(size_t)blockIdx.x * 16 + 9] = 0; P.stamps[(size_t)blockIdx.x * 16 + 15] = 0; }
 #endif
-    auto geo_search = [&]() { stage3_geo_search<D>(F, tyi, txi, ty0, tx0, ctl, tid); };
-    auto geo_stage = [&]() { stage3_geo_stage<D, S, KIND>(smem, F, P.max_sigma, hy0, hx0, ctl, tid); };
+    auto geo_search = [&]() { stage3_geo_search<D, X2>(F, tyi, txi, ty0, tx0, ctl, tid); };
+    auto geo_stage = [&]() { if constexpr (!X2) stage3_geo_stage<D, S, KIND>(smem, F, P.max_sigma, hy0, hx0, ctl, tid); };
     auto early_search = [&]() { if (D::GEO_EARLY && !EMIT && !WARP) geo_search(); };
     if constexpr (!FROM_FEAT) {
         stage1<D, GEN, false, false>(smem, P, img, H, W, fy0, fx0, interior, Bt, tid, early_search, [&](int k) {
@@ -1894,11 +1999,13 @@
         geo_stage();
     }
     __syncthreads();
-    using X3 = Stage3<D, S, KIND>;
-    X3 X(smem, P, F, outp, ctl);
+    using X3 = Stage3<D, S, KIND, X2>;
+    X3 X(smem, P, F, outp, ctl, ty0, tx0);
     LERF_STAMP(11);
-    stage3_census(X, ctl, tid);
-    __syncthreads();
+    if constexpr (!X2) {
+        stage3_census(X, ctl, tid);
+        __syncthreads();
+    }
     X.read_census(ctl);
     const bool image_ok = X.rows_align && (X.rowpitch & 15) == 0 && X.nrow <= D::OUT_ROWS && X.ophase + X.ncolc <= D::OUT_PITCH;
     const bool blk = X3::BLK && image_ok && X.rcode != 0 && X.ccode != 0;
@@ -2000,7 +2107,7 @@
 
 inline size_t feat_slice_bytes(int H, int W) { return ((size_t)H * W * CH + 15) / 16 * 16; }
 
-template <int S, int KIND, bool EMIT, bool GEN>
+template <int S, int KIND, bool EMIT, bool GEN, bool X2 = false>
 static int launch_fused_t(const FusedArgs& a, hipStream_t st) {
     using D = Dims<S, GEN, EMIT>;
     using TableT = std::conditional_t<GEN, RaggedTable, NoTable>;
@@ -2066,15 +2173,15 @@
     }
 #endif
     auto ka = s1_kernel<GEN>;
-    auto kb = sr_fused_kernel<S, KIND, EMIT, true, GEN>;
-    auto kc = sr_fused_kernel<S, KIND, EMIT, false, GEN>;
+    auto kb = sr_fused_kernel<S, KIND, EMIT, true, GEN, X2>;
+    auto kc = sr_fused_kernel<S, KIND, EMIT, false, GEN, X2>;
     int rc;
     if (two) {
         if ((rc = ensure_lds<s1_kernel<GEN>>(DimsA::LDS_BYTES)) != LERF_OK) return rc;
-        if ((rc = ensure_lds<sr_fused_kernel<S, KIND, EMIT, true, GEN>>(D::LDS_BYTES)) != LERF_OK) return rc;
-    } else if ((rc = ensure_lds<sr_fused_kernel<S, KIND, EMIT, false, GEN>>(D::LDS_BYTES)) != LERF_OK) return rc;
-
-    if constexpr (GEN) {
+        if ((rc = ensure_lds<sr_fused_kernel<S, KIND, EMIT, true, GEN, X2>>(D::LDS_BYTES)) != LERF_OK) return rc;
+    } else if ((rc = ensure_lds<sr_fused_kernel<S, KIND, EMIT, false, GEN, X2>>(D::LDS_BYTES)) != LERF_OK) return rc;
+
+    if constexpr (GEN && !X2) {
         if (a.items != nullptr) {
             size_t ws_off = 0;
             for (int i0 = 0; i0 < a.n_items; i0 += RAGGED_MAX) {
@@ -2141,8 +2248,22 @@
     return LERF_OK;
 }
 
+static bool takes_x2(const FusedArgs& a) {
+    if (!(a.flags & LERF_GEO_EXACT_X2) || (a.flags & LERF_GEO_FORCE_TABLES) || CH != 3 || a.items != nullptr) return false;
+    if (a.S != 2) return false;
+    if (a.roi_h > 0 && a.roi_w > 0) return false;
+    return (int64_t)a.oH == 2 * (int64_t)a.H && (int64_t)a.oW == 2 * (int64_t)a.W;
+}
+
 template <bool GEN>
 static int launch_sr(const FusedArgs& a, hipStream_t st) {
+#ifdef LERF_FUSED_X2
+    if (takes_x2(a)) {
+        if (a.kind == LERF_KIND_GAUSS) return launch_fused_t<2, LERF_KIND_GAUSS, false, GEN, true>(a, st);
+        if (a.kind == LERF_KIND_LINEAR) return launch_fused_t<2, LERF_KIND_LINEAR, false, GEN, true>(a, st);
+        return LERF_EUNSUPPORTED;
+    }
+#endif
     if (a.kind == LERF_KIND_GAUSS) {
         if (a.S == 2) return launch_fused_t<2, LERF_KIND_GAUSS, false, GEN>(a, st);
         if (a.S == 4) return launch_fused_t<4, LERF_KIND_GAUSS, false, GEN>(a, st);
diff --git a/lerf-pytorch_amd/csrc/lerf_host_geometry.h b/lerf-pytorch_amd/csrc/lerf_host_geometry.h
--- a/lerf-pytorch_amd/csrc/lerf_host_geometry.h
+++ b/lerf-pytorch_amd/csrc/lerf_host_geometry.h
@@ -2,6 +2,7 @@
 
 #include <math.h>
 #include <stdint.h>
+#include <string.h>
 
 #include "lerf_hip.h"
 
@@ -67,6 +68,13 @@
     return (int)ceil(g - (double)S / 2 - (double)kEps32);
 }
 
+
+LERF_HD inline int x2_left(int i, int S) { return ((i + 1) >> 1) - S / 2; }
+LERF_HD inline double x2_dis(int i, int k, int S) { return (double)(S / 2 - k) - ((i & 1) ? 0.75 : 0.25); }
+LERF_HD inline void x2_owned(int ti, int tn, int t0, int tpx, int n_out, int* o0, int* o1) {
+    *o0 = ti == 0 ? 0 : 2 * t0 - 1;
+    *o1 = ti == tn - 1 ? n_out : 2 * (t0 + tpx) - 1;
+}
 
 LERF_HD inline int pad_index(int i, int n, int mode, bool* zero) {
     *zero = false;
@@ -224,6 +232,46 @@
     return LERF_OK;
 }
 
+inline int sr_x2_tables(int n_out, int S, int32_t* left, double* dis64, float* dis32) {
+    if (n_out < 1 || S < 1 || S > LERF_MAX_SUPPORT || (S & 1)) return LERF_EINVAL;
+    for (int i = 0; i < n_out; ++i) {
+        if (left) left[i] = x2_left(i, S);
+        for (int k = 0; k < S; ++k) {
+            if (dis64) dis64[i * S + k] = x2_dis(i, k, S);
+            if (dis32) dis32[i * S + k] = (float)x2_dis(i, k, S);
+        }
+    }
+    return LERF_OK;
+}
+
+inline int sr_x2_exact(int n_in, int n_out, double scale, int S, const int32_t* left, const double* dis64, const float* dis32) {
+    if (n_in < 1 || S < 1 || S > LERF_MAX_SUPPORT || (S & 1) || !left || !dis64 || !dis32) return 0;
+    if (scale != 2.0 || (int64_t)n_out != 2 * (int64_t)n_in) return 0;
+    for (int i = 0; i < n_out; ++i) {
+        if (left[i] != x2_left(i, S)) return 0;
+        for (int k = 0; k < S; ++k) {
+            const double d = x2_dis(i, k, S);
+            const float f = (float)d;
+            if (memcmp(&dis64[i * S + k], &d, sizeof d) != 0 || memcmp(&dis32[i * S + k], &f, sizeof f) != 0) return 0;
+        }
+    }
+    return 1;
+}
+
+inline int sr_x2_owned(int n_in, int tile, int32_t* ranges) {
+    if (n_in < 1 || tile < 1 || !ranges) return LERF_EINVAL;
+    const int tn = (n_in + tile - 1) / tile;
+    for (int t = 0; t < tn; ++t) x2_owned(t, tn, t * tile, tile, 2 * n_in, &ranges[2 * t], &ranges[2 * t + 1]);
+    return LERF_OK;
+}
+
+inline int sr_geometry_flags(int H, int W, int out_h, int out_w, double scale_h, double scale_w, int S, const int32_t* left_r,
+                             const double* dis_r64, const float* dis_r32, const int32_t* left_c, const double* dis_c64,
+                             const float* dis_c32) {
+    return sr_x2_exact(H, out_h, scale_h, S, left_r, dis_r64, dis_r32) && sr_x2_exact(W, out_w, scale_w, S, left_c, dis_c64, dis_c32)
+               ? LERF_GEO_EXACT_X2 : 0;
+}
+
 inline int invert3x3(const double m[9], double out[9]) {
     if (!m || !out) return LERF_EINVAL;
     double c00 = m[4] * m[8] - m[5] * m[7], c01 = m[5] * m[6] - m[3] * m[8], c02 = m[3] * m[7] - m[4] * m[6];
diff --git a/lerf-pytorch_amd/csrc/lerf_host_sanitize.cpp b/lerf-pytorch_amd/csrc/lerf_host_sanitize.cpp
--- a/lerf-pytorch_amd/csrc/lerf_host_sanitize.cpp
+++ b/lerf-pytorch_amd/csrc/lerf_host_sanitize.cpp
@@ -14,6 +14,15 @@
 }
 int lerf_sr_axis_tables_f32(int n_in, int n_out, double scale, int S, int32_t* left, float* dis32, int32_t* pads) {
     return host::sr_axis_tables_f32(n_in, n_out, scale, S, left, dis32, pads);
+}
+int lerf_sr_x2_tables(int n_out, int S, int32_t* left, double* dis64, float* dis32) {
+    return host::sr_x2_tables(n_out, S, left, dis64, dis32);
+}
+int lerf_sr_x2_owned(int n_in, int tile, int32_t* ranges) { return host::sr_x2_owned(n_in, tile, ranges); }
+int lerf_sr_geometry_flags(int H, int W, int out_h, int out_w, double scale_h, double scale_w, int S, const int32_t* left_r,
+                           const double* dis_r64, const float* dis_r32, const int32_t* left_c, const double* dis_c64,
+                           const float* dis_c32) {
+    return host::sr_geometry_flags(H, W, out_h, out_w, scale_h, scale_w, S, left_r, dis_r64, dis_r32, left_c, dis_c64, dis_c32);
 }
 int lerf_invert3x3(const double m[9], double out[9]) { return host::invert3x3(m, out); }
 int lerf_warp_pads(const double minv[9], int in_h, int in_w, int out_h, int out_w, int S, int32_t pads[4]) {
diff --git a/lerf-pytorch_amd/ops.py b/lerf-pytorch_amd/ops.py
--- a/lerf-pytorch_amd/ops.py
+++ b/lerf-pytorch_amd/ops.py
@@ -44,6 +44,9 @@
         if sh == 2.0 and sw == 2.0 and arithmetic == "f64" and float(dis_scale) == 1.0 and self.S == 2 \
                 and self.out_hw == (2 * H, 2 * W):
             self.flags = _lib.GEO_X2_TABLES
+        if arithmetic == "f64":
+            self.flags = int(getattr(self, "flags", 0)) | _lib.sr_geometry_flags(self.in_hw, self.out_hw, self.scales, self.S,
+                                                                                 lr, dr64, dr32, lc, dc64, dc32)
         self._upload()
 
     def _upload(self):
@@ -87,7 +90,7 @@
         g.out_hw = (int(out_row1 - out_row0), self.out_hw[1])
         g.scales, g.S, g.device, g.pad_vec = self.scales, self.S, self.device, self.pad_vec
         g.pad_mode = self.pad_mode
-        g.flags = int(getattr(self, "flags", 0))
+        g.flags = int(getattr(self, "flags", 0)) & ~_lib.GEO_EXACT_X2
         h = self.host
         g.host = dict(left_r=(h["left_r"][out_row0:out_row1] - lr_row0).astype(np.int32),
                       dis_r=h["dis_r"][out_row0:out_row1], dis_r32=h["dis_r32"][out_row0:out_row1],
```
